# HDembinski/zenflow

Hardware: AMD Instinct MI355X
Metric: log_prob samples/sec (+ NLL match) 4D 16-knot 4-layer flow, batch 2^20 (higher is better)
Workload: dtype fp32 (f16x2 split MFMA, fp32 accumulate)

## Files before the change

zenflow_amd/build.py:

```python

from __future__ import annotations

import hashlib
import os
import subprocess
import sys
from concurrent.futures import ThreadPoolExecutor
from pathlib import Path

HERE = Path(__file__).resolve().parent
CSRC = HERE / "csrc"
INCLUDE = HERE.parent / "include"
LIB = HERE / "libzenflow_amd.so"
ARCH = os.environ.get("ZF_OFFLOAD_ARCH", "gfx950")
HIPCC = os.environ.get("HIPCC", "/opt/rocm/bin/hipcc")

SOURCES = ["zf_runtime.hip", "zf_rqs.hip", "zf_flow.hip", "zf_flow_x3.hip", "zf_flow_x3_k8.hip", "zf_flow_x3_k16.hip", "zf_flow_x3_k32.hip", "zf_flow_x3_k64.hip", "zf_flow_x3_k64_act.hip", "zf_flow_x3_k8_act.hip", "zf_flow_x3_k16_act.hip", "zf_flow_x3_k32_act.hip", "zf_flow_x3_k8_act2.hip", "zf_flow_x3_k16_act2.hip", "zf_flow_x3_k32_act2.hip", "zf_stats.hip", "zf_rccl.hip", "zf_train.hip", "zf_layered.hip"]
HEADERS = sorted(p.name for p in CSRC.glob("*.h"))

FLAGS = [
    f"--offload-arch={ARCH}",
    "-O3",
    "-std=c++17",
    "-fPIC",
    "-shared",
    "-Wall",
    "-Wno-unused-function",
    "-Wno-unused-variable",
    "-Wno-unused-result",
    "-I/opt/rocm/include",
    f"-I{INCLUDE}",
]

X3_FLAGS = ["-fno-slp-vectorize"]


def _src_flags(src: str):
    return X3_FLAGS if src.startswith("zf_flow_x3_k") else []


def _fingerprint() -> str:
    h = hashlib.sha256()
    for f in SOURCES + HEADERS:
        h.update((CSRC / f).read_bytes())
    h.update((INCLUDE / "zenflow_amd.h").read_bytes())
    h.update(" ".join(FLAGS + X3_FLAGS).encode())
    return h.hexdigest()


def build(force: bool = False, verbose: bool = True, out: Path = LIB, extra=()) -> Path:
    stamp = out.parent / f".{out.stem}.sha256"
    fp = _fingerprint() + " ".join(extra)
    if not force and out.exists() and stamp.exists() and stamp.read_text() == fp:
        return out
    tmp = out.with_suffix(".so.tmp")
    objdir = HERE.parent / "build" / ("obj" if not extra else "obj_" + hashlib.sha1(" ".join(extra).encode()).hexdigest()[:8])
    objdir.mkdir(parents=True, exist_ok=True)
    compile_flags = [f for f in FLAGS if f != "-shared"] + list(extra)

    hdr = hashlib.sha256(b"".join((CSRC / f).read_bytes() for f in HEADERS) + (INCLUDE / "zenflow_amd.h").read_bytes())

    def _compile(src: str) -> Path:
        obj = objdir / (Path(src).stem + ".o")
        cmd = [HIPCC, *compile_flags, *_src_flags(src), "-c", "-o", str(obj), str(CSRC / src)]
        key = hashlib.sha256(hdr.digest() + (CSRC / src).read_bytes() + " ".join(cmd).encode()).hexdigest()
        ostamp = obj.with_suffix(".o.sha256")
        if not force and obj.exists() and ostamp.exists() and ostamp.read_text() == key:
            return obj
        if verbose:
            print("[zenflow_amd.build]", " ".join(cmd), flush=True)
        subprocess.run(cmd, check=True)
        ostamp.write_text(key)
        return obj

    jobs = max(1, min(len(SOURCES), int(os.environ.get("MAX_JOBS", os.cpu_count() or 1))))
    with ThreadPoolExecutor(jobs) as pool:
        objs = list(pool.map(_compile, SOURCES))
    cmd = [HIPCC, f"--offload-arch={ARCH}", "-shared", "-fPIC", "-o", str(tmp), *map(str, objs), "-ldl"]
    if verbose:
        print("[zenflow_amd.build]", " ".join(cmd), flush=True)
    subprocess.run(cmd, check=True)
    os.replace(tmp, out)
    stamp.write_text(fp)
    return out


if __name__ == "__main__":
    argv = sys.argv[1:]
    o = LIB
    if "--out" in argv:
        i = argv.index("--out")
        o = Path(argv[i + 1]).resolve()
        del argv[i : i + 2]
    build(force="--force" in argv, out=o, extra=[a for a in argv if a.startswith("-D")])
```

zenflow_amd/csrc/zf_flow.hip:

```cpp
#include "zf_flow_dev.h"

#include <cmath>
#include <cstdlib>
#include <cstring>
#include <vector>

namespace zf {
namespace {

constexpr int kWaves = 4;
constexpr int kBlockRows = kWaves * kTile;

template <int T>
__device__ __forceinline__ floatx16 mfma_tile(const floatx4* __restrict__ p,
                                              const floatx4* __restrict__ pnext, floatx4 (&cur)[4],
                                              const floatx16 (&hb)[T]) {
  floatx16 acc = floatx16{0};
#pragma unroll
  for (int t = 0; t < T; ++t) {
    floatx4 nxt[4];
    const bool more = (t + 1 < T);
    const floatx4* src = more ? p + (t + 1) * 256 : pnext;
    const bool have = more || (pnext != nullptr);
    if (have) {
#pragma unroll
      for (int r4 = 0; r4 < 4; ++r4) {
        nxt[r4] = src[r4 * 64];
      }
    }
    asm volatile("" ::: "memory");
#pragma unroll
    for (int r4 = 0; r4 < 4; ++r4)
#pragma unroll
      for (int e = 0; e < 4; ++e)
        acc = __builtin_amdgcn_mfma_f32_32x32x2f32(cur[r4][e], hb[t][4 * r4 + e], acc, 0, 0, 0);
    if (have) {
#pragma unroll
      for (int r4 = 0; r4 < 4; ++r4) cur[r4] = nxt[r4];
    }
  }
  return acc;
}

struct RingParams {
  const float* ring;
  int base;
  int K, mask;
  float sx, sy, rsx, rsy;
  float c, norm, rnorm;
  __device__ __forceinline__ float at(int q) const { return ring[(q & mask) << 5]; }
  __device__ __forceinline__ float w(int j) const {
    return div_cr(div_cr(at(base + j), sx, rsx) + c, norm, rnorm);
  }
  __device__ __forceinline__ float h(int j) const {
    return div_cr(div_cr(at(base + K + j), sy, rsy) + c, norm, rnorm);
  }
  __device__ __forceinline__ float d(int j) const { return squareplus_fast(at(base + 2 * K + j)); }
};

template <bool INV>
__device__ __forceinline__ void spline_pair(float* ring, float* xs, int s, int hh, int next_d, int end,
                                            int S, int K, int mask, float cth, float norm, float rnorm,
                                            int rot, int D, float& ldc) {
  const int d = next_d + hh;
  float ldv = 0.f;
  if (d < end) {
    RingParams p;
    p.ring = ring + s;
    p.base = d * S;
    p.K = K;
    p.mask = (mask << 5) | 31;
    p.c = cth;
    p.norm = norm;
    p.rnorm = rnorm;
    float* rp = ring + s;
    float sx = 0.f, sy = 0.f;
    for (int j = 0; j < K; ++j) {
      const int qx = p.base + j, qy = p.base + K + j;
      float* ax = rp + ((qx & p.mask) << 5);
      float* ay = rp + ((qy & p.mask) << 5);
      const float vx = squareplus_fast(*ax), vy = squareplus_fast(*ay);
      *ax = vx;
      *ay = vy;
      sx = sx + vx;
      sy = sy + vy;
    }
    p.sx = sx;
    p.sy = sy;
    p.rsx = rcp_refined(sx);
    p.rsy = rcp_refined(sy);
    float* xp = xs + wrap(d + rot, D) * 32 + s;
    const float xv = *xp;
    const RqsBin bin = rqs_bin<!INV>(xv, K, p);
    if (!INV) {
      float yv, l;
      rqs_forward_eval(xv, bin, yv, l);
      *xp = yv;
      ldv = l;
    } else {
      *xp = rqs_inverse_eval(xv, bin);
    }
  }
  wave_lds_sync();
  if (!INV) {
    const float other = __shfl_xor(ldv, 32);
    const float first = hh == 0 ? ldv : other;
    const float second = hh == 0 ? other : ldv;
    ldc = ldc + first;
    if (end - next_d == 2) ldc = ldc + second;
  }
}

template <int HP, bool INV>
__global__ __launch_bounds__(kWaves * 64, (HP <= 128 ? 2 : 1)) void flow_kernel(
    const DevFlow* __restrict__ F, const float* __restrict__ blob, const float* __restrict__ xin,
    const float* __restrict__ cin, float* __restrict__ y_out, const float* __restrict__ ld_in,
    float* __restrict__ ld_out, float* __restrict__ lp_out, double* __restrict__ block_partial,
    int op_begin, int op_end, long long N, unsigned long long seed, int gen) {
  constexpr int T = HP / 32;
  extern __shared__ __attribute__((aligned(16))) float lds[];
  __shared__ double s_part[kWaves];

  const int D = F->D;
  const int C = F->C;
  const int wave = threadIdx.x >> 6;
  const int lane = threadIdx.x & 63;
  const int s = lane & 31;
  const int hh = lane >> 5;
  float* xs = lds + wave * F->per_wave;
  float* ring = xs + 32 * D;
  const long long row = ((long long)blockIdx.x * kWaves + wave) * kTile + s;
  const bool valid = row < N;

  load_state(xs, xin, row, valid, D, s, hh, F, seed, INV ? gen : 0);
  float ld = (ld_in != nullptr && valid) ? ld_in[row] : 0.f;
  int rot = 0;
  wave_lds_sync();

  floatx4 wc[4];
  const int nq = op_end - op_begin;
  for (int q = 0; q < nq; ++q) {
    const int oi = INV ? (op_end - 1 - q) : (op_begin + q);
    const DevOp& op = F->ops[oi];
    const int kind = op.kind;
    if (kind == ZF_OP_ROLL) {
      rot = pmod(INV ? rot + op.shift : rot - op.shift, D);
    } else if (kind == ZF_OP_SHIFT_BOUNDS) {
      shift_bounds_op<INV>(blob + op.sb, xs, s, hh, rot, D, ld);
    } else {
      const int dt = op.dt;
      {
        const floatx4* f = reinterpret_cast<const floatx4*>(blob + op.first_chunk) + lane;
#pragma unroll
        for (int r4 = 0; r4 < 4; ++r4) wc[r4] = f[r4 * 64];
      }
      floatx16 hb[T];
      layer0<T>(op, blob, xs, cin, row, valid, C, rot, D, s, hh, lane, hb, T, op.act);
      for (int l = 1; l < op.n_hidden; ++l) {
        const floatx4* wl = reinterpret_cast<const floatx4*>(blob + op.w[l]) + lane;
        const floatx4* wnext = reinterpret_cast<const floatx4*>(blob + op.w[l + 1]) + lane;
        floatx16 ho[T];
#pragma unroll
        for (int o = 0; o < T; ++o) {
          const floatx4* nx = (o + 1 < T) ? wl + (o + 1) * T * 256 : wnext;
          floatx4 bv[4];
          bias_tile(blob + op.b[l] + o * 32, hh, bv);
          floatx16 acc = mfma_tile<T>(wl + o * T * 256, nx, wc, hb);
          if (op.act == ZF_ACT_SWISH) {
#pragma unroll
            for (int r = 0; r < 16; ++r) acc[r] = swish(acc[r] + bv[r >> 2][r & 3]);
          } else {
#pragma unroll
            for (int r = 0; r < 16; ++r) acc[r] = act_other(op.act, acc[r] + bv[r >> 2][r & 3]);
          }
          ho[o] = acc;
        }
#pragma unroll
        for (int o = 0; o < T; ++o) hb[o] = ho[o];
      }
      const int K = op.K, S = op.S, mask = op.nslot_mask;
      const floatx4* wl = reinterpret_cast<const floatx4*>(blob + op.w[op.n_hidden]) + lane;
      const float* bl = blob + op.b[op.n_hidden];
      const KnotConsts kc(K);
      const float cth = kc.c, norm = kc.norm, rnorm = kc.rnorm;
      int next_d = 0;
      float ldc = 0.f;
      const int T_last = op.T_last;
      for (int o = 0; o < T_last; ++o) {
        const floatx4* nx = (o + 1 < T_last) ? wl + (o + 1) * T * 256 : nullptr;
        floatx4 bv[4];
        bias_tile(bl + o * 32, hh, bv);
        floatx16 acc = mfma_tile<T>(wl + o * T * 256, nx, wc, hb);
        float* slot = ring + ((o & mask) << 10) + s;
#pragma unroll
        for (int r = 0; r < 16; ++r) {
          const int rr = (r & 3) + 8 * (r >> 2) + 4 * hh;
          slot[rr * 32] = acc[r] + bv[r >> 2][r & 3];
        }
        wave_lds_sync();
        if (o + 1 < T_last) {
          while (next_d < dt) {
            const int end = (next_d + 2 < dt) ? next_d + 2 : dt;
            if (end * S > (o + 1) * 32) break;
            spline_pair<INV>(ring, xs, s, hh, next_d, end, S, K, mask, cth, norm, rnorm, rot, D, ldc);
            next_d += 2;
          }
        }
      }
      while (next_d < dt) {
        const int end = (next_d + 2 < dt) ? next_d + 2 : dt;
        spline_pair<INV>(ring, xs, s, hh, next_d, end, S, K, mask, cth, norm, rnorm, rot, D, ldc);
        next_d += 2;
      }
      if (!INV) ld = ld + ldc;
    }
  }

  flow_epilogue<kWaves>(F, xs, s, hh, lane, wave, rot, D, row, valid, ld, lp_out, block_partial, 1, 0,
                        y_out, ld_out, s_part);
}

__global__ __launch_bounds__(256) void latent_sample_kernel(int latent, float param, unsigned long long seed,
                                                            float* __restrict__ z, long long n, int D) {
  const long long i = (long long)blockIdx.x * 256 + threadIdx.x;
  if (i >= n) return;
  const long long row = i / D;
  const int d = (int)(i - row * D);
  z[i] = latent_draw(latent, param, seed, row, d);
}

constexpr int kReduceThreads = 1024;
__global__ __launch_bounds__(kReduceThreads) void reduce_partials(const double* __restrict__ part, long long n,
                                                                  double* __restrict__ out) {
  __shared__ double sm[kReduceThreads];
  const int t = threadIdx.x;
  double acc = 0.0;
  long long i = t;
  for (; i + 7 * kReduceThreads < n; i += 8 * kReduceThreads) {
    double v[8];
#pragma unroll
    for (int j = 0; j < 8; ++j) v[j] = part[i + j * kReduceThreads];
#pragma unroll
    for (int j = 0; j < 8; ++j) acc += v[j];
  }
  for (; i < n; i += kReduceThreads) acc += part[i];
  sm[t] = acc;
  __syncthreads();
  for (int w = kReduceThreads / 2; w >= 1; w >>= 1) {
    if (t < w) sm[t] += sm[t + w];
    __syncthreads();
  }
  if (t == 0) out[0] = sm[0];
}


int round_up(int a, int m) { return (a + m - 1) / m * m; }
int64_t round_up64(int64_t a, int64_t m) { return (a + m - 1) / m * m; }

int next_pow2(int v) {
  int p = 1;
  while (p < v) p <<= 1;
  return p;
}

struct OpGeom {
  int dt, dc, DC, K, S, OUT, KS0, T_last, nslot;
};

OpGeom nsc_geom(const zf_flow_desc* desc, const zf_op_desc& op) {
  OpGeom g;
  const int D = desc->dim;
  g.dt = D / 2;
  g.dc = D - g.dt;
  g.DC = g.dc + desc->cond_dim;
  g.K = op.knots;
  g.S = 3 * g.K - 1;
  g.OUT = g.dt * g.S;
  g.KS0 = (g.DC + 1) / 2;
  g.T_last = (g.OUT + 31) / 32;
  const int span = (g.dt >= 2 ? 2 * g.S : g.S);
  int need = (span + 31) / 32 + 1;
  if (need > g.T_last) need = g.T_last;
  g.nslot = next_pow2(need);
  return g;
}

int hidden_pad_of(const zf_flow_desc* desc) {
  int hmax = 0;
  for (int i = 0; i < desc->n_ops; ++i) {
    const zf_op_desc& op = desc->ops[i];
    if (op.kind != ZF_OP_NSC) continue;
    for (int l = 0; l < op.n_hidden; ++l) hmax = op.hidden[l] > hmax ? op.hidden[l] : hmax;
  }
  if (hmax == 0) return 32;
  int hp = 32;
  while (hp < hmax) hp <<= 1;
  return hp;
}

constexpr int kMaxFusedWidth = 256, kMaxLayeredWidth = 4096;
constexpr int kMaxFusedKnots = 64, kMaxLayeredKnots = 200;

int validate(const zf_flow_desc* desc) {
  if (!desc) return einval("desc is NULL");
  if (desc->dim < 1 || desc->dim > 64) return einval("dim %d out of range [1, 64]", desc->dim);
  if (desc->cond_dim < 0 || desc->cond_dim > 64) return einval("cond_dim out of range");
  if (desc->n_ops < 0 || desc->n_ops > kMaxOps) return einval("n_ops out of range");
  if (desc->latent < ZF_LATENT_NONE || desc->latent > ZF_LATENT_UNIFORM) return einval("bad latent");
  for (int i = 0; i < desc->n_ops; ++i) {
    const zf_op_desc& op = desc->ops[i];
    if (op.kind == ZF_OP_NSC) {
      if (desc->dim < 2) return einval("NeuralSplineCoupling needs dim >= 2");
      if (op.knots < 1 || op.knots > kMaxLayeredKnots)
        return einval("knots %d out of range [1, %d]", op.knots, kMaxLayeredKnots);
      if (op.n_hidden < 1 || op.n_hidden > 16) return enotsup("n_hidden must be in [1, 16]");
      for (int l = 0; l < op.n_hidden; ++l)
        if (op.hidden[l] < 1 || op.hidden[l] > kMaxLayeredWidth)
          return enotsup("hidden width must be in [1, 4096]");
      if (op.act < 0 || op.act >= ZF_ACT_COUNT) return einval("op %d: unknown activation %d", i, op.act);
    } else if (op.kind != ZF_OP_ROLL && op.kind != ZF_OP_SHIFT_BOUNDS) {
      return einval("op %d: unknown kind %d", i, op.kind);
    }
  }
  return ZF_OK;
}

}
}

struct zf_flow {
  zf_flow_desc desc;
  zf::DevFlow host;
  std::vector<float> natural;
  std::vector<float> packed;
  zf::DevFlow* d_desc = nullptr;
  float* d_blob = nullptr;
  void* d_x3 = nullptr;
  int x3_K = 0;
  bool x3_oact = false;
  int x3_aset = 0;
  int device = 0;
  zf::LayeredFlow* lay = nullptr;
};

namespace zf {
namespace {

void pack_nsc_bn(const zf_flow_desc* desc, const zf_op_desc& op, const float* nat, float* dst) {
  const OpGeom g = nsc_geom(desc, op);
  const int DCp = 2 * g.KS0;
  const float* mean = nat + op.off_bn;
  const float* var = mean + g.DC;
  const float* scale = var + g.DC;
  const float* bias = scale + g.DC;
  for (int k = 0; k < DCp; ++k) {
    if (k < g.DC) {
      const float mul = (1.0f / std::sqrt(var[k] + 1e-5f)) * scale[k];
      dst[k] = mean[k];
      dst[DCp + k] = mul;
      dst[2 * DCp + k] = bias[k];
    } else {
      dst[k] = dst[DCp + k] = dst[2 * DCp + k] = 0.f;
    }
  }
}

void pack_sb(const zf_flow_desc* desc, const zf_op_desc& op, const float* nat, float* dst) {
  for (int i = 0; i < desc->dim; ++i) {
    const float* r = nat + op.off_sb + 8 * i;
    const int mode = (int)r[0];
    const float a = r[1], b = r[2], xmin = r[3], xmax = r[4];
    float mul;
    if (mode == ZF_SB_BOTH) mul = (float)(1.0 / ((double)b - (double)a));
    else mul = 1.0f / (xmax - xmin);
    float* o = dst + 8 * i;
    o[0] = (float)mode; o[1] = a; o[2] = b; o[3] = xmin; o[4] = xmax;
    o[5] = mul; o[6] = std::log(mul); o[7] = 0.f;
  }
}

}
}

extern "C" {

int zf_flow_plan(zf_flow_desc* desc, int64_t* blob_floats) {
  int rc = zf::validate(desc);
  if (rc) return rc;
  if (!blob_floats) return zf::einval("blob_floats is NULL");
  int64_t off = 0;
  for (int i = 0; i < desc->n_ops; ++i) {
    zf_op_desc& op = desc->ops[i];
    op.off_bn = op.off_sb = 0;
    for (int l = 0; l < 17; ++l) op.off_w[l] = op.off_b[l] = 0;
    if (op.kind == ZF_OP_NSC) {
      const zf::OpGeom g = zf::nsc_geom(desc, op);
      op.off_bn = off;
      off += 4 * g.DC;
      int in = g.DC;
      for (int l = 0; l <= op.n_hidden; ++l) {
        const int out = l < op.n_hidden ? op.hidden[l] : g.OUT;
        op.off_w[l] = off;
        off += (int64_t)in * out;
        op.off_b[l] = off;
        off += out;
        in = out;
      }
    } else if (op.kind == ZF_OP_SHIFT_BOUNDS) {
      op.off_sb = off;
      off += 8 * desc->dim;
    }
  }
  *blob_floats = off;
  return ZF_OK;
}

int zf_flow_create(const zf_flow_desc* desc_in, const float* blob_host, int64_t blob_floats,
                   zf_flow_t** handle) {
  if (!handle) return zf::einval("handle is NULL");
  *handle = nullptr;
  zf_flow_desc desc = *desc_in;
  int64_t need = 0;
  int rc = zf_flow_plan(&desc, &need);
  if (rc) return rc;
  if (blob_floats != need) return zf::einval("blob has %lld floats, plan needs %lld", (long long)blob_floats, (long long)need);
  if (need > 0 && !blob_host) return zf::einval("blob is NULL");

  zf_flow* h = new zf_flow();
  h->desc = desc;
  h->natural.assign(blob_host, blob_host + need);
  zf::DevFlow& F = h->host;
  std::memset(&F, 0, sizeof(F));
  F.D = desc.dim;
  F.C = desc.cond_dim;
  F.latent = desc.latent;
  F.n_ops = desc.n_ops;
  F.HP = zf::hidden_pad_of(&desc);
  int kmax_ops = 0;
  for (int i = 0; i < desc.n_ops; ++i)
    if (desc.ops[i].kind == ZF_OP_NSC && desc.ops[i].knots > kmax_ops) kmax_ops = desc.ops[i].knots;
  const bool layered = F.HP > zf::kMaxFusedWidth || kmax_ops > zf::kMaxFusedKnots;
  if (layered) F.HP = 32;
  int x3K = 0;
  const bool x3 = !layered && zf::x3_eligible(desc, F.HP < 128 ? 128 : F.HP, &x3K);
  if (x3 && F.HP < 128) F.HP = 128;
  const int HP = F.HP, T = HP / 32;
  {
    const float s2 = 0.1f * 0.1f;
    F.lat_c0 = std::log(6.28318530717958647692f * s2);
    F.lat_c1 = s2;
    if (desc.latent == ZF_LATENT_BETA) {
      const double a = desc.latent_param;
      F.lat_c0 = (float)(-(std::lgamma(a) + std::lgamma(a) - std::lgamma(2.0 * a)));
      F.lat_c1 = (float)a - 1.0f;
      F.lat_c3 = (float)a;
    } else if (desc.latent == ZF_LATENT_TRUNCNORM) {
      const float nd = (float)(0.5 * std::erfc(5.0 / std::sqrt(2.0)));
      F.lat_c2 = std::log1p(-nd - nd);
    }
  }
  int64_t off = 0;
  auto take = [&](int64_t n) { const int64_t o = off; off = zf::round_up64(off + n, 4); return o; };
  int nslot = 1;
  for (int i = 0; i < desc.n_ops; ++i) {
    const zf_op_desc& op = desc.ops[i];
    zf::DevOp& d = F.ops[i];
    d.kind = op.kind;
    d.shift = op.shift;
    if (op.kind == ZF_OP_NSC) {
      const zf::OpGeom g = zf::nsc_geom(&desc, op);
      d.K = g.K; d.S = g.S; d.n_hidden = op.n_hidden; d.dt = g.dt; d.dc = g.dc; d.DC = g.DC;
      d.KS0 = g.KS0; d.T_last = g.T_last; d.nslot_mask = g.nslot - 1; d.act = op.act;
      nslot = g.nslot > nslot ? g.nslot : nslot;
      d.bn = take(3 * 2 * g.KS0);
      if (layered) continue;
      d.w[0] = take((int64_t)T * g.KS0 * 64);
      for (int l = 0; l < op.n_hidden; ++l) d.b[l] = take((int64_t)T * 32);
      d.b[op.n_hidden] = take((int64_t)g.T_last * 32);
      d.x3 = -1;
      if (x3) d.x3_blast = take((int64_t)zf::x3_pairs(desc) * zf::x3_last_tiles(x3K) * 32);
    } else if (op.kind == ZF_OP_SHIFT_BOUNDS) {
      d.sb = take(8 * desc.dim);
    }
  }
  F.small_floats = (int)off;
  for (int i = 0; i < desc.n_ops; ++i) {
    const zf_op_desc& op = desc.ops[i];
    zf::DevOp& d = F.ops[i];
    if (op.kind != ZF_OP_NSC || layered) continue;
    const zf::OpGeom g = zf::nsc_geom(&desc, op);
    for (int l = 1; l < op.n_hidden; ++l) d.w[l] = take((int64_t)T * T * 1024);
    d.w[op.n_hidden] = take((int64_t)g.T_last * T * 1024);
    d.first_chunk = op.n_hidden > 1 ? d.w[1] : d.w[op.n_hidden];
  }
  F.nslot = nslot;
  F.per_wave = zf::round_up(32 * desc.dim, 4) + nslot * 1024;
  h->packed.assign((size_t)(off > 0 ? off : 4), 0.f);
  float* P = h->packed.data();
  const float* nat = h->natural.data();
  for (int i = 0; i < desc.n_ops; ++i) {
    const zf_op_desc& op = desc.ops[i];
    const zf::DevOp& d = F.ops[i];
    if (op.kind == ZF_OP_SHIFT_BOUNDS) {
      zf::pack_sb(&desc, op, nat, P + d.sb);
    } else if (op.kind == ZF_OP_NSC) {
      const zf::OpGeom g = zf::nsc_geom(&desc, op);
      zf::pack_nsc_bn(&desc, op, nat, P + d.bn);
      if (layered) continue;
      {
        const int in = g.DC, out = op.hidden[0];
        const float* W = nat + op.off_w[0];
        const float* B = nat + op.off_b[0];
        for (int o = 0; o < T; ++o)
          for (int ks = 0; ks < g.KS0; ++ks)
            for (int l = 0; l < 64; ++l) {
              const int k = 2 * ks + (l >> 5), ii = 32 * o + (l & 31);
              P[d.w[0] + ((int64_t)o * g.KS0 + ks) * 64 + l] = (k < in && ii < out) ? W[(int64_t)k * out + ii] : 0.f;
            }
        for (int o = 0; o < T; ++o)
          for (int hh = 0; hh < 2; ++hh)
            for (int r = 0; r < 16; ++r) {
              const int ii = 32 * o + (r & 3) + 8 * (r >> 2) + 4 * hh;
              P[d.b[0] + (o * 2 + hh) * 16 + r] = ii < out ? B[ii] : 0.f;
            }
      }
      for (int l = 1; l <= op.n_hidden; ++l) {
        const int in = op.hidden[l - 1];
        const int out = l < op.n_hidden ? op.hidden[l] : g.OUT;
        const int To = l < op.n_hidden ? T : g.T_last;
        const float* W = nat + op.off_w[l];
        const float* B = nat + op.off_b[l];
        float* Wp = P + d.w[l];
        for (int o = 0; o < To; ++o)
          for (int t = 0; t < T; ++t)
            for (int r4 = 0; r4 < 4; ++r4)
              for (int ln = 0; ln < 64; ++ln)
                for (int e = 0; e < 4; ++e) {
                  const int k = 32 * t + e + 8 * r4 + 4 * (ln >> 5);
                  const int ii = 32 * o + (ln & 31);
                  Wp[((((int64_t)o * T + t) * 4 + r4) * 64 + ln) * 4 + e] =
                      (k < in && ii < out) ? W[(int64_t)k * out + ii] : 0.f;
                }
        for (int o = 0; o < To; ++o)
          for (int hh = 0; hh < 2; ++hh)
            for (int r = 0; r < 16; ++r) {
              const int ii = 32 * o + (r & 3) + 8 * (r >> 2) + 4 * hh;
              P[d.b[l] + (o * 2 + hh) * 16 + r] = ii < out ? B[ii] : 0.f;
            }
      }
    }
  }
  std::vector<uint16_t> x3s;
  const int NT = zf::x3_scheme_for(desc);
  if (x3) {
    const int tl = desc.dim / 2 == 1 ? (3 * x3K - 1 + 31) / 32 : zf::x3_last_tiles(x3K);
    int maxp = 0;
    for (int i = 0; i < desc.n_ops; ++i) {
      if (desc.ops[i].kind != ZF_OP_NSC) continue;
      zf::DevOp& d = F.ops[i];
      const int64_t end = d.x3_blast + (int64_t)zf::x3_pairs(desc) * tl * 32;
      d.x3_par_pieces = (int)((end - d.bn) * 4 + 1023) / 1024;
      maxp = d.x3_par_pieces > maxp ? d.x3_par_pieces : maxp;
    }
    F.x3_par_bytes = maxp * 1024;
  }
  if (x3 && zf::x3_lds_bytes(zf::x3_buf_tiles(desc, T, x3K), desc.dim + desc.cond_dim, NT, F.x3_par_bytes) <=
                160 * 1024) {
    zf::x3_pack(desc, nat, T, NT, x3K, F, P, x3s);
    F.x3_ok = NT == 3 ? 1 : 2;
    h->x3_K = x3K;
    for (int i = 0; i < desc.n_ops; ++i)
      if (desc.ops[i].kind == ZF_OP_NSC) F.kreal = desc.ops[i].knots;
    for (int i = 0; i < desc.n_ops; ++i)
      if (desc.ops[i].kind == ZF_OP_NSC && desc.ops[i].act != ZF_ACT_SWISH) h->x3_oact = true;
    {
      bool centred = false, plain = false;
      for (int i = 0; i < desc.n_ops; ++i) {
        if (desc.ops[i].kind != ZF_OP_NSC || desc.ops[i].act == ZF_ACT_SWISH) continue;
        if (desc.ops[i].act == ZF_ACT_SIGMOID || desc.ops[i].act == ZF_ACT_SOFTPLUS) centred = true;
        else plain = true;
      }
      h->x3_aset = centred && plain ? 0 : centred ? 2 : 1;
    }
  }
  const bool use_x3 = F.x3_ok != 0;
  int rcd = ZF_OK;
  hipError_t e = hipGetDevice(&h->device);
  if (e == hipSuccess && layered) {
    rcd = zf::layered_create(desc, nat, need, &h->lay);
    if (rcd) {
      zf_flow_destroy(h);
      return rcd;
    }
  }
  if (e == hipSuccess && use_x3) e = hipMalloc(&h->d_x3, x3s.size() * sizeof(uint16_t));
  if (e == hipSuccess && use_x3)
    e = hipMemcpy(h->d_x3, x3s.data(), x3s.size() * sizeof(uint16_t), hipMemcpyHostToDevice);
  if (e == hipSuccess) e = hipMalloc(&h->d_desc, sizeof(zf::DevFlow));
  if (e == hipSuccess) e = hipMalloc(&h->d_blob, h->packed.size() * sizeof(float) + 1024);
  if (e == hipSuccess) e = hipMemcpy(h->d_desc, &h->host, sizeof(zf::DevFlow), hipMemcpyHostToDevice);
  if (e == hipSuccess)
    e = hipMemcpy(h->d_blob, h->packed.data(), h->packed.size() * sizeof(float), hipMemcpyHostToDevice);
  if (e != hipSuccess) {
    rcd = zf::hip_status(e, "zf_flow_create");
    zf_flow_destroy(h);
    return rcd;
  }
  *handle = h;
  return ZF_OK;
}

int zf_flow_destroy(zf_flow_t* h) {
  if (!h) return ZF_OK;
  if (h->d_desc) (void)hipFree(h->d_desc);
  if (h->d_blob) (void)hipFree(h->d_blob);
  if (h->d_x3) (void)hipFree(h->d_x3);
  zf::layered_destroy(h->lay);
  delete h;
  return ZF_OK;
}

int zf_flow_kernel_variant(const zf_flow_t* h) {
  if (!h) return -1;
  if (h->lay) return ZF_KERNEL_LAYERED;
  return h->host.x3_ok == 2 ? ZF_KERNEL_F16X2 : h->host.x3_ok ? ZF_KERNEL_BF16X3 : ZF_KERNEL_FP32;
}

int64_t zf_flow_workspace_bytes(int64_t N) {
  const int64_t blocks = (N + zf::kBlockRows - 1) / zf::kBlockRows;
  return zf::round_up64(blocks * 8 + 64, 256);
}

}

namespace zf {
namespace {

template <bool INV>
int launch_flow(zf_flow* h, int op_begin, int op_end, const float* x, const float* c, float* y,
                const float* ld_in, float* ld_out, float* lp, double* part, int64_t N,
                void* stream, unsigned long long seed = 0, int gen = 0) {
  if (!h) return einval("handle is NULL");
  if (N < 0) return einval("N < 0");
  if (op_begin < 0 || op_end > h->host.n_ops || op_begin > op_end) return einval("bad op range");
  if (N == 0) return ZF_OK;
  if (!x && !gen) return einval("x is NULL");
  if (h->host.C > 0 && !c) return einval("flow is conditional (C=%d) but c is NULL", h->host.C);
  if (h->lay)
    return layered_run(h->lay, h->host, h->d_blob, INV, op_begin, op_end, x, c, y, ld_in, ld_out, lp, part, N,
                       (hipStream_t)stream, seed, gen);
  if (h->host.x3_ok) {
    X3Launch a;
    a.desc = h->d_desc; a.blob = h->d_blob; a.x3 = h->d_x3;
    a.x = x; a.c = c; a.y = y; a.ld_in = ld_in; a.ld_out = ld_out; a.lp = lp; a.part = part;
    a.nparts = (N + kBlockRows - 1) / kBlockRows;
    a.op_begin = op_begin; a.op_end = op_end; a.N = N; a.K = h->x3_K; a.D = h->host.D; a.C = h->host.C; a.T = h->host.HP / 32;
    a.NT = h->host.x3_ok == 2 ? 2 : 3;
    a.oact = h->x3_oact;
    a.aset = h->x3_aset;
    a.par_bytes = h->host.x3_par_bytes;
    a.seed = seed;
    a.gen = gen;
    a.stream = (hipStream_t)stream;
    return launch_flow_x3(a, INV);
  }
  const int64_t grid = (N + kBlockRows - 1) / kBlockRows;
  if (grid > 0x7fffffffLL) return einval("N too large");
  const size_t lds = sizeof(float) * (size_t)kWaves * h->host.per_wave;
  if (lds > 160 * 1024 - 64) return enotsup("LDS footprint too large (dim/knots)");
  hipStream_t st = (hipStream_t)stream;
  const long long n = (long long)N;
#define ZF_LAUNCH(HPV)                                                                          \
  hipLaunchKernelGGL((flow_kernel<HPV, INV>), dim3((unsigned)grid), dim3(kWaves * 64), lds, st, \
                     h->d_desc, h->d_blob, x, c, y, ld_in, ld_out, lp, part, op_begin, op_end, n, seed, gen)
  switch (h->host.HP) {
    case 32: ZF_LAUNCH(32); break;
    case 64: ZF_LAUNCH(64); break;
    case 128: ZF_LAUNCH(128); break;
    case 256: ZF_LAUNCH(256); break;
    default: return enotsup("hidden width");
  }
#undef ZF_LAUNCH
  ZF_CHECK_LAUNCH("flow_kernel");
  return ZF_OK;
}

}
}

extern "C" {

int zf_flow_log_prob_segment(zf_flow_t* h, int op_begin, int op_end, const float* x,
                             const float* c, const float* log_det_in, float* log_prob,
                             double* nll_sum, void* workspace, int64_t N, void* stream) {
  if (!h) return zf::einval("handle is NULL");
  if (!log_prob) return zf::einval("log_prob is NULL");
  if (h->host.latent == ZF_LATENT_NONE) return zf::einval("flow has no latent distribution");
  if (nll_sum && !workspace) return zf::einval("nll_sum requires a workspace");
  if (N == 0) {
    if (nll_sum) ZF_TRY_HIP(hipMemsetAsync(nll_sum, 0, sizeof(double), (hipStream_t)stream));
    return ZF_OK;
  }
  double* part = (double*)workspace;
  int rc = zf::launch_flow<false>(h, op_begin, op_end, x, c, nullptr, log_det_in, nullptr,
                                  log_prob, part, N, stream);
  if (rc) return rc;
  if (nll_sum) return zf_flow_nll_reduce(workspace, N, nll_sum, stream);
  return ZF_OK;
}

int zf_flow_nll_reduce(const void* workspace, int64_t N, double* nll_sum, void* stream) {
  if (!workspace || !nll_sum) return zf::einval("NULL argument");
  if (N <= 0) {
    ZF_TRY_HIP(hipMemsetAsync(nll_sum, 0, sizeof(double), (hipStream_t)stream));
    return ZF_OK;
  }
  const long long blocks = (N + zf::kBlockRows - 1) / zf::kBlockRows;
  hipLaunchKernelGGL(zf::reduce_partials, dim3(1), dim3(zf::kReduceThreads), 0, (hipStream_t)stream,
                     (const double*)workspace, blocks, nll_sum);
  ZF_CHECK_LAUNCH("reduce_partials");
  return ZF_OK;
}

int zf_flow_log_prob(zf_flow_t* h, const float* x, const float* c, float* log_prob,
                     double* nll_sum, void* workspace, int64_t N, void* stream) {
  if (!h) return zf::einval("handle is NULL");
  return zf_flow_log_prob_segment(h, 0, h->host.n_ops, x, c, nullptr, log_prob, nll_sum,
                                  workspace, N, stream);
}

int zf_flow_forward(zf_flow_t* h, int op_begin, int op_end, const float* x, const float* c,
                    float* y, const float* log_det_in, float* log_det, int64_t N, void* stream) {
  return zf::launch_flow<false>(h, op_begin, op_end, x, c, y, log_det_in, log_det, nullptr,
                                nullptr, N, stream);
}

int zf_flow_inverse(zf_flow_t* h, int op_begin, int op_end, const float* z, const float* c,
                    float* x, int64_t N, void* stream) {
  if (!x && N > 0) return zf::einval("x is NULL");
  return zf::launch_flow<true>(h, op_begin, op_end, z, c, x, nullptr, nullptr, nullptr, nullptr,
                               N, stream);
}

int zf_flow_sample(zf_flow_t* h, uint64_t seed, const float* c, float* x, int64_t N, void* stream) {
  if (!h) return zf::einval("handle is NULL");
  if (!x && N > 0) return zf::einval("x is NULL");
  if (h->host.latent == ZF_LATENT_NONE) return zf::einval("flow has no latent distribution");
  return zf::launch_flow<true>(h, 0, h->host.n_ops, nullptr, c, x, nullptr, nullptr, nullptr, nullptr,
                               N, stream, (unsigned long long)seed, 1);
}

int zf_latent_sample(int latent, double param, uint64_t seed, float* z, int64_t N, int D, void* stream) {
  if (latent < ZF_LATENT_NORMAL || latent > ZF_LATENT_UNIFORM) return zf::einval("bad latent %d", latent);
  if (latent == ZF_LATENT_BETA && !(param >= 1.0)) return zf::einval("Beta peakness must be >= 1");
  if (N < 0 || D < 1) return zf::einval("bad shape");
  if (N == 0) return ZF_OK;
  if (!z) return zf::einval("z is NULL");
  const long long n = (long long)N * D;
  const long long grid = (n + 255) / 256;
  if (grid > 0x7fffffffLL) return zf::einval("N too large");
  hipLaunchKernelGGL(zf::latent_sample_kernel, dim3((unsigned)grid), dim3(256), 0, (hipStream_t)stream, latent,
                     (float)param, (unsigned long long)seed, z, n, D);
  ZF_CHECK_LAUNCH("latent_sample_kernel");
  return ZF_OK;
}

static int upload_region(zf_flow* h, int64_t off, int64_t n) {
  ZF_TRY_HIP(hipSetDevice(h->device));
  ZF_TRY_HIP(hipDeviceSynchronize());
  ZF_TRY_HIP(hipMemcpy(h->d_blob + off, h->packed.data() + off, n * sizeof(float),
                       hipMemcpyHostToDevice));
  return ZF_OK;
}

int zf_flow_set_bn_stats(zf_flow_t* h, int op, const float* mean, const float* var) {
  if (!h || !mean || !var) return zf::einval("NULL argument");
  if (op < 0 || op >= h->desc.n_ops || h->desc.ops[op].kind != ZF_OP_NSC) return zf::einval("op %d is not an NSC", op);
  const zf_op_desc& od = h->desc.ops[op];
  const zf::OpGeom g = zf::nsc_geom(&h->desc, od);
  float* nat = h->natural.data() + od.off_bn;
  for (int k = 0; k < g.DC; ++k) { nat[k] = mean[k]; nat[g.DC + k] = var[k]; }
  zf::pack_nsc_bn(&h->desc, od, h->natural.data(), h->packed.data() + h->host.ops[op].bn);
  return upload_region(h, h->host.ops[op].bn, 3 * 2 * g.KS0);
}

int zf_flow_set_sb_stats(zf_flow_t* h, int op, const float* xmin, const float* xmax) {
  if (!h || !xmin || !xmax) return zf::einval("NULL argument");
  if (op < 0 || op >= h->desc.n_ops || h->desc.ops[op].kind != ZF_OP_SHIFT_BOUNDS) return zf::einval("op %d is not a ShiftBounds", op);
  const zf_op_desc& od = h->desc.ops[op];
  for (int i = 0; i < h->desc.dim; ++i) {
    h->natural[od.off_sb + 8 * i + 3] = xmin[i];
    h->natural[od.off_sb + 8 * i + 4] = xmax[i];
  }
  zf::pack_sb(&h->desc, od, h->natural.data(), h->packed.data() + h->host.ops[op].sb);
  return upload_region(h, h->host.ops[op].sb, 8 * h->desc.dim);
}

}
```

zenflow_amd/csrc/zf_flow_dev.h:

```cpp
#pragma once
#include "zf_act.h"
#include "zf_internal.h"
#include "zf_random.h"
#include "zf_spline.h"

#include <cstdint>
#include <vector>

namespace zf {

typedef float floatx16 __attribute__((ext_vector_type(16)));
typedef float floatx4 __attribute__((ext_vector_type(4)));

constexpr int kTile = 32;
constexpr int kMaxOps = 64;

struct DevOp {
  int kind, shift, K, S;
  int n_hidden, dt, dc, DC;
  int KS0, T_last, nslot_mask, act;
  long long w[17];
  long long b[17];
  long long bn;
  long long sb;
  long long first_chunk;
  long long x3;
  long long x3_blast;
  int x3_groups, x3_tlast;
  int x3_next[2];
  int x3_kw[17];
  float x3_rb[16][2];
  int x3_par_pieces;
  long long x3_nbase[2], x3_nbn[2];
  int x3_npieces[2], x3_npar[2];
};

struct DevFlow {
  int D, C, latent, n_ops;
  int HP, nslot, per_wave, x3_ok;
  int small_floats;
  int x3_par_bytes;
  int kreal;
  int _pad;
  float lat_c0, lat_c1, lat_c2, lat_c3;
  DevOp ops[kMaxOps];
};

__device__ __forceinline__ void wave_lds_sync() {
  __builtin_amdgcn_fence(__ATOMIC_SEQ_CST, "wavefront");
  __builtin_amdgcn_wave_barrier();
}

__device__ __forceinline__ float swish(float v) {
  return v * __builtin_amdgcn_rcpf(1.0f + __builtin_amdgcn_exp2f(-v * 1.44269504f));
}

__device__ __forceinline__ float rcp_refined(float x) {
  float r = __builtin_amdgcn_rcpf(x);
  return __builtin_fmaf(__builtin_fmaf(-x, r, 1.0f), r, r);
}

__device__ __forceinline__ float div_cr(float x, float d, float r) {
  const float q = x * r;
  return __builtin_fmaf(__builtin_fmaf(-q, d, x), r, q);
}

__device__ __forceinline__ float squareplus_fast(float x) {
  const float a = x * x + 4.0f;
  float sq = __builtin_amdgcn_sqrtf(a);
  sq = __builtin_fmaf(__builtin_fmaf(-sq, sq, a), 0.5f * __builtin_amdgcn_rcpf(sq), sq);
  return 0.5f * (x + sq);
}

__device__ __forceinline__ void bias_tile(const float* __restrict__ bt, int hh, floatx4 (&b)[4]) {
  const floatx4* p = reinterpret_cast<const floatx4*>(bt + hh * 16);
#pragma unroll
  for (int r4 = 0; r4 < 4; ++r4) b[r4] = p[r4];
}

__device__ __forceinline__ floatx16 bias_acc(const float* __restrict__ bt, int hh) {
#if defined(ZF_X3_ABL) && ZF_X3_ABL == 7
  floatx16 z;
#pragma unroll
  for (int r = 0; r < 16; ++r) z[r] = 0.01f * (r + hh);
  return z;
#endif
  floatx4 b[4];
  bias_tile(bt, hh, b);
  floatx16 a;
#pragma unroll
  for (int r = 0; r < 16; ++r) a[r] = b[r >> 2][r & 3];
  return a;
}

__device__ __forceinline__ int pmod(int a, int m) {
  int r = a % m;
  return r < 0 ? r + m : r;
}

__device__ __forceinline__ int wrap(int a, int m) { return a >= m ? a - m : a; }

struct KnotConsts {
  float c, norm, rnorm;
  __device__ __forceinline__ explicit KnotConsts(int K) {
    const double c64 = 1e-5 / (1.0 - (double)K * 1e-5);
    c = (float)c64;
    norm = (float)(1.0 + c64 * (double)K);
    rnorm = rcp_refined(norm);
  }
};

__device__ __forceinline__ void load_state(float* xs, const float* __restrict__ xin, long long row,
                                           bool valid, int D, int s, int hh, const DevFlow* __restrict__ F,
                                           unsigned long long seed, int gen) {
  for (int d = hh; d < D; d += 2) {
    float v = 0.f;
    if (valid) v = gen ? latent_draw(F->latent, F->lat_c3, seed, row, d) : xin[row * D + d];
    xs[d * 32 + s] = v;
  }
}

__device__ __forceinline__ float sb_forward_elem(const float* __restrict__ r, float v, float& l) {
  const int mode = (int)r[0];
  const float a = r[1], b = r[2], xmin = r[3];
  const float mul = r[5], logmul = r[6];
  if (mode == ZF_SB_BOTH) {
    l = logmul;
    return (v - a) * mul;
  }
  float t = v;
  if (mode == ZF_SB_LOWER) t = logf((v - a) + 1.17549435e-38f);
  if (mode == ZF_SB_UPPER) t = logf((b - v) + 1.17549435e-38f);
  const float zr = (t - xmin) * mul;
  l = (mode == ZF_SB_NONE) ? logmul : logmul - t;
  return (zr != zr) ? zr : fminf(fmaxf(zr, 0.f), 1.f);
}

__device__ __forceinline__ float sb_inverse_elem(const float* __restrict__ r, float zv) {
  const int mode = (int)r[0];
  const float a = r[1], b = r[2];
  const float xmin = r[3], xmax = r[4];
  if (mode == ZF_SB_BOTH) return zv * b + (1.f - zv) * a;
  const float t = zv * xmax + (1.f - zv) * xmin;
  return (mode == ZF_SB_LOWER) ? expf(t) + a : (mode == ZF_SB_UPPER ? b - expf(t) : t);
}

template <bool INV>
__device__ __forceinline__ void shift_bounds_op(const float* __restrict__ sb, float* xs, int s, int hh,
                                                int rot, int D, float& ld) {
  if (!INV) {
    float ldsb = 0.f;
    for (int i = 0; i < D; ++i) {
      const int p = wrap(i + rot, D);
      float l;
      const float z = sb_forward_elem(sb + 8 * i, xs[p * 32 + s], l);
      ldsb = ldsb + l;
      if (hh == 0) xs[p * 32 + s] = z;
    }
    ld = ld + ldsb;
  } else {
    for (int i = 0; i < D; ++i) {
      const int p = wrap(i + rot, D);
      const float xv = sb_inverse_elem(sb + 8 * i, xs[p * 32 + s]);
      if (hh == 0) xs[p * 32 + s] = xv;
    }
  }
  wave_lds_sync();
}

template <int T>
__device__ __forceinline__ void layer0(const DevOp& op, const float* __restrict__ blob, const float* xs,
                                       const float* __restrict__ cin, long long row, bool valid, int C,
                                       int rot, int D, int s, int hh, int lane, floatx16 (&hb)[T],
                                       int swish_tiles = T, int act = ZF_ACT_SWISH) {
  const int dt = op.dt, dc = op.dc, DC = op.DC, KS0 = op.KS0;
  const int DCp = 2 * KS0;
  const float* bn = blob + op.bn;
#pragma unroll
  for (int o = 0; o < T; ++o) hb[o] = bias_acc(blob + op.b[0] + o * 32, hh);
  for (int ks = 0; ks < KS0; ++ks) {
    const int k = 2 * ks + hh;
    float v = 0.f;
    if (k < dc) v = xs[wrap(dt + k + rot, D) * 32 + s];
    else if (k < DC) v = valid ? cin[row * C + (k - dc)] : 0.f;
#if defined(ZF_X3_ABL) && ZF_X3_ABL == 7
    const float u = (v - 0.1f) * 1.1f + 0.01f;
#pragma unroll
    for (int o = 0; o < T; ++o)
      hb[o] = __builtin_amdgcn_mfma_f32_32x32x2f32(0.01f * (o + lane), u, hb[o], 0, 0, 0);
#else
    const float u = (v - bn[k]) * bn[DCp + k] + bn[2 * DCp + k];
    const float* w0 = blob + op.w[0] + ks * 64 + lane;
#pragma unroll
    for (int o = 0; o < T; ++o)
      hb[o] = __builtin_amdgcn_mfma_f32_32x32x2f32(w0[o * KS0 * 64], u, hb[o], 0, 0, 0);
#endif
  }
  if (act != ZF_ACT_SWISH) {
#pragma unroll
    for (int o = 0; o < T; ++o)
#pragma unroll
      for (int r = 0; r < 16; ++r) hb[o][r] = act_other(act, hb[o][r]);
    return;
  }
#pragma unroll
  for (int o = 0; o < T; ++o)
    if (o < swish_tiles)
#pragma unroll
      for (int r = 0; r < 16; ++r) hb[o][r] = swish(hb[o][r]);
}

__device__ __forceinline__ float latent_logpdf(int lt, float c0, float c1, float c2, float v) {
  float t;
  if (lt == ZF_LATENT_NORMAL || lt == ZF_LATENT_TRUNCNORM) {
    const float dv = v - 0.5f;
    t = (c0 + (dv * dv) / c1) / -2.0f;
    if (lt == ZF_LATENT_TRUNCNORM) {
      t = t - c2;
      const float xsd = dv / 0.1f;
      if (xsd < -5.f || xsd > 5.f) t = -INFINITY;
    }
  } else if (lt == ZF_LATENT_BETA) {
    const float l1 = (c1 == 0.f) ? 0.f : c1 * logf(v);
    const float l2 = (c1 == 0.f) ? 0.f : c1 * log1pf(-v);
    t = c0 + (l1 + l2);
    if (v > 1.f || v < 0.f) t = -INFINITY;
  } else {
    t = (v > 1.f || v < 0.f) ? -INFINITY : 0.f;
  }
  return t;
}

__device__ __forceinline__ float nan_to_num_lp(float lp) {
  if (lp != lp) lp = -INFINITY;
  if (lp == INFINITY) lp = 3.40282347e38f;
  if (lp == -INFINITY) lp = -3.40282347e38f;
  return lp;
}

template <int NW>
__device__ __forceinline__ void flow_epilogue(const DevFlow* __restrict__ F, const float* xs, int s,
                                              int hh, int lane, int wave, int rot, int D, long long row,
                                              bool valid, float ld, float* __restrict__ lp_out,
                                              double* __restrict__ block_partial, int pstride,
                                              long long nparts, float* __restrict__ y_out,
                                              float* __restrict__ ld_out, double* s_part,
                                              long long slot = -1) {
  if (lp_out != nullptr) {
    float lat = 0.f;
    for (int j = 0; j < D; ++j)
      lat = lat + latent_logpdf(F->latent, F->lat_c0, F->lat_c1, F->lat_c2, xs[wrap(j + rot, D) * 32 + s]);
    const float lp = nan_to_num_lp(lat + ld);
    if (valid && hh == 0) lp_out[row] = lp;
    if (block_partial != nullptr) {
      double v = (valid && hh == 0) ? (double)lp : 0.0;
#pragma unroll
      for (int m = 32; m >= 1; m >>= 1) v += __shfl_xor(v, m);
      if (lane == 0) s_part[wave] = v;
      __syncthreads();
      if (threadIdx.x == 0) {
        double acc = 0.0;
        for (int w = 0; w < NW; ++w) acc += s_part[w];
        const long long b0 = slot >= 0 ? slot : (long long)blockIdx.x * pstride;
        block_partial[b0] = acc;
        for (int k = 1; k < pstride; ++k)
          if (b0 + k < nparts) block_partial[b0 + k] = 0.0;
      }
    }
  }
  if (y_out != nullptr && valid) {
    for (int j = hh; j < D; j += 2) y_out[row * D + j] = xs[wrap(j + rot, D) * 32 + s];
  }
  if (ld_out != nullptr && valid && hh == 0) ld_out[row] = ld;
}

struct X3Launch {
  const DevFlow* desc;
  const float* blob;
  const void* x3;
  const float *x, *c;
  float* y;
  const float* ld_in;
  float *ld_out, *lp;
  double* part;
  long long nparts;
  int op_begin, op_end;
  long long N;
  unsigned long long seed;
  int gen;
  int K, D, C, T;
  int NT;
  bool oact;
  int aset;
  int par_bytes;
  hipStream_t stream;
};
int launch_flow_x3(const X3Launch& a, bool inverse);
bool x3_eligible(const zf_flow_desc& desc, int HP, int* K);
struct LayeredFlow;
int layered_create(const zf_flow_desc& desc, const float* natural, int64_t n, LayeredFlow** out);
void layered_destroy(LayeredFlow* L);
int layered_run(LayeredFlow* L, const DevFlow& F, const float* packed, bool inverse, int op_begin, int op_end,
                const float* x, const float* c, float* y, const float* ld_in, float* ld_out, float* lp, double* part,
                long long N, hipStream_t st, unsigned long long seed, int gen);
int x3_last_tiles(int K);
int x3_pairs(const zf_flow_desc& desc);
int x3_buf_tiles(const zf_flow_desc& desc, int T, int K);
size_t x3_lds_bytes(int TB, int D, int NT, int par_bytes);
int x3_scheme();
int x3_scheme_for(const zf_flow_desc& desc);
void x3_pack(const zf_flow_desc& desc, const float* nat, int T, int NT, int Kp, DevFlow& F, float* packed,
             std::vector<uint16_t>& stream);

}
```

zenflow_amd/csrc/zf_flow_x3.hip:

```cpp
#include "zf_flow_x3_kernel.h"

#include <cmath>
#include <cstdint>
#include <cstdlib>
#include <cstring>
#include <vector>

namespace zf {

int launch_x3_k8(const X3Launch& a, bool inverse);
int launch_x3_k16(const X3Launch& a, bool inverse);
int launch_x3_k32(const X3Launch& a, bool inverse);
int launch_x3_k64(const X3Launch& a, bool inverse);

namespace {

uint16_t bf16_rne(float f) {
  uint32_t u;
  std::memcpy(&u, &f, 4);
  if ((u & 0x7fffffffu) > 0x7f800000u) return (uint16_t)((u >> 16) | 0x40);
  u += 0x7fffu + ((u >> 16) & 1u);
  return (uint16_t)(u >> 16);
}

float bf16_f(uint16_t b) {
  const uint32_t u = (uint32_t)b << 16;
  float f;
  std::memcpy(&f, &u, 4);
  return f;
}

}

int x3_padded_knots(int K);
int x3_param_of(int jp, int Kp, int K, float* fill);

bool x3_eligible(const zf_flow_desc& desc, int HP, int* K_out) {
  const char* env = std::getenv("ZF_DISABLE_X3");
  if (env && env[0] == '1') return false;
  int K = 0;
  for (int i = 0; i < desc.n_ops; ++i) {
    const zf_op_desc& op = desc.ops[i];
    if (op.kind != ZF_OP_NSC) continue;
    if (op.act == ZF_ACT_SOFTPLUS && x3_scheme() == 3) return false;
    if (op.act != ZF_ACT_SWISH && x3_scheme() == 3) return false;
    if (op.knots < 2) return false;
    if (op.knots > K) K = op.knots;
  }
  const int Kp = x3_padded_knots(K);
  if (HP > 256 || desc.dim > 64 || Kp == 0) return false;
  *K_out = Kp;
  return true;
}

int x3_padded_knots(int K) {
  if (K < 2) return 0;
  if (K <= 8) return 8;
  if (K <= 16) return 16;
  if (K <= 32) return 32;
  if (K <= 64) return 64;
  return 0;
}

int x3_param_of(int jp, int Kp, int K, float* fill) {
  if (jp < Kp) {
    *fill = -1099511627776.0f;
    return jp < K ? jp : -1;
  }
  if (jp < 2 * Kp) {
    *fill = -1099511627776.0f;
    return jp - Kp < K ? K + (jp - Kp) : -1;
  }
  const int q = jp - 2 * Kp;
  *fill = q == K - 1 ? 0.0f : __builtin_nanf("");
  return q < K - 1 ? 2 * K + q : -1;
}

int x3_scheme() {
  const char* env = std::getenv("ZF_X3_SCHEME");
  if (env && std::strcmp(env, "bf16x3") == 0) return 3;
  return 2;
}

int x3_scheme_for(const zf_flow_desc& desc) {
  (void)desc;
  return x3_scheme() == 3 ? 3 : 2;
}

int x3_last_tiles(int K) { return (3 * K - 1 + 15) / 16; }
int x3_last_tiles_one(int K) { return (3 * K - 1 + 31) / 32; }

int x3_pairs(const zf_flow_desc& desc) { return (desc.dim / 2 + 1) / 2; }

void x3_pack(const zf_flow_desc& desc, const float* nat, int T, int NT, int Kp, DevFlow& F, float* packed,
             std::vector<uint16_t>& stream) {
  stream.clear();
  int prev = -1;
  for (int i = 0; i < desc.n_ops; ++i) {
    F.ops[i].x3_next[0] = F.ops[i].x3_next[1] = -1;
    if (desc.ops[i].kind != ZF_OP_NSC) continue;
    if (prev >= 0) { F.ops[prev].x3_next[0] = i; F.ops[i].x3_next[1] = prev; }
    prev = i;
  }
  for (int i = 0; i < desc.n_ops; ++i) {
    const zf_op_desc& op = desc.ops[i];
    if (op.kind != ZF_OP_NSC) continue;
    DevOp& d = F.ops[i];
    const int dt = desc.dim / 2, K = Kp, S = 3 * K - 1;
    const int Kr = op.knots, Sr = 3 * Kr - 1;
    const bool one = dt == 1;
    const int TL = one ? x3_last_tiles_one(K) : x3_last_tiles(K), NP = x3_pairs(desc);
    d.x3 = (long long)stream.size() * 2;
    d.x3_tlast = TL;
    d.x3_groups = T * (op.n_hidden - 1) + T * NP;
    for (int l = 1; l <= op.n_hidden; ++l) {
      const bool last = (l == op.n_hidden);
      const int in = op.hidden[l - 1];
      const int out = last ? dt * Sr : op.hidden[l];
      const int NOUT = last ? TL : T;
      const float* W = nat + op.off_w[l];
      const float pre = (NT == 2 && !last && op.act == ZF_ACT_SWISH) ? kSwishPrescale : 1.0f;
      int kw = 0;
      if (NT == 2) {
        float mx = 0.f;
        for (int64_t i = 0; i < (int64_t)in * out; ++i)
          mx = std::fmax(mx, std::fabs(W[i] * pre));
        if (mx > 0.f && std::isfinite(mx)) {
          int e;
          std::frexp(mx, &e);
          kw = 14 - e;
        }
      }
      d.x3_kw[l] = kw;
      for (int pr = 0; pr < (last ? NP : 1); ++pr)
        for (int q = 0; q < T; ++q)
          for (int s = 0; s < 2; ++s)
            for (int o = 0; o < NOUT; ++o) {
              uint16_t part[3][64][8];
              for (int ln = 0; ln < 64; ++ln)
                for (int j = 0; j < 8; ++j) {
                  const int kstep = 2 * q + s;
                  const int k = 16 * kstep + 8 * (j >> 2) + 4 * (ln >> 5) + (j & 3);
                  const int rho = ln & 31;
                  int col;
                  if (!last) {
                    col = 32 * o + rho;
                    if (col >= out) col = -1;
                  } else {
                    const int h = (rho >> 2) & 1, r = (rho & 3) + 4 * (rho >> 3);
                    const int jp = one ? 32 * o + 16 * h + r : 16 * o + r;
                    const int dd = one ? 0 : 2 * pr + h;
                    float fill;
                    const int jr = jp < S ? x3_param_of(jp, K, Kr, &fill) : -1;
                    col = (dd < dt && jr >= 0) ? dd * Sr + jr : -1;
                  }
                  const float x = (k < in && col >= 0) ? W[(int64_t)k * out + col] : 0.f;
                  if (NT == 3) {
                    const uint16_t bh = bf16_rne(x);
                    const float r1 = x - bf16_f(bh);
                    const uint16_t bm = bf16_rne(r1);
                    const uint16_t bl = bf16_rne(r1 - bf16_f(bm));
                    part[0][ln][j] = bh;
                    part[1][ln][j] = bm;
                    part[2][ln][j] = bl;
                  } else {
                    const float xs = std::ldexp(x * pre, kw);
                    const _Float16 h = (_Float16)xs;
                    const _Float16 lo = (_Float16)(xs - (float)h);
                    std::memcpy(&part[0][ln][j], &h, 2);
                    std::memcpy(&part[1][ln][j], &lo, 2);
                  }
                }
              const uint16_t* pp = &part[0][0][0];
              stream.insert(stream.end(), pp, pp + NT * 64 * 8);
            }
    }
    std::vector<double> lastfold;
    if (NT == 2 && (op.act == ZF_ACT_SIGMOID || op.act == ZF_ACT_SOFTPLUS)) {
      const double C = op.act == ZF_ACT_SIGMOID ? 0.5 : 0.69314718055994530942;
      for (int l = 1; l <= op.n_hidden; ++l) {
        const bool last = l == op.n_hidden;
        const int in = op.hidden[l - 1];
        const int out = last ? dt * Sr : op.hidden[l];
        const float* W = nat + op.off_w[l];
        std::vector<double> cs(out, 0.0);
        for (int k = 0; k < in; ++k)
          for (int j = 0; j < out; ++j) cs[j] += (double)W[(int64_t)k * out + j];
        if (last) {
          for (double& v : cs) v *= C;
          lastfold.swap(cs);
          continue;
        }
        for (int o = 0; o < T; ++o)
          for (int hh = 0; hh < 2; ++hh)
            for (int r = 0; r < 16; ++r) {
              const int ii = 32 * o + (r & 3) + 8 * (r >> 2) + 4 * hh;
              if (ii < out) {
                float& b = packed[d.b[l] + (o * 2 + hh) * 16 + r];
                b = (float)((double)b + C * cs[ii]);
              }
            }
      }
    }
    if (NT == 2 && op.act == ZF_ACT_SWISH) {
      const int KS0 = d.KS0;
      for (int64_t i = 0; i < (int64_t)T * KS0 * 64; ++i) packed[d.w[0] + i] *= kSwishPrescale;
      for (int l = 0; l < op.n_hidden; ++l)
        for (int64_t i = 0; i < (int64_t)T * 32; ++i) packed[d.b[l] + i] *= kSwishPrescale;
    }
    for (int l = 0; l < 16; ++l) d.x3_rb[l][0] = d.x3_rb[l][1] = 0.f;
    if (NT == 2 && op.act == ZF_ACT_SWISH) {
      const double pre = kSwishPrescale;
      for (int l = 0; l < op.n_hidden && l < 16; ++l) {
        const int in = l == 0 ? desc.dim - dt + desc.cond_dim : op.hidden[l - 1];
        const int out = op.hidden[l];
        const float* W = nat + op.off_w[l];
        const float* Bv = nat + op.off_b[l];
        double R = 0.0, Bm = 0.0;
        for (int j = 0; j < out; ++j) {
          double rs = 0.0;
          for (int k = 0; k < in; ++k) rs += std::fabs((double)W[(int64_t)k * out + j]);
          R = std::fmax(R, rs * pre);
          Bm = std::fmax(Bm, std::fabs((double)Bv[j]) * pre);
        }
        d.x3_rb[l][0] = (float)(R * (1.0 + 0x1p-20));
        d.x3_rb[l][1] = (float)(Bm * (1.0 + 0x1p-20));
      }
    }
    d.x3_npieces[0] = d.x3_npieces[1] = (2 * (op.n_hidden > 1 ? T : TL) * NT * 1024) >> 10;
    const float* B = nat + op.off_b[op.n_hidden];
    for (int pr = 0; pr < NP; ++pr)
      for (int o = 0; o < TL; ++o)
        for (int h = 0; h < 2; ++h)
          for (int r = 0; r < 16; ++r) {
            const int jp = one ? 32 * o + 16 * h + r : 16 * o + r, dd = one ? 0 : 2 * pr + h;
            float fill = 0.f;
            const int jr = (dd < dt && jp < S) ? x3_param_of(jp, K, Kr, &fill) : -1;
            float b = 0.f;
            if (jr >= 0)
              b = lastfold.empty() ? B[dd * Sr + jr] : (float)((double)B[dd * Sr + jr] + lastfold[dd * Sr + jr]);
            else if (dd < dt && jp < S)
              b = fill;
            packed[d.x3_blast + ((pr * TL + o) * 2 + h) * 16 + r] = b;
          }
  }
  std::vector<int> own(desc.n_ops, 0);
  for (int i = 0; i < desc.n_ops; ++i) own[i] = desc.ops[i].kind == ZF_OP_NSC ? F.ops[i].x3_npieces[0] : 0;
  for (int i = 0; i < desc.n_ops; ++i) {
    if (desc.ops[i].kind != ZF_OP_NSC) continue;
    DevOp& d = F.ops[i];
    for (int dir = 0; dir < 2; ++dir) {
      const int n = d.x3_next[dir];
      d.x3_nbase[dir] = n >= 0 ? F.ops[n].x3 : -1;
      d.x3_nbn[dir] = n >= 0 ? F.ops[n].bn : 0;
      d.x3_npieces[dir] = n >= 0 ? own[n] : 0;
      d.x3_npar[dir] = n >= 0 ? F.ops[n].x3_par_pieces : 0;
    }
  }
}

int x3_buf_tiles(const zf_flow_desc& desc, int T, int K) {
  const int TL = desc.dim / 2 == 1 ? x3_last_tiles_one(K) : x3_last_tiles(K);
  return T > TL ? T : TL;
}

size_t x3_lds_bytes(int TB, int D, int NT, int par_bytes) {
  return (size_t)2 * 2 * TB * NT * 1024 + (size_t)2 * par_bytes + (size_t)kX3Waves * 32 * D * 4 +
         kX3Waves * sizeof(double);
}

int launch_flow_x3(const X3Launch& a, bool inverse) {
  if (a.NT != 2 && a.NT != 3) return einval("split-MFMA kernel: scheme %d", a.NT);
  if (a.K == 8) return launch_x3_k8(a, inverse);
  if (a.K == 16) return launch_x3_k16(a, inverse);
  if (a.K == 32) return launch_x3_k32(a, inverse);
  if (a.K == 64) return launch_x3_k64(a, inverse);
  return enotsup("split-MFMA kernel: knots not instantiated");
}

}
```

zenflow_amd/csrc/zf_flow_x3_k16.hip:

```cpp
#include "zf_flow_x3_kernel.h"

namespace zf {

int launch_x3_k16_act(const X3Launch& a, bool inverse);

int launch_x3_k16(const X3Launch& a, bool inverse) {
  if (a.oact) return launch_x3_k16_act(a, inverse);
  return a.NT == 2 ? launch_x3_k<2, 16>(a, inverse) : launch_x3_k<3, 16>(a, inverse);
}

}

#ifdef ZF_X3_TRACE
extern "C" int zf_x3_trace_set_k16(void* buf) {
  return hipMemcpyToSymbol(HIP_SYMBOL(zf::x3_trace_buf), &buf, sizeof(buf)) == hipSuccess ? 0 : 1;
}
#endif
```

zenflow_amd/csrc/zf_flow_x3_kernel.h:

```cpp
#pragma once
#include "zf_flow_dev.h"

#include <cmath>
#include <cstdint>
#include <cstdlib>
#include <cstring>
#include <utility>
#include <vector>

namespace zf {
namespace {

typedef float floatx2 __attribute__((ext_vector_type(2)));
typedef __bf16 bf16x2 __attribute__((ext_vector_type(2)));
typedef __bf16 bf16x8 __attribute__((ext_vector_type(8)));
typedef _Float16 halfx2 __attribute__((ext_vector_type(2)));
typedef _Float16 halfx8 __attribute__((ext_vector_type(8)));

template <int NT>
struct XT;
template <>
struct XT<3> {
  using E = bf16x8;
  static constexpr int kProd = 6;
};
template <>
struct XT<2> {
  using E = halfx8;
  static constexpr int kProd = 3;
};

constexpr int kWideSched = 3;

#ifndef ZF_X3_WAVES
#define ZF_X3_WAVES 4
#endif
constexpr int kX3Waves = ZF_X3_WAVES;
static_assert(kX3Waves % 4 == 0, "whole 128-row NLL partial slots per block");

#ifndef ZF_X3_ABL
#define ZF_X3_ABL 0
#endif
#ifdef ZF_X3_TRACE
constexpr int kX3TraceSlots = 16;
__device__ unsigned long long* x3_trace_buf;
#define X3T_NOW() __builtin_amdgcn_s_memtime()
#endif
template <int NT>
constexpr int group_bytes(int NOUT) { return 2 * NOUT * NT * 1024; }


template <int S>
__device__ __forceinline__ void split8(const floatx16& v, bf16x8& bh, bf16x8& bm, bf16x8& bl) {
#pragma unroll
  for (int i = 0; i < 4; ++i) {
    const floatx2 x = {v[8 * S + 2 * i], v[8 * S + 2 * i + 1]};
    const bf16x2 h = __builtin_convertvector(x, bf16x2);
    const floatx2 r = x - __builtin_convertvector(h, floatx2);
    const bf16x2 m = __builtin_convertvector(r, bf16x2);
    const floatx2 r2 = r - __builtin_convertvector(m, floatx2);
    const bf16x2 l = __builtin_convertvector(r2, bf16x2);
    bh[2 * i] = h[0]; bh[2 * i + 1] = h[1];
    bm[2 * i] = m[0]; bm[2 * i + 1] = m[1];
    bl[2 * i] = l[0]; bl[2 * i + 1] = l[1];
  }
}

template <int S>
__device__ __forceinline__ void split8h(const floatx16& v, halfx8& bh, halfx8& bl) {
  uint32_t h[4], l[4];
#pragma unroll
  for (int i = 0; i < 4; ++i) {
    const halfx2 hv = __builtin_convertvector(floatx2{v[8 * S + 2 * i], v[8 * S + 2 * i + 1]}, halfx2);
    __builtin_memcpy(&h[i], &hv, 4);
  }
  asm(
      "v_fma_mixlo_f16 %0, %4, 1.0, -%12 op_sel_hi:[0,0,1]\n\t"
      "v_fma_mixhi_f16 %0, %5, 1.0, -%12 op_sel:[0,0,1] op_sel_hi:[0,0,1]\n\t"
      "v_fma_mixlo_f16 %1, %6, 1.0, -%13 op_sel_hi:[0,0,1]\n\t"
      "v_fma_mixhi_f16 %1, %7, 1.0, -%13 op_sel:[0,0,1] op_sel_hi:[0,0,1]\n\t"
      "v_fma_mixlo_f16 %2, %8, 1.0, -%14 op_sel_hi:[0,0,1]\n\t"
      "v_fma_mixhi_f16 %2, %9, 1.0, -%14 op_sel:[0,0,1] op_sel_hi:[0,0,1]\n\t"
      "v_fma_mixlo_f16 %3, %10, 1.0, -%15 op_sel_hi:[0,0,1]\n\t"
      "v_fma_mixhi_f16 %3, %11, 1.0, -%15 op_sel:[0,0,1] op_sel_hi:[0,0,1]\n\t"
      "s_nop 1"
      : "=&v"(l[0]), "=&v"(l[1]), "=&v"(l[2]), "=&v"(l[3])
      : "v"(v[8 * S + 0]), "v"(v[8 * S + 1]), "v"(v[8 * S + 2]), "v"(v[8 * S + 3]), "v"(v[8 * S + 4]),
        "v"(v[8 * S + 5]), "v"(v[8 * S + 6]), "v"(v[8 * S + 7]), "v"(h[0]), "v"(h[1]), "v"(h[2]), "v"(h[3]));
  __builtin_memcpy(&bh, h, 16);
  __builtin_memcpy(&bl, l, 16);
}

template <int S>
__device__ __forceinline__ void split8h_hi(const floatx16& v, uint32_t (&h)[4]) {
#pragma unroll
  for (int i = 0; i < 4; ++i) {
    const halfx2 hv = __builtin_convertvector(floatx2{v[8 * S + 2 * i], v[8 * S + 2 * i + 1]}, halfx2);
    __builtin_memcpy(&h[i], &hv, 4);
  }
}

template <int S>
__device__ __forceinline__ void split8h_lo(const floatx16& v, const uint32_t (&h)[4], halfx8& bh, halfx8& bl) {
  uint32_t l[4];
  asm("v_fma_mixlo_f16 %0, %4, 1.0, -%12 op_sel_hi:[0,0,1]\n\t"
      "v_fma_mixhi_f16 %0, %5, 1.0, -%12 op_sel:[0,0,1] op_sel_hi:[0,0,1]\n\t"
      "v_fma_mixlo_f16 %1, %6, 1.0, -%13 op_sel_hi:[0,0,1]\n\t"
      "v_fma_mixhi_f16 %1, %7, 1.0, -%13 op_sel:[0,0,1] op_sel_hi:[0,0,1]\n\t"
      "v_fma_mixlo_f16 %2, %8, 1.0, -%14 op_sel_hi:[0,0,1]\n\t"
      "v_fma_mixhi_f16 %2, %9, 1.0, -%14 op_sel:[0,0,1] op_sel_hi:[0,0,1]\n\t"
      "v_fma_mixlo_f16 %3, %10, 1.0, -%15 op_sel_hi:[0,0,1]\n\t"
      "v_fma_mixhi_f16 %3, %11, 1.0, -%15 op_sel:[0,0,1] op_sel_hi:[0,0,1]\n\t"
      "s_nop 1"
      : "=&v"(l[0]), "=&v"(l[1]), "=&v"(l[2]), "=&v"(l[3])
      : "v"(v[8 * S + 0]), "v"(v[8 * S + 1]), "v"(v[8 * S + 2]), "v"(v[8 * S + 3]), "v"(v[8 * S + 4]),
        "v"(v[8 * S + 5]), "v"(v[8 * S + 6]), "v"(v[8 * S + 7]), "v"(h[0]), "v"(h[1]), "v"(h[2]), "v"(h[3]));
  __builtin_memcpy(&bh, h, 16);
  __builtin_memcpy(&bl, l, 16);
}

template <int NT, int S>
__device__ __forceinline__ void splitk(const floatx16& v, typename XT<NT>::E (&b)[NT]) {
  if constexpr (NT == 3) {
    split8<S>(v, b[0], b[1], b[2]);
  } else {
    split8h<S>(v, b[0], b[1]);
  }
}

constexpr float kSwishPrescale = 1.44269504088896341f;

template <int NT>
__device__ __forceinline__ float act_swish(float v, float c) {
  if constexpr (NT == 2) {
    const float e = __builtin_amdgcn_exp2f(-v);
    return v * __builtin_amdgcn_rcpf(__builtin_fmaf(e, c, c));
  }
  return swish(v);
}

template <int CODE>
__device__ __forceinline__ void act_tile_fixed(floatx16& t, float c) {
#pragma unroll
  for (int r = 0; r < 16; ++r) t[r] = act_other(CODE, t[r]) * c;
}

constexpr float kLn2 = 0.693147180559945309f;
__device__ __forceinline__ float act_sigmoid_centered(float v) {
  const float d = 1.0f + __builtin_amdgcn_exp2f(-v * kSwishPrescale);
  const float q = __builtin_amdgcn_rcpf(d);
  const float sg = __builtin_fmaf(q, __builtin_fmaf(-d, q, 1.0f), q);
  const float v2 = v * v;
  const float ser =
      v * __builtin_fmaf(v2, __builtin_fmaf(v2, __builtin_fmaf(v2, -17.0f / 80640.0f, 1.0f / 480.0f), -1.0f / 48.0f),
                         0.25f);
  return fabsf(v) < 0.25f ? ser : (d == __builtin_huge_valf() ? 0.0f : sg) - 0.5f;
}
__device__ __forceinline__ float act_softplus_centered(float v) {
  const float t = __builtin_amdgcn_exp2f(-fabsf(v) * kSwishPrescale);
  const float sp = __builtin_fmaf(__builtin_amdgcn_logf(1.0f + t), kLn2, fmaxf(v, 0.0f));
  const float v2 = v * v;
  const float ser = v * __builtin_fmaf(v, __builtin_fmaf(v2, __builtin_fmaf(v2, 1.0f / 2880.0f, -1.0f / 192.0f), 0.125f),
                                       0.5f);
  return fabsf(v) >= 0.25f ? sp - kLn2 : ser;
}

template <int CODE>
__device__ __forceinline__ void act_tile_centered(floatx16& t, float c) {
#pragma unroll
  for (int r = 0; r < 16; ++r)
    t[r] = (CODE == ZF_ACT_SIGMOID ? act_sigmoid_centered(t[r]) : act_softplus_centered(t[r])) * c;
}

template <int CODE>
__device__ __forceinline__ void act_tile_plain(floatx16& t) {
#pragma unroll
  for (int r = 0; r < 16; ++r) t[r] = act_other(CODE, t[r]);
}

template <>
__device__ __forceinline__ void act_tile_plain<ZF_ACT_SIGMOID>(floatx16& t) {
#pragma unroll
  for (int r = 0; r < 16; ++r) {
    const float d = 1.0f + __builtin_amdgcn_exp2f(-t[r] * kSwishPrescale);
    const float q = __builtin_amdgcn_rcpf(d);
    const float c = __builtin_fmaf(q, __builtin_fmaf(-d, q, 1.0f), q);
    t[r] = d == __builtin_huge_valf() ? 0.0f : c;
  }
}

template <int NT, bool OACT, int ASET = 0>
__device__ __forceinline__ void x3_act_tile(floatx16& t, float c, int act) {
  if constexpr (!OACT) {
#pragma unroll
    for (int r = 0; r < 16; ++r) t[r] = act_swish<NT>(t[r], c);
  } else if constexpr (NT == 3) {
    switch (act) {
      case ZF_ACT_RELU: act_tile_plain<ZF_ACT_RELU>(t); break;
      case ZF_ACT_TANH: act_tile_plain<ZF_ACT_TANH>(t); break;
      case ZF_ACT_SIGMOID: act_tile_plain<ZF_ACT_SIGMOID>(t); break;
      case ZF_ACT_GELU: act_tile_plain<ZF_ACT_GELU>(t); break;
      case ZF_ACT_SOFTPLUS: act_tile_plain<ZF_ACT_SOFTPLUS>(t); break;
      case ZF_ACT_ELU: act_tile_plain<ZF_ACT_ELU>(t); break;
      case ZF_ACT_LEAKY_RELU: act_tile_plain<ZF_ACT_LEAKY_RELU>(t); break;
      default:
#pragma unroll
        for (int r = 0; r < 16; ++r) t[r] = swish(t[r]);
    }
  } else {
    if constexpr (ASET == 2) {
      switch (act) {
        case ZF_ACT_SIGMOID: act_tile_centered<ZF_ACT_SIGMOID>(t, c); break;
        case ZF_ACT_SOFTPLUS: act_tile_centered<ZF_ACT_SOFTPLUS>(t, c); break;
        default:
#pragma unroll
          for (int r = 0; r < 16; ++r) t[r] = act_swish<NT>(t[r], c);
      }
    } else {
      switch (act) {
        case ZF_ACT_RELU: act_tile_fixed<ZF_ACT_RELU>(t, c); break;
        case ZF_ACT_TANH: act_tile_fixed<ZF_ACT_TANH>(t, c); break;
        case ZF_ACT_GELU: act_tile_fixed<ZF_ACT_GELU>(t, c); break;
        case ZF_ACT_ELU: act_tile_fixed<ZF_ACT_ELU>(t, c); break;
        case ZF_ACT_LEAKY_RELU: act_tile_fixed<ZF_ACT_LEAKY_RELU>(t, c); break;
        case ZF_ACT_SIGMOID:
          if constexpr (ASET == 0) act_tile_centered<ZF_ACT_SIGMOID>(t, c);
          break;
        case ZF_ACT_SOFTPLUS:
          if constexpr (ASET == 0) act_tile_centered<ZF_ACT_SOFTPLUS>(t, c);
          break;
        default:
#pragma unroll
          for (int r = 0; r < 16; ++r) t[r] = act_swish<NT>(t[r], c);
      }
    }
  }
}

__device__ __forceinline__ floatx16 mfma3(const bf16x8& ah, const bf16x8& am, const bf16x8& al,
                                          const bf16x8& bh, const bf16x8& bm, const bf16x8& bl,
                                          floatx16 acc) {
  acc = __builtin_amdgcn_mfma_f32_32x32x16_bf16(am, bm, acc, 0, 0, 0);
  acc = __builtin_amdgcn_mfma_f32_32x32x16_bf16(ah, bl, acc, 0, 0, 0);
  acc = __builtin_amdgcn_mfma_f32_32x32x16_bf16(al, bh, acc, 0, 0, 0);
  acc = __builtin_amdgcn_mfma_f32_32x32x16_bf16(ah, bm, acc, 0, 0, 0);
  acc = __builtin_amdgcn_mfma_f32_32x32x16_bf16(am, bh, acc, 0, 0, 0);
  return __builtin_amdgcn_mfma_f32_32x32x16_bf16(ah, bh, acc, 0, 0, 0);
}

template <int NT>
__device__ __forceinline__ floatx16 mfma_split(const typename XT<NT>::E (&a)[NT], const typename XT<NT>::E (&b)[NT],
                                               floatx16 acc) {
  if constexpr (NT == 3) {
    return mfma3(a[0], a[1], a[2], b[0], b[1], b[2], acc);
  } else {
    acc = __builtin_amdgcn_mfma_f32_32x32x16_f16(a[1], b[0], acc, 0, 0, 0);
    acc = __builtin_amdgcn_mfma_f32_32x32x16_f16(a[0], b[1], acc, 0, 0, 0);
    return __builtin_amdgcn_mfma_f32_32x32x16_f16(a[0], b[0], acc, 0, 0, 0);
  }
}

template <int NT>
__device__ __forceinline__ void load_frag(const char* a, typename XT<NT>::E (&f)[NT]) {
  using E = typename XT<NT>::E;
  if constexpr (NT == 3) f[1] = *reinterpret_cast<const E*>(a + 1024);
  f[0] = *reinterpret_cast<const E*>(a);
  if constexpr (NT == 3) f[2] = *reinterpret_cast<const E*>(a + 2048);
  else f[1] = *reinterpret_cast<const E*>(a + 1024);
}

struct X3Halves {
  float lo, hi;
};
__device__ __forceinline__ X3Halves x3_halves(float x) {
  const auto r = __builtin_amdgcn_permlane32_swap(__float_as_int(x), __float_as_int(x), false, false);
  return {__int_as_float(r[0]), __int_as_float(r[1])};
}

template <int T, bool OACT = false>
__device__ __forceinline__ void x3_act_scale(const floatx16 (&hb)[T], int kw, float& isc, float& us, float& ius,
                                             int act = ZF_ACT_SWISH) {
  float m = 0.f;
#pragma unroll
  for (int t = 0; t < T; ++t)
#pragma unroll
    for (int r = 0; r < 16; ++r) m = fmaxf(m, fabsf(hb[t][r]));
  {
    const X3Halves q = x3_halves(m);
    m = fmaxf(q.lo, q.hi);
  }
  const int e = max(__builtin_amdgcn_frexp_expf(m), -60);
  isc = (OACT && act != ZF_ACT_SWISH) ? __builtin_amdgcn_ldexpf(1.0f, 14 - e)
                                      : __builtin_amdgcn_ldexpf(kSwishPrescale, e - 14);
  us = __builtin_amdgcn_ldexpf(1.0f, e - 14 - kw);
  ius = __builtin_amdgcn_ldexpf(1.0f, 14 + kw - e);
}

template <int NT>
__device__ __forceinline__ floatx16 x3_finish(const floatx16& acc, float us, const floatx16& b) {
  if constexpr (NT == 2) {
    floatx16 r;
#pragma unroll
    for (int i = 0; i < 16; ++i) r[i] = __builtin_fmaf(acc[i], us, b[i]);
    return r;
  } else {
    return acc + b;
  }
}

template <int NT, int T, int NOUT, int Q>
__device__ __forceinline__ void x3_group(const char* buf, const floatx16 (&hb)[T], floatx16 (&acc)[NOUT],
                                         int lane) {
  using E = typename XT<NT>::E;
  const char* lb = buf + lane * 16;
if constexpr (T == 8) {
  E c[NT];
  load_frag<NT>(lb, c);
#pragma unroll
  for (int s = 0; s < 2; ++s) {
    E b[NT];
    if (s == 0) splitk<NT, 0>(hb[Q], b);
    else splitk<NT, 1>(hb[Q], b);
#pragma unroll
    for (int o = 0; o < NOUT; ++o) {
      const int t = s * NOUT + o;
      E n[NT];
      if (t + 1 < 2 * NOUT) load_frag<NT>(lb + (((t + 1) * NT) << 10), n);
      acc[o] = mfma_split<NT>(c, b, acc[o]);
      if (t + 1 < 2 * NOUT) {
#pragma unroll
        for (int i = 0; i < NT; ++i) c[i] = n[i];
      }
    }
  }
} else {
#pragma unroll
  for (int s = 0; s < 2; ++s) {
    E b[NT];
    if (s == 0) splitk<NT, 0>(hb[Q], b);
    else splitk<NT, 1>(hb[Q], b);
#pragma unroll
    for (int o = 0; o < NOUT; ++o) {
      E a[NT];
      load_frag<NT>(lb + (((s * NOUT + o) * NT) << 10), a);
      acc[o] = mfma_split<NT>(a, b, acc[o]);
    }
  }
}
}

struct X3Span {
  long long base;
  long long next_base;
  int G, nhid;
  int last_pieces;
  int next_pieces;
};

template <int NT, int T>
__device__ __forceinline__ int first_pieces(const DevOp& op) {
  return (op.n_hidden > 1 ? group_bytes<NT>(T) : group_bytes<NT>(op.x3_tlast)) >> 10;
}

struct X3Sc {
  int kind, shift, nh, act, dt, dc, DC, KS0, G, tlast, nxt, npieces, npar, kw1, kw_last, kreal;
  long long x3, nbase, nbn, bn, w0_rel, b_rel, blast_rel, sb;
};

template <bool INV>
__device__ __forceinline__ X3Sc x3_scalars(const DevOp& op) {
  constexpr int d = INV ? 1 : 0;
  X3Sc c;
  c.kind = op.kind; c.shift = op.shift; c.nh = op.n_hidden; c.act = op.act;
  c.dt = op.dt; c.dc = op.dc; c.DC = op.DC; c.KS0 = op.KS0;
  c.G = op.x3_groups; c.tlast = op.x3_tlast; c.nxt = op.x3_next[d];
  c.npieces = op.x3_npieces[d]; c.npar = op.x3_npar[d];
  c.kw1 = op.x3_kw[1];
  c.kreal = op.K;
  c.kw_last = op.x3_kw[op.n_hidden & 15];
  c.x3 = op.x3; c.nbase = op.x3_nbase[d]; c.nbn = op.x3_nbn[d]; c.bn = op.bn;
  c.w0_rel = op.w[0] - op.bn; c.b_rel = op.b[0] - op.bn; c.blast_rel = op.x3_blast - op.bn;
  c.sb = op.sb;
  return c;
}

template <int NT, int T>
__device__ __forceinline__ X3Span make_span(const X3Sc& c, bool has_next) {
  X3Span sp;
  sp.base = c.x3;
  sp.G = c.G;
  sp.nhid = T * (c.nh - 1);
  sp.last_pieces = group_bytes<NT>(c.tlast) >> 10;
  sp.next_base = has_next ? c.nbase : -1;
  sp.next_pieces = has_next ? c.npieces : 0;
  return sp;
}

__device__ __forceinline__ void x3_dma(const char* __restrict__ src, char* dst, int pieces, int wave, int lane) {
#if ZF_X3_ABL == 5
  pieces = (pieces + 3) / 4;
#endif
  for (int p = wave; p < pieces; p += kX3Waves)
    __builtin_amdgcn_global_load_lds((const void*)(src + (p << 10) + lane * 16),
                                     (__attribute__((address_space(3))) void*)(dst + (p << 10)), 16, 0, 0);
}

struct X3Pipe {
  char* cur;
  char* nxt;
  int g;
  X3Span span;
  int wave;
  const char* par_src;
  char* par_dst;
  int par_pieces;
#ifdef ZF_X3_TRACE
  unsigned long long tbar;
  unsigned long long tdma;
  unsigned long long tgrp;
#endif
};

template <int NT, int T>
__device__ __forceinline__ void x3_issue_next(const char* __restrict__ x3, const X3Pipe& p, char* dst, int lane) {
  constexpr int kHid = group_bytes<NT>(T);
  if (p.g == 0 && p.par_src != nullptr) x3_dma(p.par_src, p.par_dst, p.par_pieces, p.wave, lane);
  const int g = p.g + 1;
#if ZF_X3_ABL == 6
  if (g > 1 && g < p.span.G) return;
#endif
  long long off;
  int pieces;
  if (g < p.span.nhid) {
    off = p.span.base + (long long)g * kHid;
    pieces = kHid >> 10;
  } else if (g < p.span.G) {
    off = p.span.base + (long long)p.span.nhid * kHid + (long long)(g - p.span.nhid) * (p.span.last_pieces << 10);
    pieces = p.span.last_pieces;
  } else {
    if (p.span.next_base < 0) return;
    off = p.span.next_base;
    pieces = p.span.next_pieces;
  }
  x3_dma(x3 + off, dst, pieces, p.wave, lane);
}

template <int NT, int T, int NOUT, int Q, bool SW, bool OACT>
__device__ __forceinline__ void x3_step(const char* __restrict__ x3, X3Pipe& p, floatx16 (&hb)[T],
                                        floatx16 (&acc)[NOUT], int lane, const float* __restrict__ bias,
                                        int hh, float isc, float us, int act) {
#ifdef ZF_X3_TRACE
  const unsigned long long tb0 = X3T_NOW();
#endif
  asm volatile("s_waitcnt vmcnt(0)" ::: "memory");
  __syncthreads();
#ifdef ZF_X3_TRACE
  p.tbar += X3T_NOW() - tb0;
#endif
#ifdef ZF_X3_TRACE
  const unsigned long long td0 = X3T_NOW();
#endif
  x3_issue_next<NT, T>(x3, p, p.nxt, lane);
#ifdef ZF_X3_TRACE
  const unsigned long long td1 = X3T_NOW();
  p.tdma += td1 - td0;
#endif
  if (bias != nullptr) {
    floatx16 bt[NOUT];
#pragma unroll
    for (int o = 0; o < NOUT; ++o) bt[o] = bias_acc(bias + o * 32, hh);
    x3_group<NT, T, NOUT, Q>(p.cur, hb, acc, lane);
#pragma unroll
    for (int o = 0; o < NOUT; ++o) acc[o] = x3_finish<NT>(acc[o], us, bt[o]);
  } else {
    x3_group<NT, T, NOUT, Q>(p.cur, hb, acc, lane);
  }
#ifdef ZF_X3_TRACE
  {
    float sink = acc[0][0];
    asm volatile("; use %0" : "+v"(sink));
    p.tgrp += X3T_NOW() - td1;
  }
#endif
  if constexpr (SW && !OACT && Q + 1 < T) {
    x3_act_tile<NT, OACT>(hb[Q + 1], isc, act);
  }
  if constexpr (T == 8) {
    constexpr int kP = XT<NT>::kProd;
    __builtin_amdgcn_sched_group_barrier(0x100, NT, 0);
    __builtin_amdgcn_sched_group_barrier(0x402, 20, 0);
#pragma unroll
    for (int i = 0; i < 2 * kP * NOUT; ++i) {
      __builtin_amdgcn_sched_group_barrier(0x008, 1, 0);
      if ((NT == 3 && i % 2 == 0) || (NT == 2 && i % 3 != 2)) __builtin_amdgcn_sched_group_barrier(0x100, 1, 0);
      __builtin_amdgcn_sched_group_barrier(0x402, kWideSched, 0);
    }
  }
  char* const t = p.cur;
  p.cur = p.nxt;
  p.nxt = t;
  p.g += 1;
}

template <int NT, int T, int NOUT, int Q, bool HASB, bool OACT, int AS = 0>
__device__ __forceinline__ void x3_step_pipe(const char* __restrict__ x3, X3Pipe& p, floatx16 (&hb)[T],
                                             floatx16 (&acc)[NOUT], int lane, const float* __restrict__ bias,
                                             int hh, typename XT<NT>::E (&cs)[NT], float isc, float us,
                                             int act) {
  using E = typename XT<NT>::E;
#ifdef ZF_X3_TRACE
  const unsigned long long tb0 = X3T_NOW();
#endif
#if ZF_X3_ABL != 3
  asm volatile("s_waitcnt vmcnt(0)" ::: "memory");
  __syncthreads();
#endif
#ifdef ZF_X3_TRACE
  p.tbar += X3T_NOW() - tb0;
#endif
  x3_issue_next<NT, T>(x3, p, p.nxt, lane);
  const char* lb = p.cur + lane * 16;
  E s1[NT];
  splitk<NT, 1>(hb[Q], s1);
#if ZF_X3_ABL == 1
  E a1[NT];
  load_frag<NT>(lb, a1);
#endif
#pragma unroll
  for (int o = 0; o < NOUT; ++o) {
#if ZF_X3_ABL == 1
    acc[o] = mfma_split<NT>(a1, cs, acc[o]);
#else
    E a[NT];
    load_frag<NT>(lb + ((o * NT) << 10), a);
    acc[o] = mfma_split<NT>(a, cs, acc[o]);
#endif
  }
  if constexpr (Q + 1 < T) {
#if ZF_X3_ABL != 2
    if constexpr (!OACT || (NT == 2 && AS != 0)) x3_act_tile<NT, OACT, AS>(hb[Q + 1], isc, act);
#endif
    splitk<NT, 0>(hb[Q + 1], cs);
  }
#pragma unroll
  for (int o = 0; o < NOUT; ++o) {
#if ZF_X3_ABL == 1
    acc[o] = mfma_split<NT>(a1, s1, acc[o]);
#else
    E a[NT];
    load_frag<NT>(lb + (((NOUT + o) * NT) << 10), a);
    acc[o] = mfma_split<NT>(a, s1, acc[o]);
#endif
  }
  if constexpr (HASB) {
#pragma unroll
    for (int o = 0; o < NOUT; ++o) acc[o] = x3_finish<NT>(acc[o], us, bias_acc(bias + o * 32, hh));
  }
  char* const t = p.cur;
  p.cur = p.nxt;
  p.nxt = t;
  p.g += 1;
}


__device__ __forceinline__ floatx16 mfma_term2(const halfx8 (&a)[2], const halfx8 (&b)[2], int j, floatx16 acc) {
  if (j == 0) return __builtin_amdgcn_mfma_f32_32x32x16_f16(a[1], b[0], acc, 0, 0, 0);
  if (j == 1) return __builtin_amdgcn_mfma_f32_32x32x16_f16(a[0], b[1], acc, 0, 0, 0);
  return __builtin_amdgcn_mfma_f32_32x32x16_f16(a[0], b[0], acc, 0, 0, 0);
}

template <int T, int NOUT, int Q, int m>
__device__ __forceinline__ void x3_valu_slot(floatx16 (&hb)[T], halfx8 (&cs)[2], halfx8 (&s1)[2], float (&tq)[4],
                                             uint32_t (&s1h)[4], uint32_t (&csh)[4], float c) {
  constexpr int kCs = 3 * NOUT > 12 ? 3 * NOUT : 12;
  if constexpr (m == 0) split8h_hi<1>(hb[Q], s1h);
  if constexpr (m == 1) split8h_lo<1>(hb[Q], s1h, s1[0], s1[1]);
  if constexpr (Q + 1 < T) {
    constexpr int i0 = m - 1, i1 = m - 2, i2 = m - 3, i3 = m - 4;
    if constexpr (i3 >= 0 && i3 < 16) {
      hb[Q + 1][i3] = hb[Q + 1][i3] * tq[i3 & 3];
      asm volatile("" ::"v"(hb[Q + 1][i3]));
    }
    if constexpr (i2 >= 0 && i2 < 16) tq[i2 & 3] = __builtin_amdgcn_rcpf(tq[i2 & 3]);
    if constexpr (i1 >= 0 && i1 < 16) tq[i1 & 3] = __builtin_fmaf(tq[i1 & 3], c, c);
    if constexpr (i0 >= 0 && i0 < 16) tq[i0 & 3] = __builtin_amdgcn_exp2f(-hb[Q + 1][i0]);
    if constexpr (m == kCs) split8h_hi<0>(hb[Q + 1], csh);
    if constexpr (m == kCs + 1) split8h_lo<0>(hb[Q + 1], csh, cs[0], cs[1]);
  }
}

template <int T, int NOUT, int Q, int m>
__device__ __forceinline__ void x3_slot(const char* lb, floatx16 (&hb)[T], floatx16 (&acc)[NOUT],
                                        halfx8 (&fr)[2][2], halfx8 (&cs)[2], halfx8 (&s1)[2], float (&tq)[4],
                                        uint32_t (&s1h)[4], uint32_t (&csh)[4], float c) {
  constexpr int t = m / 3, j = m % 3, ks = t / NOUT, o = t % NOUT;
  if constexpr (j == 0 && t + 1 < 2 * NOUT) load_frag<2>(lb + (((t + 1) * 2) << 10), fr[(t + 1) & 1]);
  if constexpr (ks == 0) acc[o] = mfma_term2(fr[t & 1], cs, j, acc[o]);
  else acc[o] = mfma_term2(fr[t & 1], s1, j, acc[o]);
  x3_valu_slot<T, NOUT, Q, m>(hb, cs, s1, tq, s1h, csh, c);
#if ZF_X3_ABL == 12 || ZF_X3_ABL == 13
  if constexpr (j == 0) {
    float dd;
    if (ZF_X3_ABL == 12) asm volatile("v_add_f32 %0, %1, %2" : "=v"(dd) : "v"(acc[o][0]), "v"(acc[o][1]));
    else asm volatile("v_exp_f32 %0, %1" : "=v"(dd) : "v"(acc[o][0]));
  }
#endif
  __builtin_amdgcn_sched_barrier(0);
}

template <int T, int NOUT, int Q, int... M>
__device__ __forceinline__ void x3_slots_all(std::integer_sequence<int, M...>, const char* lb, floatx16 (&hb)[T],
                                             floatx16 (&acc)[NOUT], halfx8 (&fr)[2][2], halfx8 (&cs)[2],
                                             halfx8 (&s1)[2], float (&tq)[4], uint32_t (&s1h)[4],
                                             uint32_t (&csh)[4], float c) {
  (x3_slot<T, NOUT, Q, M>(lb, hb, acc, fr, cs, s1, tq, s1h, csh, c), ...);
}

template <int T, int NOUT, int Q, int... M>
__device__ __forceinline__ void x3_valu_tail(std::integer_sequence<int, M...>, floatx16 (&hb)[T], halfx8 (&cs)[2],
                                             halfx8 (&s1)[2], float (&tq)[4], uint32_t (&s1h)[4],
                                             uint32_t (&csh)[4], float c) {
  (x3_valu_slot<T, NOUT, Q, 2 * NOUT * 3 + M>(hb, cs, s1, tq, s1h, csh, c), ...);
}

template <int T, int NOUT, int Q, bool HASB>
__device__ __forceinline__ void x3_step_slots(const char* __restrict__ x3, X3Pipe& p, floatx16 (&hb)[T],
                                              floatx16 (&acc)[NOUT], int lane, const float* __restrict__ bias,
                                              int hh, halfx8 (&cs)[2], float isc, float us) {
  constexpr int NT = 2;
#ifdef ZF_X3_TRACE
  const unsigned long long tb0 = X3T_NOW();
#endif
  asm volatile("s_waitcnt vmcnt(0)" ::: "memory");
  __syncthreads();
#ifdef ZF_X3_TRACE
  p.tbar += X3T_NOW() - tb0;
#endif
  x3_issue_next<NT, T>(x3, p, p.nxt, lane);
  const char* lb = p.cur + lane * 16;
  halfx8 fr[2][NT];
  load_frag<NT>(lb, fr[0]);
  halfx8 s1[NT];
  constexpr int kSlots = 2 * NOUT * 3;
  float tq[4];
  uint32_t s1h[4], csh[4];
  x3_slots_all<T, NOUT, Q>(std::make_integer_sequence<int, kSlots>{}, lb, hb, acc, fr, cs, s1, tq, s1h, csh, isc);
  x3_valu_tail<T, NOUT, Q>(std::make_integer_sequence<int, (kSlots < 20 ? 20 - kSlots : 0)>{}, hb, cs, s1, tq,
                           s1h, csh, isc);
  static_assert(kSlots >= 2, "at least one triple per k-step");
  if constexpr (HASB) {
#pragma unroll
    for (int o = 0; o < NOUT; ++o) acc[o] = x3_finish<NT>(acc[o], us, bias_acc(bias + o * 32, hh));
  }
  char* const t = p.cur;
  p.cur = p.nxt;
  p.nxt = t;
  p.g += 1;
}

__device__ __forceinline__ void x3_scale_from(float U, int kw, float& isc, float& us, float& ius) {
  const int e = max(__builtin_amdgcn_frexp_expf(fminf(U, 3.40282347e38f)), -60);
  isc = __builtin_amdgcn_ldexpf(kSwishPrescale, e - 14);
  us = __builtin_amdgcn_ldexpf(1.0f, e - 14 - kw);
  ius = __builtin_amdgcn_ldexpf(1.0f, 14 + kw - e);
}

template <bool CR>
__device__ __forceinline__ float x3_squareplus2_t(float x);

template <int T, int NOUT, bool NEXT, int SPT, int m>
__device__ __forceinline__ void x3_valu_slot_last(floatx16 (&hb)[T], floatx16 (&acc)[NOUT], halfx8 (&cs)[2],
                                                  halfx8 (&s1)[2], float (&tq)[4], uint32_t (&s1h)[4],
                                                  uint32_t (&csh)[4], floatx16& bt, const float* __restrict__ bias,
                                                  int hh, float us, float cn, float& mx) {
  constexpr int Q = T - 1;
  if constexpr (m == 0) split8h_hi<1>(hb[Q], s1h);
  if constexpr (m == 1) split8h_lo<1>(hb[Q], s1h, s1[0], s1[1]);
  constexpr int ob = (m - 4) / 6;
  if constexpr (m >= 4 && (m - 4) % 6 == 0 && ob < NOUT) bt = bias_acc(bias + ob * 32, hh);
  constexpr int of = (m - 7) / 6;
  if constexpr (m >= 7 && of < NOUT && ((m - 7) % 6 == 0 || (m - 7) % 6 == 1)) {
    constexpr int r0 = (m - 7) % 6 == 0 ? 0 : 8;
#pragma unroll
    for (int r = r0; r < r0 + 8; ++r) acc[of][r] = __builtin_fmaf(acc[of][r], us, bt[r]);
  }
#pragma unroll
  for (int o2 = 0; o2 < SPT && o2 < NOUT; ++o2) {
    const int rr = m - 9 - 6 * o2;
    if (rr >= 0 && rr < 8) {
      acc[o2][2 * rr] = x3_squareplus2_t<false>(acc[o2][2 * rr]);
      acc[o2][2 * rr + 1] = x3_squareplus2_t<false>(acc[o2][2 * rr + 1]);
    }
  }
  constexpr int oq = (m - 8) / 6;
  if constexpr (NEXT && m >= 8 && oq < NOUT && ((m - 8) % 6 == 0 || (m - 8) % 6 == 1)) {
    constexpr int r0 = (m - 8) % 6 == 0 ? 0 : 8;
#pragma unroll
    for (int r = r0; r < r0 + 8; r += 2)
      asm("v_max3_f32 %0, %0, |%1|, |%2|" : "+v"(mx) : "v"(acc[oq][r]), "v"(acc[oq][r + 1]));
  }
  if constexpr (NEXT) {
    constexpr int i0 = m - 9, i1 = m - 10, i2 = m - 11, i3 = m - 12;
    if constexpr (i3 >= 0 && i3 < 16) {
      acc[0][i3] = acc[0][i3] * tq[i3 & 3];
      asm volatile("" ::"v"(acc[0][i3]));
    }
    if constexpr (i2 >= 0 && i2 < 16) tq[i2 & 3] = __builtin_amdgcn_rcpf(tq[i2 & 3]);
    if constexpr (i1 >= 0 && i1 < 16) tq[i1 & 3] = __builtin_fmaf(tq[i1 & 3], cn, cn);
    if constexpr (i0 >= 0 && i0 < 16) tq[i0 & 3] = __builtin_amdgcn_exp2f(-acc[0][i0]);
    if constexpr (m == 20) split8h_hi<0>(acc[0], csh);
    if constexpr (m == 21) split8h_lo<0>(acc[0], csh, cs[0], cs[1]);
  }
}

template <int T, int NOUT, bool NEXT, int SPT, int m>
__device__ __forceinline__ void x3_slot_last(const char* lb, floatx16 (&hb)[T], floatx16 (&acc)[NOUT],
                                             halfx8 (&fr)[2][2], halfx8 (&cs)[2], halfx8 (&s1)[2], float (&tq)[4],
                                             uint32_t (&s1h)[4], uint32_t (&csh)[4], floatx16& bt,
                                             const float* __restrict__ bias, int hh, float us, float cn, float& mx) {
  constexpr int t = m / 3, j = m % 3, o = t / 2, ks = t % 2;
  constexpr int tn = t + 1, on = tn / 2, ksn = tn % 2;
  if constexpr (j == 0 && tn < 2 * NOUT) load_frag<2>(lb + (((ksn * NOUT + on) * 2) << 10), fr[tn & 1]);
  if constexpr (ks == 0) acc[o] = mfma_term2(fr[t & 1], cs, j, acc[o]);
  else acc[o] = mfma_term2(fr[t & 1], s1, j, acc[o]);
  x3_valu_slot_last<T, NOUT, NEXT, SPT, m>(hb, acc, cs, s1, tq, s1h, csh, bt, bias, hh, us, cn, mx);
  __builtin_amdgcn_sched_barrier(0);
}

template <int T, int NOUT, bool NEXT, int SPT, int... M>
__device__ __forceinline__ void x3_slots_all_last(std::integer_sequence<int, M...>, const char* lb,
                                                  floatx16 (&hb)[T], floatx16 (&acc)[NOUT], halfx8 (&fr)[2][2],
                                                  halfx8 (&cs)[2], halfx8 (&s1)[2], float (&tq)[4],
                                                  uint32_t (&s1h)[4], uint32_t (&csh)[4], floatx16& bt,
                                                  const float* __restrict__ bias, int hh, float us, float cn,
                                                  float& mx) {
  (x3_slot_last<T, NOUT, NEXT, SPT, M>(lb, hb, acc, fr, cs, s1, tq, s1h, csh, bt, bias, hh, us, cn, mx), ...);
}

template <int T, int NOUT, bool NEXT, int SPT, int... M>
__device__ __forceinline__ void x3_valu_tail_last(std::integer_sequence<int, M...>, floatx16 (&hb)[T],
                                                  floatx16 (&acc)[NOUT], halfx8 (&cs)[2], halfx8 (&s1)[2],
                                                  float (&tq)[4], uint32_t (&s1h)[4], uint32_t (&csh)[4],
                                                  floatx16& bt, const float* __restrict__ bias, int hh, float us,
                                                  float cn, float& mx) {
  (x3_valu_slot_last<T, NOUT, NEXT, SPT, 6 * NOUT + M>(hb, acc, cs, s1, tq, s1h, csh, bt, bias, hh, us, cn, mx),
   ...);
}

template <int T, int NOUT, bool NEXT, int SPT = 0>
__device__ __forceinline__ void x3_step_slots_last(const char* __restrict__ x3, X3Pipe& p, floatx16 (&hb)[T],
                                                   floatx16 (&acc)[NOUT], int lane, const float* __restrict__ bias,
                                                   int hh, halfx8 (&cs)[2], float us, float cn, float& mx) {
  asm volatile("s_waitcnt vmcnt(0)" ::: "memory");
  __syncthreads();
  x3_issue_next<2, T>(x3, p, p.nxt, lane);
  const char* lb = p.cur + lane * 16;
  halfx8 fr[2][2];
  load_frag<2>(lb, fr[0]);
  halfx8 s1[2];
  float tq[4];
  uint32_t s1h[4], csh[4];
  floatx16 bt;
  constexpr int kSlots = 6 * NOUT;
  constexpr int kEnd0 = NEXT ? (6 * NOUT > 28 ? 6 * NOUT : 28) : 6 * (NOUT - 1) + 9;
  constexpr int kEnd = SPT > 0 && 6 * (SPT - 1) + 17 > kEnd0 ? 6 * (SPT - 1) + 17 : kEnd0;
  mx = 0.f;
  x3_slots_all_last<T, NOUT, NEXT, SPT>(std::make_integer_sequence<int, kSlots>{}, lb, hb, acc, fr, cs, s1, tq, s1h,
                                        csh, bt, bias, hh, us, cn, mx);
  x3_valu_tail_last<T, NOUT, NEXT, SPT>(std::make_integer_sequence<int, (kEnd > kSlots ? kEnd - kSlots : 0)>{}, hb,
                                        acc, cs, s1, tq, s1h, csh, bt, bias, hh, us, cn, mx);
  char* const t = p.cur;
  p.cur = p.nxt;
  p.nxt = t;
  p.g += 1;
}

template <int ODD>
__device__ __forceinline__ void mix_hi(uint32_t& h, float v, float r) {
  if constexpr (ODD == 0) asm("v_fma_mixlo_f16 %0, %1, %2, 0" : "=v"(h) : "v"(v), "v"(r));
  else asm("v_fma_mixhi_f16 %0, %1, %2, 0" : "+v"(h) : "v"(v), "v"(r));
}
template <int ODD>
__device__ __forceinline__ void mix_lo(uint32_t& l, float v, float r, uint32_t h) {
  if constexpr (ODD == 0)
    asm("v_fma_mixlo_f16 %0, %1, %2, -%3 op_sel_hi:[0,0,1]" : "=v"(l) : "v"(v), "v"(r), "v"(h));
  else
    asm("v_fma_mixhi_f16 %0, %1, %2, -%3 op_sel:[0,0,1] op_sel_hi:[0,0,1]" : "+v"(l) : "v"(v), "v"(r), "v"(h));
}

template <int T, int NOUT, int Q, int m>
__device__ __forceinline__ void x3_valu_slot_f(floatx16 (&hb)[T], halfx8 (&s1)[2], uint32_t (&s1h)[4],
                                               float (&tq)[5], uint32_t (&nh)[8], uint32_t (&nl)[8], float c) {
  if constexpr (Q == 0 && m == 0) split8h_hi<1>(hb[0], s1h);
  if constexpr (Q == 0 && m == 1) split8h_lo<1>(hb[0], s1h, s1[0], s1[1]);
  if constexpr (Q + 1 < T) {
    constexpr int i0 = m - 1, i1 = m - 2, i2 = m - 3, i3 = m - 4, i4 = m - 5;
    if constexpr (i4 >= 0 && i4 < 16) mix_lo<i4 & 1>(nl[i4 >> 1], hb[Q + 1][i4], tq[i4 % 5], nh[i4 >> 1]);
    if constexpr (i3 >= 0 && i3 < 16) mix_hi<i3 & 1>(nh[i3 >> 1], hb[Q + 1][i3], tq[i3 % 5]);
    if constexpr (i2 >= 0 && i2 < 16) tq[i2 % 5] = __builtin_amdgcn_rcpf(tq[i2 % 5]);
    if constexpr (i1 >= 0 && i1 < 16) tq[i1 % 5] = __builtin_fmaf(tq[i1 % 5], c, c);
    if constexpr (i0 >= 0 && i0 < 16) tq[i0 % 5] = __builtin_amdgcn_exp2f(-hb[Q + 1][i0]);
  }
}

template <int T, int NOUT, int Q, int m>
__device__ __forceinline__ void x3_slot_f(const char* lb, floatx16 (&hb)[T], floatx16 (&acc)[NOUT],
                                          halfx8 (&fr)[2][2], halfx8 (&cs)[2], halfx8 (&s1)[2], uint32_t (&s1h)[4],
                                          float (&tq)[5], uint32_t (&nh)[8], uint32_t (&nl)[8], float c) {
  constexpr int t = m / 3, j = m % 3, ks = t / NOUT, o = t % NOUT;
  if constexpr (j == 0 && t + 1 < 2 * NOUT) load_frag<2>(lb + (((t + 1) * 2) << 10), fr[(t + 1) & 1]);
  if constexpr (ks == 0) acc[o] = mfma_term2(fr[t & 1], cs, j, acc[o]);
  else acc[o] = mfma_term2(fr[t & 1], s1, j, acc[o]);
  x3_valu_slot_f<T, NOUT, Q, m>(hb, s1, s1h, tq, nh, nl, c);
  __builtin_amdgcn_sched_barrier(0);
}

template <int T, int NOUT, int Q, int... M>
__device__ __forceinline__ void x3_slots_all_f(std::integer_sequence<int, M...>, const char* lb, floatx16 (&hb)[T],
                                               floatx16 (&acc)[NOUT], halfx8 (&fr)[2][2], halfx8 (&cs)[2],
                                               halfx8 (&s1)[2], uint32_t (&s1h)[4], float (&tq)[5],
                                               uint32_t (&nh)[8], uint32_t (&nl)[8], float c) {
  (x3_slot_f<T, NOUT, Q, M>(lb, hb, acc, fr, cs, s1, s1h, tq, nh, nl, c), ...);
}

template <int T, int NOUT, int Q, int... M>
__device__ __forceinline__ void x3_valu_tail_f(std::integer_sequence<int, M...>, floatx16 (&hb)[T], halfx8 (&s1)[2],
                                               uint32_t (&s1h)[4], float (&tq)[5], uint32_t (&nh)[8],
                                               uint32_t (&nl)[8], float c) {
  (x3_valu_slot_f<T, NOUT, Q, 2 * NOUT * 3 + M>(hb, s1, s1h, tq, nh, nl, c), ...);
}

template <int T, int NOUT, int Q, bool HASB>
__device__ __forceinline__ void x3_step_slots_f(const char* __restrict__ x3, X3Pipe& p, floatx16 (&hb)[T],
                                                floatx16 (&acc)[NOUT], int lane, const float* __restrict__ bias,
                                                int hh, halfx8 (&cs)[2], halfx8 (&s1)[2], float isc, float us) {
  constexpr int NT = 2;
  asm volatile("s_waitcnt vmcnt(0)" ::: "memory");
  __syncthreads();
  x3_issue_next<NT, T>(x3, p, p.nxt, lane);
  const char* lb = p.cur + lane * 16;
  halfx8 fr[2][NT];
  load_frag<NT>(lb, fr[0]);
  constexpr int kSlots = 2 * NOUT * 3;
  float tq[5];
  uint32_t s1h[4], nh[8], nl[8];
  x3_slots_all_f<T, NOUT, Q>(std::make_integer_sequence<int, kSlots>{}, lb, hb, acc, fr, cs, s1, s1h, tq, nh, nl,
                             isc);
  x3_valu_tail_f<T, NOUT, Q>(std::make_integer_sequence<int, (kSlots < 21 ? 21 - kSlots : 0)>{}, hb, s1, s1h, tq,
                             nh, nl, isc);
  if constexpr (HASB) {
#pragma unroll
    for (int o = 0; o < NOUT; ++o) acc[o] = x3_finish<NT>(acc[o], us, bias_acc(bias + o * 32, hh));
  }
  if constexpr (Q + 1 < T) {
    __builtin_memcpy(&cs[0], &nh[0], 16);
    __builtin_memcpy(&cs[1], &nl[0], 16);
    __builtin_memcpy(&s1[0], &nh[4], 16);
    __builtin_memcpy(&s1[1], &nl[4], 16);
  }
  char* const t = p.cur;
  p.cur = p.nxt;
  p.nxt = t;
  p.g += 1;
}

template <int T, int NOUT, int Q>
__device__ __forceinline__ void x3_step_pre(const char* __restrict__ x3, X3Pipe& p, const halfx8 (&sp)[T][2][2],
                                            floatx16 (&acc)[NOUT], int lane) {
  asm volatile("s_waitcnt vmcnt(0)" ::: "memory");
  __syncthreads();
  x3_issue_next<2, T>(x3, p, p.nxt, lane);
  const char* lb = p.cur + lane * 16;
  halfx8 c[2];
  load_frag<2>(lb, c);
#pragma unroll
  for (int s = 0; s < 2; ++s)
#pragma unroll
    for (int o = 0; o < NOUT; ++o) {
      const int t = s * NOUT + o;
      halfx8 n[2];
      if (t + 1 < 2 * NOUT) load_frag<2>(lb + (((t + 1) * 2) << 10), n);
      acc[o] = mfma_split<2>(c, sp[Q][s], acc[o]);
      if (t + 1 < 2 * NOUT) {
        c[0] = n[0];
        c[1] = n[1];
      }
    }
  char* const tb = p.cur;
  p.cur = p.nxt;
  p.nxt = tb;
  p.g += 1;
}

template <int T, int NOUT, int Q = 0>
__device__ __forceinline__ void x3_layer_pre(const char* __restrict__ x3, X3Pipe& p, const halfx8 (&sp)[T][2][2],
                                             floatx16 (&acc)[NOUT], int lane) {
  x3_step_pre<T, NOUT, Q>(x3, p, sp, acc, lane);
  if constexpr (Q + 1 < T) x3_layer_pre<T, NOUT, Q + 1>(x3, p, sp, acc, lane);
}

template <int NT, int T, int NOUT, bool HASB, bool OACT, int Q = 0, int AS = 0>
__device__ __forceinline__ void x3_layer_pipe(const char* __restrict__ x3, X3Pipe& p, floatx16 (&hb)[T],
                                              floatx16 (&acc)[NOUT], int lane, const float* bias_last, int hh,
                                              typename XT<NT>::E (&cs)[NT], float isc, float us, int act,
                                              halfx8 (&fused_s1)[2]) {
#ifndef ZF_X3_FUSED
#define ZF_X3_FUSED 0
#endif
  if constexpr (NT == 2 && !OACT && ZF_X3_FUSED) {
    static_assert(sizeof(typename XT<NT>::E) == 16, "halfx8 terms");
    halfx8(&s1)[2] = fused_s1;
    if constexpr (Q + 1 < T) {
      x3_step_slots_f<T, NOUT, Q, false>(x3, p, hb, acc, lane, nullptr, hh, cs, s1, isc, us);
      x3_layer_pipe<NT, T, NOUT, HASB, OACT, Q + 1>(x3, p, hb, acc, lane, bias_last, hh, cs, isc, us, act, s1);
    } else {
      x3_step_slots_f<T, NOUT, Q, HASB>(x3, p, hb, acc, lane, bias_last, hh, cs, s1, isc, us);
    }
    return;
  }
  if constexpr (NT == 2 && !OACT) {
    if constexpr (Q + 1 < T) {
      x3_step_slots<T, NOUT, Q, false>(x3, p, hb, acc, lane, nullptr, hh, cs, isc, us);
      x3_layer_pipe<NT, T, NOUT, HASB, OACT, Q + 1>(x3, p, hb, acc, lane, bias_last, hh, cs, isc, us, act,
                                                    fused_s1);
    } else {
      x3_step_slots<T, NOUT, Q, HASB>(x3, p, hb, acc, lane, bias_last, hh, cs, isc, us);
    }
    return;
  }
  if constexpr (Q + 1 < T) {
    x3_step_pipe<NT, T, NOUT, Q, false, OACT, AS>(x3, p, hb, acc, lane, nullptr, hh, cs, isc, us, act);
    x3_layer_pipe<NT, T, NOUT, HASB, OACT, Q + 1, AS>(x3, p, hb, acc, lane, bias_last, hh, cs, isc, us, act,
                                                      fused_s1);
  } else {
    x3_step_pipe<NT, T, NOUT, Q, HASB, OACT, AS>(x3, p, hb, acc, lane, bias_last, hh, cs, isc, us, act);
  }
}

template <int T, int NOUT, bool NEXT, int SPT = 0, int Q = 0>
__device__ __forceinline__ void x3_layer_early(const char* __restrict__ x3, X3Pipe& p, floatx16 (&hb)[T],
                                               floatx16 (&acc)[NOUT], int lane, const float* __restrict__ bias,
                                               int hh, halfx8 (&cs)[2], float c, float us, float cn, float& mx) {
  if constexpr (Q + 1 < T) {
    x3_step_slots<T, NOUT, Q, false>(x3, p, hb, acc, lane, nullptr, hh, cs, c, us);
    x3_layer_early<T, NOUT, NEXT, SPT, Q + 1>(x3, p, hb, acc, lane, bias, hh, cs, c, us, cn, mx);
  } else {
    x3_step_slots_last<T, NOUT, NEXT, SPT>(x3, p, hb, acc, lane, bias, hh, cs, us, cn, mx);
  }
}

template <int NT, int T, int NOUT, bool SW, bool OACT, int Q = 0>
__device__ __forceinline__ void x3_layer(const char* __restrict__ x3, X3Pipe& p, floatx16 (&hb)[T],
                                         floatx16 (&acc)[NOUT], int lane, const float* bias_last, int hh,
                                         float isc, float us, int act) {
  if constexpr (Q + 1 < T) {
    x3_step<NT, T, NOUT, Q, SW, OACT>(x3, p, hb, acc, lane, nullptr, hh, isc, us, act);
    x3_layer<NT, T, NOUT, SW, OACT, Q + 1>(x3, p, hb, acc, lane, bias_last, hh, isc, us, act);
  } else {
    x3_step<NT, T, NOUT, Q, SW, OACT>(x3, p, hb, acc, lane, bias_last, hh, isc, us, act);
  }
}

template <int T, bool OACT>
__device__ __forceinline__ void x3_layer0(const X3Sc& c, const float* par, const float* xs, int rot, int D,
                                          int s, int hh, int lane, floatx16 (&hb)[T], int swish_tiles,
                                          float* umax = nullptr) {
  const int dt = c.dt, dc = c.dc, DC = c.DC, KS0 = c.KS0;
  const int DCp = 2 * KS0;
  const float* bn = par;
  const float* w0b = par + c.w0_rel;
  const float* b0 = par + c.b_rel;
#pragma unroll
  for (int o = 0; o < T; ++o) hb[o] = bias_acc(b0 + o * 32, hh);
  for (int ks = 0; ks < KS0; ++ks) {
    const int k = 2 * ks + hh;
    float v = 0.f;
    if (k < dc) v = xs[wrap(dt + k + rot, D) * 32 + s];
    else if (k < DC) v = xs[(D + k - dc) * 32 + s];
    const float u = (v - bn[k]) * bn[DCp + k] + bn[2 * DCp + k];
    if (umax != nullptr) *umax = fmaxf(*umax, fabsf(u));
    const float* w0 = w0b + ks * 64 + lane;
#pragma unroll
    for (int o = 0; o < T; ++o) hb[o] = __builtin_amdgcn_mfma_f32_32x32x2f32(w0[o * KS0 * 64], u, hb[o], 0, 0, 0);
  }
#pragma unroll
  for (int o = 0; o < T; ++o)
    if (o < swish_tiles) {
      if constexpr (OACT) {
        x3_act_tile<3, true>(hb[o], 1.f, c.act);
      } else {
#pragma unroll
        for (int r = 0; r < 16; ++r) hb[o][r] = swish(hb[o][r]);
      }
    }
}

__device__ __forceinline__ float x3_squareplus(float x) {
  return 0.5f * (x + __builtin_amdgcn_sqrtf(__builtin_fmaf(x, x, 4.0f)));
}

__device__ __forceinline__ float x3_squareplus2(float x) {
  return x + __builtin_amdgcn_sqrtf(__builtin_fmaf(x, x, 4.0f));
}

__device__ __forceinline__ void x3_forward_eval(float x, const RqsBin& b, float& y, float& ld) {
  const float rw = rcp_refined(b.w);
  const float sk = b.h * rw;
  const float zr = (x - b.xk) * rw;
  const float z = (zr != zr) ? zr : fminf(fmaxf(zr, kEps), kOneMinusEps);
  const float az = 1.0f - z;
  const float num = b.h * z * (sk * z + b.dk * az);
  const float den = sk + (b.dkp1 + b.dk - 2.0f * sk) * z * az;
  const float rd = rcp_refined(den + kEps);
  const float yv = b.yk + num * rd;
  y = b.oob ? x : yv;
  const float num2 = z * (b.dkp1 * z + 2.0f * sk * az) + b.dk * (az * az);
  const float sq = (sk + kEps) * rd;
  const float l = __logf((num2 + kEps) * (sq * sq));
  ld = b.oob ? 0.0f : l;
}

__device__ __forceinline__ float x3_sqrt_cr(float a) {
  const float y = __builtin_amdgcn_rsqf(a);
  const float sq = a * y;
  const float r = __builtin_fmaf(__builtin_fmaf(-sq, sq, a), 0.5f * y, sq);
  return a == __builtin_huge_valf() ? a : r;
}
template <bool CR>
__device__ __forceinline__ float x3_squareplus2_t(float x) {
  const float a = __builtin_fmaf(x, x, 4.0f);
  return x + (CR ? x3_sqrt_cr(a) : __builtin_amdgcn_sqrtf(a));
}
template <bool CR>
__device__ __forceinline__ float x3_squareplus_t(float x) {
  const float a = __builtin_fmaf(x, x, 4.0f);
  return 0.5f * (x + (CR ? x3_sqrt_cr(a) : __builtin_amdgcn_sqrtf(a)));
}

template <bool FWD, int N, int MX>
__device__ __forceinline__ void x3_bsel(float v, const float (&X)[MX], const float (&Y)[MX], const float (&Wd)[N],
                                        const float (&Ht)[N], const float (&S)[N + 1], float (&out)[6]) {
  static_assert(MX >= N, "knot arrays cover the bins");
  if constexpr (N == 1) {
    out[0] = X[0]; out[1] = Y[0]; out[2] = Wd[0]; out[3] = Ht[0]; out[4] = S[0]; out[5] = S[1];
  } else {
    constexpr int H = N / 2;
    const bool c = (FWD ? X[H] : Y[H]) <= v;
    float X2[H], Y2[H], W2[H], H2[H], S2[H + 1];
#pragma unroll
    for (int i = 0; i < H; ++i) {
      X2[i] = c ? X[H + i] : X[i];
      Y2[i] = c ? Y[H + i] : Y[i];
      W2[i] = c ? Wd[H + i] : Wd[i];
      H2[i] = c ? Ht[H + i] : Ht[i];
    }
#pragma unroll
    for (int i = 0; i <= H; ++i) S2[i] = c ? S[H + i] : S[i];
    x3_bsel<FWD, H, H>(v, X2, Y2, W2, H2, S2, out);
  }
}

template <int K>
struct KnotLit {
  static constexpr double c64 = 1e-5 / (1.0 - (double)K * 1e-5);
  static constexpr float c = (float)c64;
  static constexpr float norm = (float)(1.0 + c64 * (double)K);
  static constexpr float rnorm = (float)(1.0 / (double)norm);
  static constexpr float bc = c * rnorm;
};

template <bool FWD, int K, bool CR, bool KLIT, int NPV>
__device__ __forceinline__ RqsBin x3_bin(float v, const float (&P)[NPV], const KnotConsts& kc) {
  float ws[K], hs[K];
#pragma unroll
  for (int j = 0; j < K; ++j) {
    ws[j] = x3_squareplus2_t<CR>(P[j]);
    hs[j] = x3_squareplus2_t<CR>(P[K + j]);
  }
  float X[K + 1], Y[K + 1];
  X[0] = 0.f;
  Y[0] = 0.f;
  X[1] = ws[0];
  Y[1] = hs[0];
#pragma unroll
  for (int j = 1; j < K; ++j) {
    X[j + 1] = X[j] + ws[j];
    Y[j + 1] = Y[j] + hs[j];
  }
  const float rn = KLIT ? KnotLit<K>::rnorm : kc.rnorm;
  const float bc = KLIT ? KnotLit<K>::bc : kc.c * kc.rnorm;
  const float ax = rcp_refined(X[K]) * rn, ay = rcp_refined(Y[K]) * rn;
#pragma unroll
  for (int j = 1; j <= K; ++j) {
    const float jb = KLIT ? (float)j * KnotLit<K>::bc : (float)j * bc;
    X[j] = __builtin_fmaf(X[j], ax, jb);
    Y[j] = __builtin_fmaf(Y[j], ay, jb);
  }
  float S[K + 1];
  S[0] = 0.f;
  S[K] = 0.f;
#pragma unroll
  for (int j = 1; j < K; ++j) S[j] = P[2 * K + j - 1];
  float o[6];
  x3_bsel<FWD, K, K + 1>(v, X, Y, ws, hs, S, o);
  RqsBin b;
  const bool sliver = (FWD ? X[K] : Y[K]) <= v;
  b.xk = sliver ? X[K] : o[0];
  b.yk = sliver ? Y[K] : o[1];
  b.w = sliver ? qnan() : __builtin_fmaf(o[2], ax, bc);
  b.h = sliver ? qnan() : __builtin_fmaf(o[3], ay, bc);
  const float lo = sliver ? 0.f : o[4];
  const float hi = sliver ? qnan() : o[5];
  b.dk = lo == 0.f ? 1.f : x3_squareplus_t<CR>(lo);
  b.dkp1 = hi == 0.f ? 1.f : x3_squareplus_t<CR>(hi);
  b.sk = b.h / b.w;
  b.oob = (v < 0.f) || (v >= 1.f);
  return b;
}

template <int T, int K, bool PAIRS>
constexpr int x3_occupancy() { return (T == 8 || K > 32) ? 1 : (PAIRS || K > 16) ? 2 : 3; }

template <int NT, int K, int T, bool PAIRS, bool ONE, bool INV, bool OACT, int ASET = 0>
__global__ __launch_bounds__(kX3Waves * 64, (x3_occupancy<T, K, PAIRS>())) void flow_kernel_x3(
    const DevFlow* __restrict__ F, const float* __restrict__ blob, const char* __restrict__ x3,
    const float* __restrict__ xin, const float* __restrict__ cin, float* __restrict__ y_out,
    const float* __restrict__ ld_in, float* __restrict__ ld_out, float* __restrict__ lp_out,
    double* __restrict__ block_partial, long long nparts, int op_begin, int op_end, long long N,
    unsigned long long seed, int gen) {
  constexpr int TL = ONE ? (3 * K - 1 + 31) / 32 : (3 * K - 1 + 15) / 16;
  constexpr int NPV = ONE ? 32 * TL : 16 * TL;
  constexpr int NW = kX3Waves;
  extern __shared__ __attribute__((aligned(16))) char lds[];
  const int D = F->D;
  const int C = F->C;
  const int wave = __builtin_amdgcn_readfirstlane(threadIdx.x >> 6);
  const int lane = threadIdx.x & 63;
  const int s = lane & 31;
  const int hh = lane >> 5;
  constexpr int kBuf = group_bytes<NT>(T > TL ? T : TL);
  const int PB = F->x3_par_bytes;
  const int DS = D + C;
  char* par_lds = lds + 2 * kBuf;
  float* xs = reinterpret_cast<float*>(par_lds + 2 * PB) + wave * (32 * DS);
  double* s_part = reinterpret_cast<double*>(reinterpret_cast<float*>(par_lds + 2 * PB) + NW * 32 * DS);
  const float* sp = blob;
  const long long row = ((long long)blockIdx.x * NW + wave) * kTile + s;
  const bool valid = row < N;

  X3Pipe pipe;
  pipe.cur = lds;
  pipe.nxt = lds + kBuf;
  pipe.g = 0;
  pipe.wave = wave;
  {
    int first = -1;
    const int nq = op_end - op_begin;
    for (int q = 0; q < nq; ++q) {
      const int oi = INV ? (op_end - 1 - q) : (op_begin + q);
      if (F->ops[oi].kind == ZF_OP_NSC) { first = oi; break; }
    }
    if (first >= 0) {
      const DevOp& fo = F->ops[first];
      x3_dma(x3 + fo.x3, pipe.cur, first_pieces<NT, T>(fo), wave, lane);
      x3_dma(reinterpret_cast<const char*>(blob + fo.bn), par_lds, fo.x3_par_pieces, wave, lane);
    }
  }
  load_state(xs, xin, row, valid, D, s, hh, F, seed, INV ? gen : 0);
  for (int j = hh; j < C; j += 2) xs[(D + j) * 32 + s] = valid ? cin[row * C + j] : 0.f;
  float ld = (ld_in != nullptr && valid) ? ld_in[row] : 0.f;
  int rot = 0;
  wave_lds_sync();
#ifdef ZF_X3_TRACE
  unsigned long long tacc[kX3TraceSlots] = {};
  pipe.tbar = 0;
  pipe.tdma = 0;
  pipe.tgrp = 0;
  const unsigned long long t_begin = X3T_NOW();
  unsigned long long t_last = t_begin;
#define X3T(k)                                   \
  {                                              \
    const unsigned long long t_ = X3T_NOW();     \
    tacc[k] += t_ - t_last;                      \
    t_last = t_;                                 \
  }
#elif defined(ZF_X3_MARK)
#define X3T(k) asm volatile(";ZFMARK " #k)
#else
#define X3T(k)
#endif
#ifdef ZF_X3_MARK
#define X3M(k) asm volatile(";ZFMARK " #k)
#else
#define X3M(k)
#endif
  pipe.par_src = nullptr;
  pipe.par_dst = nullptr;
  pipe.par_pieces = 0;
  {
    asm volatile("s_waitcnt vmcnt(0)" ::: "memory");
    __syncthreads();
  }
  int nsc_i = 0;

  const int nq = op_end - op_begin;
  for (int q = 0; q < nq; ++q) {
    const int oi = INV ? (op_end - 1 - q) : (op_begin + q);
    const DevOp& op = F->ops[oi];
    const X3Sc opc = x3_scalars<INV>(op);
    const int kind = opc.kind;
    if (kind == ZF_OP_ROLL) {
      rot = pmod(INV ? rot + opc.shift : rot - opc.shift, D);
    } else if (kind == ZF_OP_SHIFT_BOUNDS) {
      shift_bounds_op<INV>(sp + opc.sb, xs, s, hh, rot, D, ld);
      X3T(10);
    } else {
      X3T(0);
#ifdef ZF_X3_TRACE
      tacc[9] += 1;
#endif
      {
        const bool has_next = opc.nxt >= op_begin && opc.nxt < op_end;
        pipe.span = make_span<NT, T>(opc, has_next);
        pipe.par_src = has_next ? reinterpret_cast<const char*>(blob + opc.nbn) : nullptr;
        pipe.par_dst = par_lds + ((nsc_i + 1) & 1) * PB;
        pipe.par_pieces = has_next ? opc.npar : 0;
      }
      pipe.g = 0;
      const float* par = reinterpret_cast<const float*>(par_lds + (nsc_i & 1) * PB);
      ++nsc_i;
      const int nh = opc.nh, act = opc.act, dt = opc.dt, kw_last = opc.kw_last;
      const KnotConsts kc(opc.kreal);
      const bool padlast = opc.kreal == K - 1;
#ifdef ZF_X3_MARK
      const bool klit = true;
#else
      const bool klit = opc.kreal == K;
#endif
      const long long b_rel = opc.b_rel + T * 32, blast_rel = opc.blast_rel;
      floatx16 hb[T];
      constexpr bool kLastSW = !PAIRS;
      constexpr bool kPipe = T == 4 && !PAIRS;
#ifndef ZF_X3_EARLY
#define ZF_X3_EARLY 1
#endif
      constexpr bool kEarly = ZF_X3_EARLY && NT == 2 && !OACT && kPipe;
#ifndef ZF_X3_PRESP
#define ZF_X3_PRESP 1
#endif
      constexpr int kPreSP = (!ZF_X3_PRESP || !kEarly) ? 0 : !ONE ? K / 8 : (K == 16 ? 1 : 0);
      float umax = 0.f;
      x3_layer0<T, OACT>(opc, par, xs, rot, D, s, hh, lane, hb, NT == 2 ? 0 : (!OACT && (nh > 1 || kLastSW)) ? 1 : T,
                         kEarly ? &umax : nullptr);
      float eU = 0.f, eisc = 1.f, eus = 1.f, eius = 1.f;
      halfx8 ecs[2];
      if constexpr (kEarly) {
        const X3Halves uq = x3_halves(umax);
        umax = fmaxf(uq.lo, uq.hi);
        eU = __builtin_fmaf(op.x3_rb[0][0], umax, op.x3_rb[0][1]);
        x3_scale_from(eU, nh > 1 ? opc.kw1 : kw_last, eisc, eus, eius);
        x3_act_tile<NT, false>(hb[0], eisc, act);
        split8h<0>(hb[0], ecs[0], ecs[1]);
      }
#ifndef ZF_X3_SEEDSCALED
#define ZF_X3_SEEDSCALED 0
#endif
      constexpr bool kSeedScaled = NT == 2 && (ZF_X3_SEEDSCALED || !kPipe);
#ifndef ZF_X3_WIDE_PIPE
#define ZF_X3_WIDE_PIPE 1
#endif
#ifndef ZF_X3_PAIRS_PIPE
#define ZF_X3_PAIRS_PIPE 1
#endif
      constexpr bool kPipeH = kPipe || (ZF_X3_PAIRS_PIPE && (T == 4 || ZF_X3_WIDE_PIPE) && NT == 2 && !OACT);
#ifndef ZF_X3_ACTIN
#define ZF_X3_ACTIN 1
#endif
      constexpr bool kActIn = ZF_X3_ACTIN && NT == 2 && ASET == 2 && kPipeH;
      constexpr bool kSeedScaledH = NT == 2 && (ZF_X3_SEEDSCALED || !kPipeH);
#if ZF_X3_ABL != 4
      if constexpr (T == 4) __builtin_amdgcn_s_setprio(2);
#endif
      X3T(1);
      if constexpr (kEarly) {
        float eM = eU;
        for (int l = 1; l < nh; ++l) {
          const float nU = __builtin_fmaf(op.x3_rb[l][0], eM, op.x3_rb[l][1]);
          float nisc, nus, nius;
          x3_scale_from(nU, l + 1 < nh ? op.x3_kw[l + 1] : kw_last, nisc, nus, nius);
          floatx16 acc[T];
#pragma unroll
          for (int o = 0; o < T; ++o) acc[o] = floatx16{0};
          float mx;
          x3_layer_early<T, T, true>(x3, pipe, hb, acc, lane, par + b_rel + (l - 1) * (T * 32), hh, ecs, eisc, eus,
                                     nisc, mx);
#pragma unroll
          for (int o = 0; o < T; ++o) hb[o] = acc[o];
          eU = nU; eisc = nisc; eus = nus; eius = nius;
          const X3Halves mq = x3_halves(mx);
          eM = fmaxf(mq.lo, mq.hi);
        }
      } else
      for (int l = 1; l < nh; ++l) {
        floatx16 acc[T];
        float isc = 1.f, us = 1.f, ius = 1.f;
        if constexpr (NT == 2) {
          x3_act_scale<T, OACT>(hb, l == 1 ? opc.kw1 : op.x3_kw[l], isc, us, ius, act);
#pragma unroll
          for (int o = 0; o < (OACT && !kActIn ? T : 1); ++o) x3_act_tile<NT, OACT, ASET>(hb[o], isc, act);
        }
        const float* bl_l = par + b_rel + (l - 1) * (T * 32);
#pragma unroll
        for (int o = 0; o < T; ++o)
          acc[o] = NT == 3 ? bias_acc(bl_l + o * 32, hh)
                           : (kSeedScaledH ? bias_acc(bl_l + o * 32, hh) * ius : floatx16{0});
        const float* bh = (NT == 2 && !kSeedScaledH) ? bl_l : nullptr;
        if constexpr (kPipeH) {
          typename XT<NT>::E cs[NT];
          splitk<NT, 0>(hb[0], cs);
          halfx8 fs1[2];
          x3_layer_pipe<NT, T, T, NT == 2 && !kSeedScaledH, OACT, 0, kActIn ? ASET : 0>(x3, pipe, hb, acc, lane, bh, hh,
                                                                                     cs, isc, us,
                                                                 act, fs1);
        } else {
          x3_layer<NT, T, T, true, OACT>(x3, pipe, hb, acc, lane, bh, hh, isc, us, act);
        }
        if constexpr (kSeedScaledH) {
#pragma unroll
          for (int o = 0; o < T; ++o) acc[o] *= us;
        }
        const int nsw = NT == 2 ? 0 : (!OACT && (l + 1 < nh || kLastSW)) ? 1 : T;
#pragma unroll
        for (int o = 0; o < T; ++o) {
          if (o < nsw) {
            if constexpr (OACT) {
              hb[o] = acc[o];
              x3_act_tile<3, true>(hb[o], 1.f, act);
            } else {
#pragma unroll
              for (int r = 0; r < 16; ++r) hb[o][r] = swish(acc[o][r]);
            }
          } else {
            hb[o] = acc[o];
          }
        }
      }
      X3T(2);
      float ldn = 0.f;
      const int npair = PAIRS ? (dt + 1) / 2 : 1;
      float lisc = 1.f, lus = 1.f, lius = 1.f;
      if constexpr (kEarly) {
        lisc = eisc; lus = eus; lius = eius;
      } else if constexpr (NT == 2) {
        x3_act_scale<T, OACT>(hb, kw_last, lisc, lus, lius, act);
#pragma unroll
        for (int o = 0; o < T; ++o)
          if (o == 0 || !kLastSW || (OACT && !(kActIn && kPipe))) x3_act_tile<NT, OACT, ASET>(hb[o], lisc, act);
      }
#ifndef ZF_X3_PRESPLIT
#define ZF_X3_PRESPLIT 1
#endif
      constexpr bool kPre = ZF_X3_PRESPLIT && PAIRS && T == 4 && NT == 2 && !OACT;
      halfx8 sp[kPre ? T : 1][2][2];
      if constexpr (kPre) {
#pragma unroll
        for (int q = 0; q < T; ++q) {
          split8h<0>(hb[q], sp[q][0][0], sp[q][0][1]);
          split8h<1>(hb[q], sp[q][1][0], sp[q][1][1]);
        }
      }
      for (int pr = 0; pr < npair; ++pr) {
        const float* bl = par + blast_rel + pr * TL * 32;
        floatx16 pa[TL];
        constexpr bool kSeed = PAIRS && NT == 3;
#pragma unroll
        for (int o = 0; o < TL; ++o)
          pa[o] = kSeed ? bias_acc(bl + o * 32, hh) : (kSeedScaled ? bias_acc(bl + o * 32, hh) * lius : floatx16{0});
        X3T(3);
        if constexpr (kEarly) {
          float mx;
          x3_layer_early<T, TL, false, kPreSP>(x3, pipe, hb, pa, lane, bl, hh, ecs, lisc, lus, 0.f, mx);
        } else if constexpr (kPre) {
          x3_layer_pre<T, TL>(x3, pipe, sp, pa, lane);
        } else if constexpr (kPipe) {
          typename XT<NT>::E cs[NT];
          splitk<NT, 0>(hb[0], cs);
          halfx8 fs1[2];
          x3_layer_pipe<NT, T, TL, !kSeedScaled, OACT, 0, kActIn ? ASET : 0>(x3, pipe, hb, pa, lane, bl, hh, cs, lisc,
                                                                             lus, act, fs1);
        } else {
          x3_layer<NT, T, TL, kLastSW, OACT>(x3, pipe, hb, pa, lane, (kSeed || kSeedScaled) ? nullptr : bl, hh,
                                             lisc, lus, act);
        }
        if constexpr (kSeedScaled) {
#pragma unroll
          for (int o = 0; o < TL; ++o) pa[o] *= lus;
        }
        if constexpr (T == 4) __builtin_amdgcn_s_setprio(0);
        X3T(4);
        constexpr bool kSplitWH = ONE && K == 16;
        float P[NPV];
#pragma unroll
        for (int o = 0; o < TL; ++o)
#pragma unroll
          for (int r = 0; r < 16; ++r) {
            if constexpr (kSplitWH) {
              if (o == 0) P[r] = pa[0][r];
              else
                P[2 * K + r] = x3_halves(pa[1][r]).lo;
            } else if constexpr (ONE) {
              const X3Halves q = x3_halves(pa[o][r]);
              P[32 * o + r] = q.lo;
              P[32 * o + 16 + r] = q.hi;
            } else {
              P[16 * o + r] = pa[o][r];
            }
          }
        X3M(11);
#if ZF_X3_ABL == 10 || ZF_X3_ABL == 11
#pragma unroll
        for (int q2 = 0; q2 < 64; ++q2) {
          float dd;
          if (ZF_X3_ABL == 10) asm volatile("v_add_f32 %0, %1, %2" : "=v"(dd) : "v"(pa[0][q2 & 15]), "v"(pa[1][q2 & 15]));
          else asm volatile("v_exp_f32 %0, %1" : "=v"(dd) : "v"(pa[0][q2 & 15]));
        }
#endif
        const int d = 2 * pr + hh;
        const bool dact = d < dt;
        float ldv = 0.f;
        {
          float* xp = xs + wrap((dact ? d : 0) + rot, D) * 32 + s;
          const float xv = *xp;
#ifndef ZF_X3_BSEARCH
#define ZF_X3_BSEARCH 0
#endif
          RqsBin bin;
          bool binned = false;
          if constexpr (ZF_X3_BSEARCH && !kSplitWH && !kPreSP && (K == 8 || K == 16 || K == 32 || K == 64)) {
            if (klit) {
              bin = x3_bin<!INV, K, OACT, true>(xv, P, kc);
              binned = true;
            }
          }
          if (!binned) {
            float w[K], hg[K];
            const float bc = kc.c * kc.rnorm;
            if constexpr (kSplitWH) {
              float sw = 0.f;
#pragma unroll
              for (int j = 0; j < K; ++j) {
                w[j] = kPreSP ? P[j] : x3_squareplus2_t<OACT>(P[j]);
                sw = sw + w[j];
              }
              const float a = rcp_refined(sw) * kc.rnorm;
#pragma unroll
              for (int j = 0; j < K; ++j) {
                const X3Halves q = x3_halves(__builtin_fmaf(w[j], a, bc));
                w[j] = q.lo;
                hg[j] = q.hi;
              }
            } else {
              float sx = 0.f, sy = 0.f;
#pragma unroll
              for (int j = 0; j < K; ++j) {
                w[j] = kPreSP ? P[j] : x3_squareplus2_t<OACT>(P[j]);
                hg[j] = kPreSP ? P[K + j] : x3_squareplus2_t<OACT>(P[K + j]);
                sx = sx + w[j];
                sy = sy + hg[j];
              }
              const float ax = rcp_refined(sx) * kc.rnorm, ay = rcp_refined(sy) * kc.rnorm;
#pragma unroll
              for (int j = 0; j < K; ++j) {
                w[j] = __builtin_fmaf(w[j], ax, bc);
                hg[j] = __builtin_fmaf(hg[j], ay, bc);
              }
            }
            X3M(12);
            float sl[K - 1];
#pragma unroll
            for (int j = 0; j < K - 1; ++j) sl[j] = P[2 * K + j];
#ifndef ZF_X3_EXECBIN
#define ZF_X3_EXECBIN 1
#endif
            const auto spf = [](float v) { return v == 0.f ? 1.f : x3_squareplus_t<OACT>(v); };
            if constexpr (ZF_X3_EXECBIN && K % 8 == 0) bin = rqs_bin_exec<!INV, K>(xv, w, hg, sl, spf, padlast);
            else bin = rqs_bin_monotone<!INV, K>(xv, w, hg, sl, spf, padlast);
            X3M(13);
          }
          float yv;
          if (!INV) {
            float l;
            x3_forward_eval(xv, bin, yv, l);
            ldv = dact ? l : 0.f;
          } else {
            yv = rqs_inverse_eval(xv, bin);
          }
          if (dact) *xp = yv;
        }
        wave_lds_sync();
        if (!INV) {
          const X3Halves q = x3_halves(ldv);
          ldn = ldn + q.lo;
          if (2 * pr + 1 < dt) ldn = ldn + q.hi;
        }
      }
      if (!INV) ld = ld + ldn;
      X3T(5);
    }
  }

  flow_epilogue<NW>(F, xs, s, hh, lane, wave, rot, D, row, valid, ld, lp_out, block_partial, NW / 4, nparts, y_out,
                    ld_out, s_part);
#ifdef ZF_X3_TRACE
  X3T(6);
  tacc[7] = pipe.tbar;
  tacc[11] = pipe.tdma;
  tacc[12] = pipe.tgrp;
  tacc[8] = t_last - t_begin;
  if (lane == 0 && x3_trace_buf != nullptr) {
    unsigned long long* o = x3_trace_buf + ((long long)blockIdx.x * NW + wave) * kX3TraceSlots;
#pragma unroll
    for (int k = 0; k < kX3TraceSlots; ++k) o[k] = tacc[k];
  }
#endif
#undef X3T
#undef X3M
}

template <int NT, int K, int T, bool PAIRS, bool ONE, bool OACT, int ASET = 0>
int launch_x3(const X3Launch& a, bool inverse) {
  const long long rows = kX3Waves * kTile;
  const long long grid = (a.N + rows - 1) / rows;
  if (grid > 0x7fffffffLL) return einval("N too large");
  constexpr int TL = ONE ? (3 * K - 1 + 31) / 32 : (3 * K - 1 + 15) / 16;
  size_t lds = (size_t)2 * group_bytes<NT>(T > TL ? T : TL) + (size_t)2 * a.par_bytes +
               (size_t)kX3Waves * 32 * (a.D + a.C) * 4 + kX3Waves * sizeof(double);
#ifdef ZF_X3_TRACE
  if (const char* pad = std::getenv("ZF_X3_LDS_PAD")) lds += (size_t)std::atoi(pad) * 1024;
#endif
  if (lds > 160 * 1024) return enotsup("bf16x3 LDS footprint too large");
  if (inverse)
    hipLaunchKernelGGL((flow_kernel_x3<NT, K, T, PAIRS, ONE, true, OACT, ASET>), dim3((unsigned)grid), dim3(kX3Waves * 64), lds, a.stream,
                       a.desc, a.blob, (const char*)a.x3, a.x, a.c, a.y, a.ld_in, a.ld_out, a.lp, a.part,
                       a.nparts, a.op_begin, a.op_end, a.N, a.seed, a.gen);
  else
    hipLaunchKernelGGL((flow_kernel_x3<NT, K, T, PAIRS, ONE, false, OACT, ASET>), dim3((unsigned)grid), dim3(kX3Waves * 64), lds, a.stream,
                       a.desc, a.blob, (const char*)a.x3, a.x, a.c, a.y, a.ld_in, a.ld_out, a.lp, a.part,
                       a.nparts, a.op_begin, a.op_end, a.N, a.seed, a.gen);
  ZF_CHECK_LAUNCH("flow_kernel_x3");
  return ZF_OK;
}

template <int NT, int K, bool OACT = false, int ASET = 0>
int launch_x3_k(const X3Launch& a, bool inverse) {
  const int dt = a.D / 2;
  const bool one = dt == 1;
  if (a.T == 4) {
    if (dt > 2) return launch_x3<NT, K, 4, true, false, OACT, ASET>(a, inverse);
    return one ? launch_x3<NT, K, 4, false, true, OACT, ASET>(a, inverse)
               : launch_x3<NT, K, 4, false, false, OACT, ASET>(a, inverse);
  }
  if (a.T == 8)
    return one ? launch_x3<NT, K, 8, true, true, OACT, ASET>(a, inverse)
               : launch_x3<NT, K, 8, true, false, OACT, ASET>(a, inverse);
  return enotsup("split-MFMA kernel: hidden tiles not instantiated");
}

}
}
```

Baseline: 1.338 billion.

## Add resident-weights persistent x3 kernel for K16 two-dim-pair flows

Adds a persistent kernel variant that launches one block per CU and keeps all split-MFMA weight groups resident in LDS, instead of streaming them through a double buffer with a barrier per group. Each block loops over many row slots, and per-row state is staged in a device scratch buffer sized from N. The goal is to remove the repeated global-to-LDS weight DMA and the per-step syncthreads. In exchange it adds a large LDS footprint, a hipMalloc on first use, and reduced occupancy. It is enabled automatically for K=16, NT=2, T=4, dt=2 flows with N of at least 2^19, or when forced through an environment variable.

```diff
diff --git a/zenflow_amd/build.py b/zenflow_amd/build.py
--- a/zenflow_amd/build.py
+++ b/zenflow_amd/build.py
@@ -15,7 +15,7 @@
 ARCH = os.environ.get("ZF_OFFLOAD_ARCH", "gfx950")
 HIPCC = os.environ.get("HIPCC", "/opt/rocm/bin/hipcc")
 
-SOURCES = ["zf_runtime.hip", "zf_rqs.hip", "zf_flow.hip", "zf_flow_x3.hip", "zf_flow_x3_k8.hip", "zf_flow_x3_k16.hip", "zf_flow_x3_k32.hip", "zf_flow_x3_k64.hip", "zf_flow_x3_k64_act.hip", "zf_flow_x3_k8_act.hip", "zf_flow_x3_k16_act.hip", "zf_flow_x3_k32_act.hip", "zf_flow_x3_k8_act2.hip", "zf_flow_x3_k16_act2.hip", "zf_flow_x3_k32_act2.hip", "zf_stats.hip", "zf_rccl.hip", "zf_train.hip", "zf_layered.hip"]
+SOURCES = ["zf_runtime.hip", "zf_rqs.hip", "zf_flow.hip", "zf_flow_x3.hip", "zf_flow_x3_k8.hip", "zf_flow_x3_k16.hip", "zf_flow_x3_k16_res.hip", "zf_flow_x3_k32.hip", "zf_flow_x3_k64.hip", "zf_flow_x3_k64_act.hip", "zf_flow_x3_k8_act.hip", "zf_flow_x3_k16_act.hip", "zf_flow_x3_k32_act.hip", "zf_flow_x3_k8_act2.hip", "zf_flow_x3_k16_act2.hip", "zf_flow_x3_k32_act2.hip", "zf_stats.hip", "zf_rccl.hip", "zf_train.hip", "zf_layered.hip"]
 HEADERS = sorted(p.name for p in CSRC.glob("*.h"))
 
 FLAGS = [
diff --git a/zenflow_amd/csrc/zf_flow.hip b/zenflow_amd/csrc/zf_flow.hip
--- a/zenflow_amd/csrc/zf_flow.hip
+++ b/zenflow_amd/csrc/zf_flow.hip
@@ -340,6 +340,10 @@
   bool x3_oact = false;
   int x3_aset = 0;
   int device = 0;
+  int x3_res_mode = -1;
+  int ncu = 0;
+  float* d_res_state = nullptr;
+  long long res_floats = 0;
   zf::LayeredFlow* lay = nullptr;
 };
 
@@ -443,6 +447,7 @@
   if (layered) F.HP = 32;
   int x3K = 0;
   const bool x3 = !layered && zf::x3_eligible(desc, F.HP < 128 ? 128 : F.HP, &x3K);
+  h->x3_res_mode = zf::x3_resident_mode();
   if (x3 && F.HP < 128) F.HP = 128;
   const int HP = F.HP, T = HP / 32;
   {
@@ -586,6 +591,8 @@
   const bool use_x3 = F.x3_ok != 0;
   int rcd = ZF_OK;
   hipError_t e = hipGetDevice(&h->device);
+  if (e == hipSuccess && use_x3)
+    (void)hipDeviceGetAttribute(&h->ncu, hipDeviceAttributeMultiprocessorCount, h->device);
   if (e == hipSuccess && layered) {
     rcd = zf::layered_create(desc, nat, need, &h->lay);
     if (rcd) {
@@ -615,6 +622,7 @@
   if (h->d_desc) (void)hipFree(h->d_desc);
   if (h->d_blob) (void)hipFree(h->d_blob);
   if (h->d_x3) (void)hipFree(h->d_x3);
+  if (h->d_res_state) (void)hipFree(h->d_res_state);
   zf::layered_destroy(h->lay);
   delete h;
   return ZF_OK;
@@ -635,6 +643,8 @@
 
 namespace zf {
 namespace {
+
+constexpr int64_t kX3ResidentAutoRows = 1 << 19;
 
 template <bool INV>
 int launch_flow(zf_flow* h, int op_begin, int op_end, const float* x, const float* c, float* y,
@@ -662,6 +672,21 @@
     a.seed = seed;
     a.gen = gen;
     a.stream = (hipStream_t)stream;
+    if (h->x3_res_mode != 0 && (h->x3_res_mode == 1 || N >= kX3ResidentAutoRows) &&
+        x3_resident_fits(h->desc, a, INV, h->ncu)) {
+      const long long need = ((long long)(N + kTile - 1) / kTile) * kTile * (h->host.D + 1);
+      if (need > h->res_floats) {
+        hipStreamCaptureStatus cs = hipStreamCaptureStatusNone;
+        if (hipStreamIsCapturing(a.stream, &cs) == hipSuccess && cs == hipStreamCaptureStatusNone) {
+          if (h->d_res_state) (void)hipFree(h->d_res_state);
+          h->d_res_state = nullptr;
+          h->res_floats = 0;
+          ZF_TRY_HIP(hipMalloc(&h->d_res_state, (size_t)need * sizeof(float)));
+          h->res_floats = need;
+        }
+      }
+      if (need <= h->res_floats) a.res_state = h->d_res_state;
+    }
     return launch_flow_x3(a, INV);
   }
   const int64_t grid = (N + kBlockRows - 1) / kBlockRows;
diff --git a/zenflow_amd/csrc/zf_flow_dev.h b/zenflow_amd/csrc/zf_flow_dev.h
--- a/zenflow_amd/csrc/zf_flow_dev.h
+++ b/zenflow_amd/csrc/zf_flow_dev.h
@@ -238,6 +238,32 @@
   return lp;
 }
 
+__device__ __forceinline__ double flow_lp_rows(const DevFlow* __restrict__ F, const float* xs, int s, int hh,
+                                               int rot, int D, long long row, bool valid, float ld,
+                                               float* __restrict__ lp_out, bool want_sum) {
+  float lat = 0.f;
+  for (int j = 0; j < D; ++j)
+    lat = lat + latent_logpdf(F->latent, F->lat_c0, F->lat_c1, F->lat_c2, xs[wrap(j + rot, D) * 32 + s]);
+  const float lp = nan_to_num_lp(lat + ld);
+  if (valid && hh == 0) lp_out[row] = lp;
+  double v = 0.0;
+  if (want_sum) {
+    v = (valid && hh == 0) ? (double)lp : 0.0;
+#pragma unroll
+    for (int m = 32; m >= 1; m >>= 1) v += __shfl_xor(v, m);
+  }
+  return v;
+}
+
+__device__ __forceinline__ void flow_out_rows(const float* xs, int s, int hh, int rot, int D, long long row,
+                                              bool valid, float ld, float* __restrict__ y_out,
+                                              float* __restrict__ ld_out) {
+  if (y_out != nullptr && valid) {
+    for (int j = hh; j < D; j += 2) y_out[row * D + j] = xs[wrap(j + rot, D) * 32 + s];
+  }
+  if (ld_out != nullptr && valid && hh == 0) ld_out[row] = ld;
+}
+
 template <int NW>
 __device__ __forceinline__ void flow_epilogue(const DevFlow* __restrict__ F, const float* xs, int s,
                                               int hh, int lane, int wave, int rot, int D, long long row,
@@ -247,15 +273,8 @@
                                               float* __restrict__ ld_out, double* s_part,
                                               long long slot = -1) {
   if (lp_out != nullptr) {
-    float lat = 0.f;
-    for (int j = 0; j < D; ++j)
-      lat = lat + latent_logpdf(F->latent, F->lat_c0, F->lat_c1, F->lat_c2, xs[wrap(j + rot, D) * 32 + s]);
-    const float lp = nan_to_num_lp(lat + ld);
-    if (valid && hh == 0) lp_out[row] = lp;
+    const double v = flow_lp_rows(F, xs, s, hh, rot, D, row, valid, ld, lp_out, block_partial != nullptr);
     if (block_partial != nullptr) {
-      double v = (valid && hh == 0) ? (double)lp : 0.0;
-#pragma unroll
-      for (int m = 32; m >= 1; m >>= 1) v += __shfl_xor(v, m);
       if (lane == 0) s_part[wave] = v;
       __syncthreads();
       if (threadIdx.x == 0) {
@@ -268,10 +287,7 @@
       }
     }
   }
-  if (y_out != nullptr && valid) {
-    for (int j = hh; j < D; j += 2) y_out[row * D + j] = xs[wrap(j + rot, D) * 32 + s];
-  }
-  if (ld_out != nullptr && valid && hh == 0) ld_out[row] = ld;
+  flow_out_rows(xs, s, hh, rot, D, row, valid, ld, y_out, ld_out);
 }
 
 struct X3Launch {
@@ -293,9 +309,13 @@
   bool oact;
   int aset;
   int par_bytes;
+  float* res_state = nullptr;
+  int res_blocks = 0, res_slots = 0, res_span = 0;
   hipStream_t stream;
 };
 int launch_flow_x3(const X3Launch& a, bool inverse);
+int x3_resident_mode();
+bool x3_resident_fits(const zf_flow_desc& desc, X3Launch& a, bool inverse, int ncu);
 bool x3_eligible(const zf_flow_desc& desc, int HP, int* K);
 struct LayeredFlow;
 int layered_create(const zf_flow_desc& desc, const float* natural, int64_t n, LayeredFlow** out);
diff --git a/zenflow_amd/csrc/zf_flow_x3.hip b/zenflow_amd/csrc/zf_flow_x3.hip
--- a/zenflow_amd/csrc/zf_flow_x3.hip
+++ b/zenflow_amd/csrc/zf_flow_x3.hip
@@ -35,6 +35,9 @@
 int x3_padded_knots(int K);
 int x3_param_of(int jp, int Kp, int K, float* fill);
 
+int x3_last_tiles(int K) { return (3 * K - 1 + 15) / 16; }
+int x3_last_tiles_one(int K) { return (3 * K - 1 + 31) / 32; }
+
 bool x3_eligible(const zf_flow_desc& desc, int HP, int* K_out) {
   const char* env = std::getenv("ZF_DISABLE_X3");
   if (env && env[0] == '1') return false;
@@ -50,6 +53,37 @@
   const int Kp = x3_padded_knots(K);
   if (HP > 256 || desc.dim > 64 || Kp == 0) return false;
   *K_out = Kp;
+  return true;
+}
+
+int x3_resident_mode() {
+  const char* env = std::getenv("ZF_X3_RESIDENT");
+  if (env && env[0] == '0' && env[1] == 0) return 0;
+  if (env && env[0] == '1' && env[1] == 0) return 1;
+  return -1;
+}
+
+bool x3_resident_fits(const zf_flow_desc& desc, X3Launch& a, bool inverse, int ncu) {
+  if (a.NT != 2 || a.T != 4 || a.oact || ncu <= 0 || a.N <= 0) return false;
+  const int dt = desc.dim / 2;
+  if (dt > 2) return false;
+  bool in_range = false;
+  for (int i = 0; i < desc.n_ops; ++i) {
+    if (desc.ops[i].kind != ZF_OP_NSC) continue;
+    if (desc.ops[i].n_hidden != 2) return false;
+    if (i >= a.op_begin && i < a.op_end) in_range = true;
+  }
+  if (!in_range) return false;
+  const int TL = dt == 1 ? x3_last_tiles_one(a.K) : x3_last_tiles(a.K);
+  const long long span = 4ll * (2 * 4 * 2 * 1024) + 4ll * (2 * TL * 2 * 1024);
+  const long long nslots = (a.N + 127) / 128;
+  const long long slots = (nslots + ncu - 1) / ncu;
+  if (slots > (1 << 20)) return false;
+  if (x3_res_lds_bytes((size_t)span, a.par_bytes, a.D + a.C, 4 * slots) > 160 * 1024) return false;
+  if (a.K != 16 || dt != 2) return false;
+  a.res_blocks = ncu;
+  a.res_slots = (int)slots;
+  a.res_span = (int)span;
   return true;
 }
 
@@ -87,8 +121,6 @@
   return x3_scheme() == 3 ? 3 : 2;
 }
 
-int x3_last_tiles(int K) { return (3 * K - 1 + 15) / 16; }
-int x3_last_tiles_one(int K) { return (3 * K - 1 + 31) / 32; }
 
 int x3_pairs(const zf_flow_desc& desc) { return (desc.dim / 2 + 1) / 2; }
 
diff --git a/zenflow_amd/csrc/zf_flow_x3_k16.hip b/zenflow_amd/csrc/zf_flow_x3_k16.hip
--- a/zenflow_amd/csrc/zf_flow_x3_k16.hip
+++ b/zenflow_amd/csrc/zf_flow_x3_k16.hip
@@ -3,9 +3,11 @@
 namespace zf {
 
 int launch_x3_k16_act(const X3Launch& a, bool inverse);
+int launch_x3r_k16(const X3Launch& a, bool inverse);
 
 int launch_x3_k16(const X3Launch& a, bool inverse) {
   if (a.oact) return launch_x3_k16_act(a, inverse);
+  if (a.res_state != nullptr) return launch_x3r_k16(a, inverse);
   return a.NT == 2 ? launch_x3_k<2, 16>(a, inverse) : launch_x3_k<3, 16>(a, inverse);
 }
 
diff --git a/zenflow_amd/csrc/zf_flow_x3_k16_res.hip b/zenflow_amd/csrc/zf_flow_x3_k16_res.hip
--- /dev/null
+++ b/zenflow_amd/csrc/zf_flow_x3_k16_res.hip
@@ -0,0 +1,7 @@
+#include "zf_flow_x3_kernel.h"
+
+namespace zf {
+
+int launch_x3r_k16(const X3Launch& a, bool inverse) { return launch_x3r<16, false>(a, inverse); }
+
+}
diff --git a/zenflow_amd/csrc/zf_flow_x3_kernel.h b/zenflow_amd/csrc/zf_flow_x3_kernel.h
--- a/zenflow_amd/csrc/zf_flow_x3_kernel.h
+++ b/zenflow_amd/csrc/zf_flow_x3_kernel.h
@@ -396,11 +396,12 @@
   return sp;
 }
 
-__device__ __forceinline__ void x3_dma(const char* __restrict__ src, char* dst, int pieces, int wave, int lane) {
+__device__ __forceinline__ void x3_dma(const char* __restrict__ src, char* dst, int pieces, int wave, int lane,
+                                       int nw = kX3Waves) {
 #if ZF_X3_ABL == 5
   pieces = (pieces + 3) / 4;
 #endif
-  for (int p = wave; p < pieces; p += kX3Waves)
+  for (int p = wave; p < pieces; p += nw)
     __builtin_amdgcn_global_load_lds((const void*)(src + (p << 10) + lane * 16),
                                      (__attribute__((address_space(3))) void*)(dst + (p << 10)), 16, 0, 0);
 }
@@ -443,6 +444,18 @@
     pieces = p.span.next_pieces;
   }
   x3_dma(x3 + off, dst, pieces, p.wave, lane);
+}
+
+template <bool RES, int BYTES>
+__device__ __forceinline__ void x3_advance(X3Pipe& p) {
+  if constexpr (RES) {
+    p.cur += BYTES;
+  } else {
+    char* const t = p.cur;
+    p.cur = p.nxt;
+    p.nxt = t;
+  }
+  p.g += 1;
 }
 
 template <int NT, int T, int NOUT, int Q, bool SW, bool OACT>
@@ -623,20 +636,22 @@
   (x3_valu_slot<T, NOUT, Q, 2 * NOUT * 3 + M>(hb, cs, s1, tq, s1h, csh, c), ...);
 }
 
-template <int T, int NOUT, int Q, bool HASB>
+template <int T, int NOUT, int Q, bool HASB, bool RES = false>
 __device__ __forceinline__ void x3_step_slots(const char* __restrict__ x3, X3Pipe& p, floatx16 (&hb)[T],
                                               floatx16 (&acc)[NOUT], int lane, const float* __restrict__ bias,
                                               int hh, halfx8 (&cs)[2], float isc, float us) {
   constexpr int NT = 2;
+  if constexpr (!RES) {
 #ifdef ZF_X3_TRACE
-  const unsigned long long tb0 = X3T_NOW();
-#endif
-  asm volatile("s_waitcnt vmcnt(0)" ::: "memory");
-  __syncthreads();
+    const unsigned long long tb0 = X3T_NOW();
+#endif
+    asm volatile("s_waitcnt vmcnt(0)" ::: "memory");
+    __syncthreads();
 #ifdef ZF_X3_TRACE
-  p.tbar += X3T_NOW() - tb0;
-#endif
-  x3_issue_next<NT, T>(x3, p, p.nxt, lane);
+    p.tbar += X3T_NOW() - tb0;
+#endif
+    x3_issue_next<NT, T>(x3, p, p.nxt, lane);
+  }
   const char* lb = p.cur + lane * 16;
   halfx8 fr[2][NT];
   load_frag<NT>(lb, fr[0]);
@@ -652,10 +667,7 @@
 #pragma unroll
     for (int o = 0; o < NOUT; ++o) acc[o] = x3_finish<NT>(acc[o], us, bias_acc(bias + o * 32, hh));
   }
-  char* const t = p.cur;
-  p.cur = p.nxt;
-  p.nxt = t;
-  p.g += 1;
+  x3_advance<RES, group_bytes<NT>(NOUT)>(p);
 }
 
 __device__ __forceinline__ void x3_scale_from(float U, int kw, float& isc, float& us, float& ius) {
@@ -747,13 +759,15 @@
    ...);
 }
 
-template <int T, int NOUT, bool NEXT, int SPT = 0>
+template <int T, int NOUT, bool NEXT, int SPT = 0, bool RES = false>
 __device__ __forceinline__ void x3_step_slots_last(const char* __restrict__ x3, X3Pipe& p, floatx16 (&hb)[T],
                                                    floatx16 (&acc)[NOUT], int lane, const float* __restrict__ bias,
                                                    int hh, halfx8 (&cs)[2], float us, float cn, float& mx) {
-  asm volatile("s_waitcnt vmcnt(0)" ::: "memory");
-  __syncthreads();
-  x3_issue_next<2, T>(x3, p, p.nxt, lane);
+  if constexpr (!RES) {
+    asm volatile("s_waitcnt vmcnt(0)" ::: "memory");
+    __syncthreads();
+    x3_issue_next<2, T>(x3, p, p.nxt, lane);
+  }
   const char* lb = p.cur + lane * 16;
   halfx8 fr[2][2];
   load_frag<2>(lb, fr[0]);
@@ -769,10 +783,7 @@
                                         csh, bt, bias, hh, us, cn, mx);
   x3_valu_tail_last<T, NOUT, NEXT, SPT>(std::make_integer_sequence<int, (kEnd > kSlots ? kEnd - kSlots : 0)>{}, hb,
                                         acc, cs, s1, tq, s1h, csh, bt, bias, hh, us, cn, mx);
-  char* const t = p.cur;
-  p.cur = p.nxt;
-  p.nxt = t;
-  p.g += 1;
+  x3_advance<RES, group_bytes<2>(NOUT)>(p);
 }
 
 template <int ODD>
@@ -937,15 +948,15 @@
   }
 }
 
-template <int T, int NOUT, bool NEXT, int SPT = 0, int Q = 0>
+template <int T, int NOUT, bool NEXT, int SPT = 0, int Q = 0, bool RES = false>
 __device__ __forceinline__ void x3_layer_early(const char* __restrict__ x3, X3Pipe& p, floatx16 (&hb)[T],
                                                floatx16 (&acc)[NOUT], int lane, const float* __restrict__ bias,
                                                int hh, halfx8 (&cs)[2], float c, float us, float cn, float& mx) {
   if constexpr (Q + 1 < T) {
-    x3_step_slots<T, NOUT, Q, false>(x3, p, hb, acc, lane, nullptr, hh, cs, c, us);
-    x3_layer_early<T, NOUT, NEXT, SPT, Q + 1>(x3, p, hb, acc, lane, bias, hh, cs, c, us, cn, mx);
+    x3_step_slots<T, NOUT, Q, false, RES>(x3, p, hb, acc, lane, nullptr, hh, cs, c, us);
+    x3_layer_early<T, NOUT, NEXT, SPT, Q + 1, RES>(x3, p, hb, acc, lane, bias, hh, cs, c, us, cn, mx);
   } else {
-    x3_step_slots_last<T, NOUT, NEXT, SPT>(x3, p, hb, acc, lane, bias, hh, cs, us, cn, mx);
+    x3_step_slots_last<T, NOUT, NEXT, SPT, RES>(x3, p, hb, acc, lane, bias, hh, cs, us, cn, mx);
   }
 }
 
@@ -1121,6 +1132,492 @@
 template <int T, int K, bool PAIRS>
 constexpr int x3_occupancy() { return (T == 8 || K > 32) ? 1 : (PAIRS || K > 16) ? 2 : 3; }
 
+#ifdef ZF_X3_TRACE
+struct X3Tr {
+  unsigned long long tacc[kX3TraceSlots];
+  unsigned long long t_last;
+};
+#define X3T(k)                                   \
+  {                                              \
+    const unsigned long long t_ = X3T_NOW();     \
+    tr.tacc[k] += t_ - tr.t_last;                \
+    tr.t_last = t_;                              \
+  }
+#elif defined(ZF_X3_MARK)
+struct X3Tr {};
+#define X3T(k) asm volatile(";ZFMARK " #k)
+#else
+struct X3Tr {};
+#define X3T(k)
+#endif
+#ifdef ZF_X3_MARK
+#define X3M(k) asm volatile(";ZFMARK " #k)
+#else
+#define X3M(k)
+#endif
+
+template <int NT, int K, int T, bool PAIRS, bool ONE, bool INV, bool OACT, int ASET, bool RES>
+__device__ __forceinline__ void x3_nsc(const DevOp& op, const X3Sc& opc, const char* __restrict__ x3, X3Pipe& pipe,
+                                       const float* par, float* xs, int rot, int D, int s, int hh, int lane,
+                                       float& ld, X3Tr& tr) {
+  constexpr int TL = ONE ? (3 * K - 1 + 31) / 32 : (3 * K - 1 + 15) / 16;
+  constexpr int NPV = ONE ? 32 * TL : 16 * TL;
+  const int nh = opc.nh, act = opc.act, dt = opc.dt, kw_last = opc.kw_last;
+  const KnotConsts kc(opc.kreal);
+  const bool padlast = opc.kreal == K - 1;
+#ifdef ZF_X3_MARK
+  const bool klit = true;
+#else
+  const bool klit = opc.kreal == K;
+#endif
+  const long long b_rel = opc.b_rel + T * 32, blast_rel = opc.blast_rel;
+  floatx16 hb[T];
+  constexpr bool kLastSW = !PAIRS;
+  constexpr bool kPipe = T == 4 && !PAIRS;
+#ifndef ZF_X3_EARLY
+#define ZF_X3_EARLY 1
+#endif
+  constexpr bool kEarly = ZF_X3_EARLY && NT == 2 && !OACT && kPipe;
+  static_assert(!RES || kEarly, "the resident form runs the early-scale slot schedule only");
+#ifndef ZF_X3_PRESP
+#define ZF_X3_PRESP 1
+#endif
+  constexpr int kPreSP = (!ZF_X3_PRESP || !kEarly) ? 0 : !ONE ? K / 8 : (K == 16 ? 1 : 0);
+  float umax = 0.f;
+  x3_layer0<T, OACT>(opc, par, xs, rot, D, s, hh, lane, hb, NT == 2 ? 0 : (!OACT && (nh > 1 || kLastSW)) ? 1 : T,
+                     kEarly ? &umax : nullptr);
+  float eU = 0.f, eisc = 1.f, eus = 1.f, eius = 1.f;
+  halfx8 ecs[2];
+  if constexpr (kEarly) {
+    const X3Halves uq = x3_halves(umax);
+    umax = fmaxf(uq.lo, uq.hi);
+    eU = __builtin_fmaf(op.x3_rb[0][0], umax, op.x3_rb[0][1]);
+    x3_scale_from(eU, nh > 1 ? opc.kw1 : kw_last, eisc, eus, eius);
+    x3_act_tile<NT, false>(hb[0], eisc, act);
+    split8h<0>(hb[0], ecs[0], ecs[1]);
+  }
+#ifndef ZF_X3_SEEDSCALED
+#define ZF_X3_SEEDSCALED 0
+#endif
+  constexpr bool kSeedScaled = NT == 2 && (ZF_X3_SEEDSCALED || !kPipe);
+#ifndef ZF_X3_WIDE_PIPE
+#define ZF_X3_WIDE_PIPE 1
+#endif
+#ifndef ZF_X3_PAIRS_PIPE
+#define ZF_X3_PAIRS_PIPE 1
+#endif
+  constexpr bool kPipeH = kPipe || (ZF_X3_PAIRS_PIPE && (T == 4 || ZF_X3_WIDE_PIPE) && NT == 2 && !OACT);
+#ifndef ZF_X3_ACTIN
+#define ZF_X3_ACTIN 1
+#endif
+  constexpr bool kActIn = ZF_X3_ACTIN && NT == 2 && ASET == 2 && kPipeH;
+  constexpr bool kSeedScaledH = NT == 2 && (ZF_X3_SEEDSCALED || !kPipeH);
+#if ZF_X3_ABL != 4
+  if constexpr (T == 4) __builtin_amdgcn_s_setprio(2);
+#endif
+  X3T(1);
+  if constexpr (kEarly) {
+    float eM = eU;
+    for (int l = 1; l < nh; ++l) {
+      const float nU = __builtin_fmaf(op.x3_rb[l][0], eM, op.x3_rb[l][1]);
+      float nisc, nus, nius;
+      x3_scale_from(nU, l + 1 < nh ? op.x3_kw[l + 1] : kw_last, nisc, nus, nius);
+      floatx16 acc[T];
+#pragma unroll
+      for (int o = 0; o < T; ++o) acc[o] = floatx16{0};
+      float mx;
+      x3_layer_early<T, T, true, 0, 0, RES>(x3, pipe, hb, acc, lane, par + b_rel + (l - 1) * (T * 32), hh, ecs, eisc, eus,
+                                 nisc, mx);
+#pragma unroll
+      for (int o = 0; o < T; ++o) hb[o] = acc[o];
+      eU = nU; eisc = nisc; eus = nus; eius = nius;
+      const X3Halves mq = x3_halves(mx);
+      eM = fmaxf(mq.lo, mq.hi);
+    }
+  } else
+  for (int l = 1; l < nh; ++l) {
+    floatx16 acc[T];
+    float isc = 1.f, us = 1.f, ius = 1.f;
+    if constexpr (NT == 2) {
+      x3_act_scale<T, OACT>(hb, l == 1 ? opc.kw1 : op.x3_kw[l], isc, us, ius, act);
+#pragma unroll
+      for (int o = 0; o < (OACT && !kActIn ? T : 1); ++o) x3_act_tile<NT, OACT, ASET>(hb[o], isc, act);
+    }
+    const float* bl_l = par + b_rel + (l - 1) * (T * 32);
+#pragma unroll
+    for (int o = 0; o < T; ++o)
+      acc[o] = NT == 3 ? bias_acc(bl_l + o * 32, hh)
+                       : (kSeedScaledH ? bias_acc(bl_l + o * 32, hh) * ius : floatx16{0});
+    const float* bh = (NT == 2 && !kSeedScaledH) ? bl_l : nullptr;
+    if constexpr (kPipeH) {
+      typename XT<NT>::E cs[NT];
+      splitk<NT, 0>(hb[0], cs);
+      halfx8 fs1[2];
+      x3_layer_pipe<NT, T, T, NT == 2 && !kSeedScaledH, OACT, 0, kActIn ? ASET : 0>(x3, pipe, hb, acc, lane, bh, hh,
+                                                                                 cs, isc, us,
+                                                             act, fs1);
+    } else {
+      x3_layer<NT, T, T, true, OACT>(x3, pipe, hb, acc, lane, bh, hh, isc, us, act);
+    }
+    if constexpr (kSeedScaledH) {
+#pragma unroll
+      for (int o = 0; o < T; ++o) acc[o] *= us;
+    }
+    const int nsw = NT == 2 ? 0 : (!OACT && (l + 1 < nh || kLastSW)) ? 1 : T;
+#pragma unroll
+    for (int o = 0; o < T; ++o) {
+      if (o < nsw) {
+        if constexpr (OACT) {
+          hb[o] = acc[o];
+          x3_act_tile<3, true>(hb[o], 1.f, act);
+        } else {
+#pragma unroll
+          for (int r = 0; r < 16; ++r) hb[o][r] = swish(acc[o][r]);
+        }
+      } else {
+        hb[o] = acc[o];
+      }
+    }
+  }
+  X3T(2);
+  float ldn = 0.f;
+  const int npair = PAIRS ? (dt + 1) / 2 : 1;
+  float lisc = 1.f, lus = 1.f, lius = 1.f;
+  if constexpr (kEarly) {
+    lisc = eisc; lus = eus; lius = eius;
+  } else if constexpr (NT == 2) {
+    x3_act_scale<T, OACT>(hb, kw_last, lisc, lus, lius, act);
+#pragma unroll
+    for (int o = 0; o < T; ++o)
+      if (o == 0 || !kLastSW || (OACT && !(kActIn && kPipe))) x3_act_tile<NT, OACT, ASET>(hb[o], lisc, act);
+  }
+#ifndef ZF_X3_PRESPLIT
+#define ZF_X3_PRESPLIT 1
+#endif
+  constexpr bool kPre = ZF_X3_PRESPLIT && PAIRS && T == 4 && NT == 2 && !OACT;
+  halfx8 sp[kPre ? T : 1][2][2];
+  if constexpr (kPre) {
+#pragma unroll
+    for (int q = 0; q < T; ++q) {
+      split8h<0>(hb[q], sp[q][0][0], sp[q][0][1]);
+      split8h<1>(hb[q], sp[q][1][0], sp[q][1][1]);
+    }
+  }
+  for (int pr = 0; pr < npair; ++pr) {
+    const float* bl = par + blast_rel + pr * TL * 32;
+    floatx16 pa[TL];
+    constexpr bool kSeed = PAIRS && NT == 3;
+#pragma unroll
+    for (int o = 0; o < TL; ++o)
+      pa[o] = kSeed ? bias_acc(bl + o * 32, hh) : (kSeedScaled ? bias_acc(bl + o * 32, hh) * lius : floatx16{0});
+    X3T(3);
+    if constexpr (kEarly) {
+      float mx;
+      x3_layer_early<T, TL, false, kPreSP, 0, RES>(x3, pipe, hb, pa, lane, bl, hh, ecs, lisc, lus, 0.f, mx);
+    } else if constexpr (kPre) {
+      x3_layer_pre<T, TL>(x3, pipe, sp, pa, lane);
+    } else if constexpr (kPipe) {
+      typename XT<NT>::E cs[NT];
+      splitk<NT, 0>(hb[0], cs);
+      halfx8 fs1[2];
+      x3_layer_pipe<NT, T, TL, !kSeedScaled, OACT, 0, kActIn ? ASET : 0>(x3, pipe, hb, pa, lane, bl, hh, cs, lisc,
+                                                                         lus, act, fs1);
+    } else {
+      x3_layer<NT, T, TL, kLastSW, OACT>(x3, pipe, hb, pa, lane, (kSeed || kSeedScaled) ? nullptr : bl, hh,
+                                         lisc, lus, act);
+    }
+    if constexpr (kSeedScaled) {
+#pragma unroll
+      for (int o = 0; o < TL; ++o) pa[o] *= lus;
+    }
+    if constexpr (T == 4) __builtin_amdgcn_s_setprio(0);
+    X3T(4);
+    constexpr bool kSplitWH = ONE && K == 16;
+    float P[NPV];
+#pragma unroll
+    for (int o = 0; o < TL; ++o)
+#pragma unroll
+      for (int r = 0; r < 16; ++r) {
+        if constexpr (kSplitWH) {
+          if (o == 0) P[r] = pa[0][r];
+          else
+            P[2 * K + r] = x3_halves(pa[1][r]).lo;
+        } else if constexpr (ONE) {
+          const X3Halves q = x3_halves(pa[o][r]);
+          P[32 * o + r] = q.lo;
+          P[32 * o + 16 + r] = q.hi;
+        } else {
+          P[16 * o + r] = pa[o][r];
+        }
+      }
+    X3M(11);
+#if ZF_X3_ABL == 10 || ZF_X3_ABL == 11
+#pragma unroll
+    for (int q2 = 0; q2 < 64; ++q2) {
+      float dd;
+      if (ZF_X3_ABL == 10) asm volatile("v_add_f32 %0, %1, %2" : "=v"(dd) : "v"(pa[0][q2 & 15]), "v"(pa[1][q2 & 15]));
+      else asm volatile("v_exp_f32 %0, %1" : "=v"(dd) : "v"(pa[0][q2 & 15]));
+    }
+#endif
+    const int d = 2 * pr + hh;
+    const bool dact = d < dt;
+    float ldv = 0.f;
+    {
+      float* xp = xs + wrap((dact ? d : 0) + rot, D) * 32 + s;
+      const float xv = *xp;
+#ifndef ZF_X3_BSEARCH
+#define ZF_X3_BSEARCH 0
+#endif
+      RqsBin bin;
+      bool binned = false;
+      if constexpr (ZF_X3_BSEARCH && !kSplitWH && !kPreSP && (K == 8 || K == 16 || K == 32 || K == 64)) {
+        if (klit) {
+          bin = x3_bin<!INV, K, OACT, true>(xv, P, kc);
+          binned = true;
+        }
+      }
+      if (!binned) {
+        float w[K], hg[K];
+        const float bc = kc.c * kc.rnorm;
+        if constexpr (kSplitWH) {
+          float sw = 0.f;
+#pragma unroll
+          for (int j = 0; j < K; ++j) {
+            w[j] = kPreSP ? P[j] : x3_squareplus2_t<OACT>(P[j]);
+            sw = sw + w[j];
+          }
+          const float a = rcp_refined(sw) * kc.rnorm;
+#pragma unroll
+          for (int j = 0; j < K; ++j) {
+            const X3Halves q = x3_halves(__builtin_fmaf(w[j], a, bc));
+            w[j] = q.lo;
+            hg[j] = q.hi;
+          }
+        } else {
+          float sx = 0.f, sy = 0.f;
+#pragma unroll
+          for (int j = 0; j < K; ++j) {
+            w[j] = kPreSP ? P[j] : x3_squareplus2_t<OACT>(P[j]);
+            hg[j] = kPreSP ? P[K + j] : x3_squareplus2_t<OACT>(P[K + j]);
+            sx = sx + w[j];
+            sy = sy + hg[j];
+          }
+          const float ax = rcp_refined(sx) * kc.rnorm, ay = rcp_refined(sy) * kc.rnorm;
+#pragma unroll
+          for (int j = 0; j < K; ++j) {
+            w[j] = __builtin_fmaf(w[j], ax, bc);
+            hg[j] = __builtin_fmaf(hg[j], ay, bc);
+          }
+        }
+        X3M(12);
+        float sl[K - 1];
+#pragma unroll
+        for (int j = 0; j < K - 1; ++j) sl[j] = P[2 * K + j];
+#ifndef ZF_X3_EXECBIN
+#define ZF_X3_EXECBIN 1
+#endif
+        const auto spf = [](float v) { return v == 0.f ? 1.f : x3_squareplus_t<OACT>(v); };
+        if constexpr (ZF_X3_EXECBIN && K % 8 == 0) bin = rqs_bin_exec<!INV, K>(xv, w, hg, sl, spf, padlast);
+        else bin = rqs_bin_monotone<!INV, K>(xv, w, hg, sl, spf, padlast);
+        X3M(13);
+      }
+      float yv;
+      if (!INV) {
+        float l;
+        x3_forward_eval(xv, bin, yv, l);
+        ldv = dact ? l : 0.f;
+      } else {
+        yv = rqs_inverse_eval(xv, bin);
+      }
+      if (dact) *xp = yv;
+    }
+    wave_lds_sync();
+    if (!INV) {
+      const X3Halves q = x3_halves(ldv);
+      ldn = ldn + q.lo;
+      if (2 * pr + 1 < dt) ldn = ldn + q.hi;
+    }
+  }
+  if (!INV) ld = ld + ldn;
+  X3T(5);
+}
+
+constexpr int kX3ResWaves = 12;
+
+inline size_t x3_res_lds_bytes(size_t span, int par_bytes, int DS, long long tiles_per_block) {
+  return span + (size_t)par_bytes + (size_t)kX3ResWaves * 2 * (DS + 1) * 32 * 4 + (size_t)tiles_per_block * 8;
+}
+
+__device__ __forceinline__ void x3r_fetch(const float* __restrict__ st, float* buf, int D, int DS, int lane) {
+#pragma nounroll
+  for (int j = 0; j < D; j += 2)
+    if (j + (lane >> 5) < D)
+      __builtin_amdgcn_global_load_lds((const void*)(st + j * 32 + lane),
+                                       (__attribute__((address_space(3))) void*)(buf + j * 32), 4, 0, 0);
+  if (lane < 32)
+    __builtin_amdgcn_global_load_lds((const void*)(st + D * 32 + lane),
+                                     (__attribute__((address_space(3))) void*)(buf + DS * 32), 4, 0, 0);
+}
+
+template <int K, bool ONE, bool INV>
+__global__ __launch_bounds__(kX3ResWaves * 64, 1) void flow_kernel_x3r(
+    const DevFlow* __restrict__ F, const float* __restrict__ blob, const char* __restrict__ x3,
+    const float* __restrict__ xin, const float* __restrict__ cin, float* __restrict__ y_out,
+    const float* __restrict__ ld_in, float* __restrict__ ld_out, float* __restrict__ lp_out,
+    double* __restrict__ block_partial, int op_begin, int op_end, long long N, unsigned long long seed, int gen,
+    float* __restrict__ state, int slots_per_block, int span_bytes) {
+  constexpr int NT = 2, T = 4, NW = kX3ResWaves;
+  extern __shared__ __attribute__((aligned(16))) char lds[];
+  const int D = F->D;
+  const int C = F->C;
+  const int wave = __builtin_amdgcn_readfirstlane(threadIdx.x >> 6);
+  const int lane = threadIdx.x & 63;
+  const int s = lane & 31;
+  const int hh = lane >> 5;
+  const int PB = F->x3_par_bytes;
+  const int DS = D + C;
+  const int SB = (DS + 1) * 32;
+  const int ST = (D + 1) * 32;
+  char* par_lds = lds + span_bytes;
+  float* xs0 = reinterpret_cast<float*>(par_lds + PB) + wave * (2 * SB);
+  double* s_part = reinterpret_cast<double*>(reinterpret_cast<float*>(par_lds + PB) + NW * 2 * SB);
+  const long long slot0 = (long long)blockIdx.x * slots_per_block;
+  const long long tile0 = slot0 * 4;
+  const long long left = (N + kTile - 1) / kTile - tile0;
+  const int nt = left <= 0 ? 0 : (left < 4ll * slots_per_block ? (int)left : 4 * slots_per_block);
+  for (int i = threadIdx.x; i < 4 * slots_per_block; i += NW * 64) s_part[i] = 0.0;
+
+  X3Pipe pipe;
+  pipe.nxt = nullptr;
+  pipe.wave = wave;
+  pipe.par_src = nullptr;
+  pipe.par_dst = nullptr;
+  pipe.par_pieces = 0;
+  X3Tr tr = {};
+  const int nq = op_end - op_begin;
+  int rot0 = 0;
+  bool first = true;
+  for (int q = 0; q < nq;) {
+    int nsc = -1, seg_end = nq;
+    for (int r = q; r < nq; ++r)
+      if (F->ops[INV ? (op_end - 1 - r) : (op_begin + r)].kind == ZF_OP_NSC) {
+        if (nsc < 0) {
+          nsc = r;
+        } else {
+          seg_end = nsc + 1;
+          break;
+        }
+      }
+    const bool last = seg_end == nq;
+    __syncthreads();
+    if (nsc >= 0 && nt > 0) {
+      const DevOp& fo = F->ops[INV ? (op_end - 1 - nsc) : (op_begin + nsc)];
+      const int pieces = (T * (fo.n_hidden - 1) * group_bytes<NT>(T) + T * group_bytes<NT>(fo.x3_tlast)) >> 10;
+      x3_dma(x3 + fo.x3, lds, pieces, wave, lane, NW);
+      x3_dma(reinterpret_cast<const char*>(blob + fo.bn), par_lds, fo.x3_par_pieces, wave, lane, NW);
+    }
+    asm volatile("s_waitcnt vmcnt(0)" ::: "memory");
+    __syncthreads();
+
+    int cur = 0;
+    if (!first && wave < nt) x3r_fetch(state + (tile0 + wave) * ST, xs0, D, DS, lane);
+    for (int t = wave; t < nt; t += NW) {
+      float* xs = xs0 + cur * SB;
+      const long long tile = tile0 + t;
+      int ln = lane;
+      asm volatile("" : "+v"(ln));
+      {
+        const int s1 = ln & 31, h1 = ln >> 5;
+        const long long row1 = tile * kTile + s1;
+        const bool valid1 = row1 < N;
+        if (first) {
+          load_state(xs, xin, row1, valid1, D, s1, h1, F, seed, INV ? gen : 0);
+        } else if (t == wave) {
+          asm volatile("s_waitcnt vmcnt(0)" ::: "memory");
+        }
+#pragma nounroll
+        for (int j = h1; j < C; j += 2) xs[(D + j) * 32 + s1] = valid1 ? cin[row1 * C + j] : 0.f;
+      }
+      wave_lds_sync();
+      float ld;
+      if (first) {
+        const long long row1 = tile * kTile + (ln & 31);
+        ld = (ld_in != nullptr && row1 < N) ? ld_in[row1] : 0.f;
+      } else {
+        ld = xs[DS * 32 + (ln & 31)];
+        if (t + NW < nt) x3r_fetch(state + (tile + NW) * ST, xs0 + (cur ^ 1) * SB, D, DS, ln);
+      }
+      int rot = rot0;
+      for (int r = q; r < seg_end; ++r) {
+        const DevOp& op = F->ops[INV ? (op_end - 1 - r) : (op_begin + r)];
+        const X3Sc opc = x3_scalars<INV>(op);
+        if (opc.kind == ZF_OP_ROLL) {
+          rot = pmod(INV ? rot + opc.shift : rot - opc.shift, D);
+        } else if (opc.kind == ZF_OP_SHIFT_BOUNDS) {
+          shift_bounds_op<INV>(blob + opc.sb, xs, s, hh, rot, D, ld);
+        } else {
+          int zoff = 0;
+          asm volatile("" : "+s"(zoff));
+          pipe.cur = lds + zoff;
+          pipe.g = 0;
+          x3_nsc<NT, K, T, false, ONE, INV, false, 0, true>(
+              op, opc, x3, pipe, reinterpret_cast<const float*>(par_lds + zoff), xs, rot, D, s, hh, lane, ld, tr);
+        }
+      }
+      asm volatile("s_waitcnt vmcnt(0)" ::: "memory");
+      asm volatile("" : "+v"(ln));
+      const int s2 = ln & 31, h2 = ln >> 5;
+      const long long row = tile * kTile + s2;
+      const bool valid = row < N;
+      if (!last) {
+        float* st = state + tile * ST;
+#pragma nounroll
+        for (int d = h2; d < D; d += 2) st[d * 32 + s2] = xs[d * 32 + s2];
+        if (h2 == 0) st[D * 32 + s2] = ld;
+      } else {
+        if (lp_out != nullptr) {
+          const double v = flow_lp_rows(F, xs, s2, h2, rot, D, row, valid, ld, lp_out, block_partial != nullptr);
+          if (block_partial != nullptr && ln == 0) s_part[t] = v;
+        }
+        flow_out_rows(xs, s2, h2, rot, D, row, valid, ld, y_out, ld_out);
+      }
+      wave_lds_sync();
+      cur ^= 1;
+    }
+    for (int r = q; r < seg_end; ++r) {
+      const DevOp& op = F->ops[INV ? (op_end - 1 - r) : (op_begin + r)];
+      if (op.kind == ZF_OP_ROLL) rot0 = pmod(INV ? rot0 + op.shift : rot0 - op.shift, D);
+    }
+    q = seg_end;
+    first = false;
+  }
+  __syncthreads();
+  if (lp_out != nullptr && block_partial != nullptr) {
+    const int ns = (nt + 3) / 4;
+    for (int i = threadIdx.x; i < ns; i += NW * 64) {
+      double acc = 0.0;
+      for (int w = 0; w < 4; ++w) acc += s_part[4 * i + w];
+      block_partial[slot0 + i] = acc;
+    }
+  }
+}
+
+template <int K, bool ONE>
+int launch_x3r(const X3Launch& a, bool inverse) {
+  const size_t lds = x3_res_lds_bytes((size_t)a.res_span, a.par_bytes, a.D + a.C, 4ll * a.res_slots);
+  if (lds > 160 * 1024 || a.res_state == nullptr) return enotsup("resident split-MFMA kernel: shape");
+  if (inverse)
+    hipLaunchKernelGGL((flow_kernel_x3r<K, ONE, true>), dim3((unsigned)a.res_blocks), dim3(kX3ResWaves * 64), lds,
+                       a.stream, a.desc, a.blob, (const char*)a.x3, a.x, a.c, a.y, a.ld_in, a.ld_out, a.lp, a.part,
+                       a.op_begin, a.op_end, a.N, a.seed, a.gen, a.res_state, a.res_slots, a.res_span);
+  else
+    hipLaunchKernelGGL((flow_kernel_x3r<K, ONE, false>), dim3((unsigned)a.res_blocks), dim3(kX3ResWaves * 64), lds,
+                       a.stream, a.desc, a.blob, (const char*)a.x3, a.x, a.c, a.y, a.ld_in, a.ld_out, a.lp, a.part,
+                       a.op_begin, a.op_end, a.N, a.seed, a.gen, a.res_state, a.res_slots, a.res_span);
+  ZF_CHECK_LAUNCH("flow_kernel_x3r");
+  return ZF_OK;
+}
+
 template <int NT, int K, int T, bool PAIRS, bool ONE, bool INV, bool OACT, int ASET = 0>
 __global__ __launch_bounds__(kX3Waves * 64, (x3_occupancy<T, K, PAIRS>())) void flow_kernel_x3(
     const DevFlow* __restrict__ F, const float* __restrict__ blob, const char* __restrict__ x3,
@@ -1129,7 +1626,6 @@
     double* __restrict__ block_partial, long long nparts, int op_begin, int op_end, long long N,
     unsigned long long seed, int gen) {
   constexpr int TL = ONE ? (3 * K - 1 + 31) / 32 : (3 * K - 1 + 15) / 16;
-  constexpr int NPV = ONE ? 32 * TL : 16 * TL;
   constexpr int NW = kX3Waves;
   extern __shared__ __attribute__((aligned(16))) char lds[];
   const int D = F->D;
@@ -1171,28 +1667,14 @@
   float ld = (ld_in != nullptr && valid) ? ld_in[row] : 0.f;
   int rot = 0;
   wave_lds_sync();
+  X3Tr tr;
 #ifdef ZF_X3_TRACE
-  unsigned long long tacc[kX3TraceSlots] = {};
+  for (int k = 0; k < kX3TraceSlots; ++k) tr.tacc[k] = 0;
   pipe.tbar = 0;
   pipe.tdma = 0;
   pipe.tgrp = 0;
   const unsigned long long t_begin = X3T_NOW();
-  unsigned long long t_last = t_begin;
-#define X3T(k)                                   \
-  {                                              \
-    const unsigned long long t_ = X3T_NOW();     \
-    tacc[k] += t_ - t_last;                      \
-    t_last = t_;                                 \
-  }
-#elif defined(ZF_X3_MARK)
-#define X3T(k) asm volatile(";ZFMARK " #k)
-#else
-#define X3T(k)
-#endif
-#ifdef ZF_X3_MARK
-#define X3M(k) asm volatile(";ZFMARK " #k)
-#else
-#define X3M(k)
+  tr.t_last = t_begin;
 #endif
   pipe.par_src = nullptr;
   pipe.par_dst = nullptr;
@@ -1217,7 +1699,7 @@
     } else {
       X3T(0);
 #ifdef ZF_X3_TRACE
-      tacc[9] += 1;
+      tr.tacc[9] += 1;
 #endif
       {
         const bool has_next = opc.nxt >= op_begin && opc.nxt < op_end;
@@ -1229,283 +1711,8 @@
       pipe.g = 0;
       const float* par = reinterpret_cast<const float*>(par_lds + (nsc_i & 1) * PB);
       ++nsc_i;
-      const int nh = opc.nh, act = opc.act, dt = opc.dt, kw_last = opc.kw_last;
-      const KnotConsts kc(opc.kreal);
-      const bool padlast = opc.kreal == K - 1;
-#ifdef ZF_X3_MARK
-      const bool klit = true;
-#else
-      const bool klit = opc.kreal == K;
-#endif
-      const long long b_rel = opc.b_rel + T * 32, blast_rel = opc.blast_rel;
-      floatx16 hb[T];
-      constexpr bool kLastSW = !PAIRS;
-      constexpr bool kPipe = T == 4 && !PAIRS;
-#ifndef ZF_X3_EARLY
-#define ZF_X3_EARLY 1
-#endif
-      constexpr bool kEarly = ZF_X3_EARLY && NT == 2 && !OACT && kPipe;
-#ifndef ZF_X3_PRESP
-#define ZF_X3_PRESP 1
-#endif
-      constexpr int kPreSP = (!ZF_X3_PRESP || !kEarly) ? 0 : !ONE ? K / 8 : (K == 16 ? 1 : 0);
-      float umax = 0.f;
-      x3_layer0<T, OACT>(opc, par, xs, rot, D, s, hh, lane, hb, NT == 2 ? 0 : (!OACT && (nh > 1 || kLastSW)) ? 1 : T,
-                         kEarly ? &umax : nullptr);
-      float eU = 0.f, eisc = 1.f, eus = 1.f, eius = 1.f;
-      halfx8 ecs[2];
-      if constexpr (kEarly) {
-        const X3Halves uq = x3_halves(umax);
-        umax = fmaxf(uq.lo, uq.hi);
-        eU = __builtin_fmaf(op.x3_rb[0][0], umax, op.x3_rb[0][1]);
-        x3_scale_from(eU, nh > 1 ? opc.kw1 : kw_last, eisc, eus, eius);
-        x3_act_tile<NT, false>(hb[0], eisc, act);
-        split8h<0>(hb[0], ecs[0], ecs[1]);
-      }
-#ifndef ZF_X3_SEEDSCALED
-#define ZF_X3_SEEDSCALED 0
-#endif
-      constexpr bool kSeedScaled = NT == 2 && (ZF_X3_SEEDSCALED || !kPipe);
-#ifndef ZF_X3_WIDE_PIPE
-#define ZF_X3_WIDE_PIPE 1
-#endif
-#ifndef ZF_X3_PAIRS_PIPE
-#define ZF_X3_PAIRS_PIPE 1
-#endif
-      constexpr bool kPipeH = kPipe || (ZF_X3_PAIRS_PIPE && (T == 4 || ZF_X3_WIDE_PIPE) && NT == 2 && !OACT);
-#ifndef ZF_X3_ACTIN
-#define ZF_X3_ACTIN 1
-#endif
-      constexpr bool kActIn = ZF_X3_ACTIN && NT == 2 && ASET == 2 && kPipeH;
-      constexpr bool kSeedScaledH = NT == 2 && (ZF_X3_SEEDSCALED || !kPipeH);
-#if ZF_X3_ABL != 4
-      if constexpr (T == 4) __builtin_amdgcn_s_setprio(2);
-#endif
-      X3T(1);
-      if constexpr (kEarly) {
-        float eM = eU;
-        for (int l = 1; l < nh; ++l) {
-          const float nU = __builtin_fmaf(op.x3_rb[l][0], eM, op.x3_rb[l][1]);
-          float nisc, nus, nius;
-          x3_scale_from(nU, l + 1 < nh ? op.x3_kw[l + 1] : kw_last, nisc, nus, nius);
-          floatx16 acc[T];
-#pragma unroll
-          for (int o = 0; o < T; ++o) acc[o] = floatx16{0};
-          float mx;
-          x3_layer_early<T, T, true>(x3, pipe, hb, acc, lane, par + b_rel + (l - 1) * (T * 32), hh, ecs, eisc, eus,
-                                     nisc, mx);
-#pragma unroll
-          for (int o = 0; o < T; ++o) hb[o] = acc[o];
-          eU = nU; eisc = nisc; eus = nus; eius = nius;
-          const X3Halves mq = x3_halves(mx);
-          eM = fmaxf(mq.lo, mq.hi);
-        }
-      } else
-      for (int l = 1; l < nh; ++l) {
-        floatx16 acc[T];
-        float isc = 1.f, us = 1.f, ius = 1.f;
-        if constexpr (NT == 2) {
-          x3_act_scale<T, OACT>(hb, l == 1 ? opc.kw1 : op.x3_kw[l], isc, us, ius, act);
-#pragma unroll
-          for (int o = 0; o < (OACT && !kActIn ? T : 1); ++o) x3_act_tile<NT, OACT, ASET>(hb[o], isc, act);
-        }
-        const float* bl_l = par + b_rel + (l - 1) * (T * 32);
-#pragma unroll
-        for (int o = 0; o < T; ++o)
-          acc[o] = NT == 3 ? bias_acc(bl_l + o * 32, hh)
-                           : (kSeedScaledH ? bias_acc(bl_l + o * 32, hh) * ius : floatx16{0});
-        const float* bh = (NT == 2 && !kSeedScaledH) ? bl_l : nullptr;
-        if constexpr (kPipeH) {
-          typename XT<NT>::E cs[NT];
-          splitk<NT, 0>(hb[0], cs);
-          halfx8 fs1[2];
-          x3_layer_pipe<NT, T, T, NT == 2 && !kSeedScaledH, OACT, 0, kActIn ? ASET : 0>(x3, pipe, hb, acc, lane, bh, hh,
-                                                                                     cs, isc, us,
-                                                                 act, fs1);
-        } else {
-          x3_layer<NT, T, T, true, OACT>(x3, pipe, hb, acc, lane, bh, hh, isc, us, act);
-        }
-        if constexpr (kSeedScaledH) {
-#pragma unroll
-          for (int o = 0; o < T; ++o) acc[o] *= us;
-        }
-        const int nsw = NT == 2 ? 0 : (!OACT && (l + 1 < nh || kLastSW)) ? 1 : T;
-#pragma unroll
-        for (int o = 0; o < T; ++o) {
-          if (o < nsw) {
-            if constexpr (OACT) {
-              hb[o] = acc[o];
-              x3_act_tile<3, true>(hb[o], 1.f, act);
-            } else {
-#pragma unroll
-              for (int r = 0; r < 16; ++r) hb[o][r] = swish(acc[o][r]);
-            }
-          } else {
-            hb[o] = acc[o];
-          }
-        }
-      }
-      X3T(2);
-      float ldn = 0.f;
-      const int npair = PAIRS ? (dt + 1) / 2 : 1;
-      float lisc = 1.f, lus = 1.f, lius = 1.f;
-      if constexpr (kEarly) {
-        lisc = eisc; lus = eus; lius = eius;
-      } else if constexpr (NT == 2) {
-        x3_act_scale<T, OACT>(hb, kw_last, lisc, lus, lius, act);
-#pragma unroll
-        for (int o = 0; o < T; ++o)
-          if (o == 0 || !kLastSW || (OACT && !(kActIn && kPipe))) x3_act_tile<NT, OACT, ASET>(hb[o], lisc, act);
-      }
-#ifndef ZF_X3_PRESPLIT
-#define ZF_X3_PRESPLIT 1
-#endif
-      constexpr bool kPre = ZF_X3_PRESPLIT && PAIRS && T == 4 && NT == 2 && !OACT;
-      halfx8 sp[kPre ? T : 1][2][2];
-      if constexpr (kPre) {
-#pragma unroll
-        for (int q = 0; q < T; ++q) {
-          split8h<0>(hb[q], sp[q][0][0], sp[q][0][1]);
-          split8h<1>(hb[q], sp[q][1][0], sp[q][1][1]);
-        }
-      }
-      for (int pr = 0; pr < npair; ++pr) {
-        const float* bl = par + blast_rel + pr * TL * 32;
-        floatx16 pa[TL];
-        constexpr bool kSeed = PAIRS && NT == 3;
-#pragma unroll
-        for (int o = 0; o < TL; ++o)
-          pa[o] = kSeed ? bias_acc(bl + o * 32, hh) : (kSeedScaled ? bias_acc(bl + o * 32, hh) * lius : floatx16{0});
-        X3T(3);
-        if constexpr (kEarly) {
-          float mx;
-          x3_layer_early<T, TL, false, kPreSP>(x3, pipe, hb, pa, lane, bl, hh, ecs, lisc, lus, 0.f, mx);
-        } else if constexpr (kPre) {
-          x3_layer_pre<T, TL>(x3, pipe, sp, pa, lane);
-        } else if constexpr (kPipe) {
-          typename XT<NT>::E cs[NT];
-          splitk<NT, 0>(hb[0], cs);
-          halfx8 fs1[2];
-          x3_layer_pipe<NT, T, TL, !kSeedScaled, OACT, 0, kActIn ? ASET : 0>(x3, pipe, hb, pa, lane, bl, hh, cs, lisc,
-                                                                             lus, act, fs1);
-        } else {
-          x3_layer<NT, T, TL, kLastSW, OACT>(x3, pipe, hb, pa, lane, (kSeed || kSeedScaled) ? nullptr : bl, hh,
-                                             lisc, lus, act);
-        }
-        if constexpr (kSeedScaled) {
-#pragma unroll
-          for (int o = 0; o < TL; ++o) pa[o] *= lus;
-        }
-        if constexpr (T == 4) __builtin_amdgcn_s_setprio(0);
-        X3T(4);
-        constexpr bool kSplitWH = ONE && K == 16;
-        float P[NPV];
-#pragma unroll
-        for (int o = 0; o < TL; ++o)
-#pragma unroll
-          for (int r = 0; r < 16; ++r) {
-            if constexpr (kSplitWH) {
-              if (o == 0) P[r] = pa[0][r];
-              else
-                P[2 * K + r] = x3_halves(pa[1][r]).lo;
-            } else if constexpr (ONE) {
-              const X3Halves q = x3_halves(pa[o][r]);
-              P[32 * o + r] = q.lo;
-              P[32 * o + 16 + r] = q.hi;
-            } else {
-              P[16 * o + r] = pa[o][r];
-            }
-          }
-        X3M(11);
-#if ZF_X3_ABL == 10 || ZF_X3_ABL == 11
-#pragma unroll
-        for (int q2 = 0; q2 < 64; ++q2) {
-          float dd;
-          if (ZF_X3_ABL == 10) asm volatile("v_add_f32 %0, %1, %2" : "=v"(dd) : "v"(pa[0][q2 & 15]), "v"(pa[1][q2 & 15]));
-          else asm volatile("v_exp_f32 %0, %1" : "=v"(dd) : "v"(pa[0][q2 & 15]));
-        }
-#endif
-        const int d = 2 * pr + hh;
-        const bool dact = d < dt;
-        float ldv = 0.f;
-        {
-          float* xp = xs + wrap((dact ? d : 0) + rot, D) * 32 + s;
-          const float xv = *xp;
-#ifndef ZF_X3_BSEARCH
-#define ZF_X3_BSEARCH 0
-#endif
-          RqsBin bin;
-          bool binned = false;
-          if constexpr (ZF_X3_BSEARCH && !kSplitWH && !kPreSP && (K == 8 || K == 16 || K == 32 || K == 64)) {
-            if (klit) {
-              bin = x3_bin<!INV, K, OACT, true>(xv, P, kc);
-              binned = true;
-            }
-          }
-          if (!binned) {
-            float w[K], hg[K];
-            const float bc = kc.c * kc.rnorm;
-            if constexpr (kSplitWH) {
-              float sw = 0.f;
-#pragma unroll
-              for (int j = 0; j < K; ++j) {
-                w[j] = kPreSP ? P[j] : x3_squareplus2_t<OACT>(P[j]);
-                sw = sw + w[j];
-              }
-              const float a = rcp_refined(sw) * kc.rnorm;
-#pragma unroll
-              for (int j = 0; j < K; ++j) {
-                const X3Halves q = x3_halves(__builtin_fmaf(w[j], a, bc));
-                w[j] = q.lo;
-                hg[j] = q.hi;
-              }
-            } else {
-              float sx = 0.f, sy = 0.f;
-#pragma unroll
-              for (int j = 0; j < K; ++j) {
-                w[j] = kPreSP ? P[j] : x3_squareplus2_t<OACT>(P[j]);
-                hg[j] = kPreSP ? P[K + j] : x3_squareplus2_t<OACT>(P[K + j]);
-                sx = sx + w[j];
-                sy = sy + hg[j];
-              }
-              const float ax = rcp_refined(sx) * kc.rnorm, ay = rcp_refined(sy) * kc.rnorm;
-#pragma unroll
-              for (int j = 0; j < K; ++j) {
-                w[j] = __builtin_fmaf(w[j], ax, bc);
-                hg[j] = __builtin_fmaf(hg[j], ay, bc);
-              }
-            }
-            X3M(12);
-            float sl[K - 1];
-#pragma unroll
-            for (int j = 0; j < K - 1; ++j) sl[j] = P[2 * K + j];
-#ifndef ZF_X3_EXECBIN
-#define ZF_X3_EXECBIN 1
-#endif
-            const auto spf = [](float v) { return v == 0.f ? 1.f : x3_squareplus_t<OACT>(v); };
-            if constexpr (ZF_X3_EXECBIN && K % 8 == 0) bin = rqs_bin_exec<!INV, K>(xv, w, hg, sl, spf, padlast);
-            else bin = rqs_bin_monotone<!INV, K>(xv, w, hg, sl, spf, padlast);
-            X3M(13);
-          }
-          float yv;
-          if (!INV) {
-            float l;
-            x3_forward_eval(xv, bin, yv, l);
-            ldv = dact ? l : 0.f;
-          } else {
-            yv = rqs_inverse_eval(xv, bin);
-          }
-          if (dact) *xp = yv;
-        }
-        wave_lds_sync();
-        if (!INV) {
-          const X3Halves q = x3_halves(ldv);
-          ldn = ldn + q.lo;
-          if (2 * pr + 1 < dt) ldn = ldn + q.hi;
-        }
-      }
-      if (!INV) ld = ld + ldn;
-      X3T(5);
+      x3_nsc<NT, K, T, PAIRS, ONE, INV, OACT, ASET, false>(op, opc, x3, pipe, par, xs, rot, D, s, hh, lane, ld,
+                                                           tr);
     }
   }
 
@@ -1513,18 +1720,16 @@
                     ld_out, s_part);
 #ifdef ZF_X3_TRACE
   X3T(6);
-  tacc[7] = pipe.tbar;
-  tacc[11] = pipe.tdma;
-  tacc[12] = pipe.tgrp;
-  tacc[8] = t_last - t_begin;
+  tr.tacc[7] = pipe.tbar;
+  tr.tacc[11] = pipe.tdma;
+  tr.tacc[12] = pipe.tgrp;
+  tr.tacc[8] = tr.t_last - t_begin;
   if (lane == 0 && x3_trace_buf != nullptr) {
     unsigned long long* o = x3_trace_buf + ((long long)blockIdx.x * NW + wave) * kX3TraceSlots;
 #pragma unroll
-    for (int k = 0; k < kX3TraceSlots; ++k) o[k] = tacc[k];
-  }
-#endif
-#undef X3T
-#undef X3M
+    for (int k = 0; k < kX3TraceSlots; ++k) o[k] = tr.tacc[k];
+  }
+#endif
 }
 
 template <int NT, int K, int T, bool PAIRS, bool ONE, bool OACT, int ASET = 0>
@@ -1566,5 +1771,8 @@
   return enotsup("split-MFMA kernel: hidden tiles not instantiated");
 }
 
-}
-}
+#undef X3T
+#undef X3M
+
+}
+}
```

Result: faster. 1.411 billion, median of 6 (+5.4%).
